# mpkuse/rgbd_odometry

Measured on AMD Instinct MI355X. Metric: frame-pair aligns/sec (640x480, 4-lvl pyr), higher is better.
Workload: dtype f32

## Files before the change

include/dvo_amd.h:

```cpp
#ifndef DVO_AMD_H_
#define DVO_AMD_H_

#include <stddef.h>
#include <stdint.h>

#ifdef __cplusplus
extern "C" {
#endif

#define DVO_MAX_LEVELS 8
#define DVO_NUM_ACC 29

enum {
    DVO_OK = 0,
    DVO_ERR_INVALID = 1,
    DVO_ERR_NO_DEVICE = 2,
    DVO_ERR_HIP = 3,
    DVO_ERR_STATE = 4,
    DVO_ERR_NOMEM = 5
};

enum {
    DVO_FLAG_FINAL_OUTPUTS = 1,
    DVO_FLAG_IDENTITY_START = 2,
// ... 62 lines not shown
                                   float *xyz_out, float *uv_out, int capacity, int *N_out);

int  dvo_run_iterations(dvo_ctx *ctx, int level, int max_iters, double *R, double *t,
                        float *energy, float *final_eps, float *final_reproj,
                        int *best_idx, float *visible_ratio);
int  dvo_run_iterations_pair(dvo_ctx *ctx, int pair, int level, int max_iters, double *R, double *t,
                             float *energy, float *final_eps, float *final_reproj,
                             int *best_idx, float *visible_ratio);

int  dvo_align_pyramid(dvo_ctx *ctx, int n_levels, const int *iters, int flags, double *R, double *t);
int  dvo_align_batch(dvo_ctx *ctx, int first_pair, int n_pairs, int n_levels, const int *iters,
                     int flags, double *R, double *t);

int  dvo_set_poses(dvo_ctx *ctx, int first_pair, int n_pairs, const double *R, const double *t);
int  dvo_align_batch_enqueue(dvo_ctx *ctx, int first_pair, int n_pairs, int n_levels,
                             const int *iters, int flags);
int  dvo_get_poses(dvo_ctx *ctx, int first_pair, int n_pairs, double *R, double *t);

int  dvo_get_level_report(dvo_ctx *ctx, int pair, int level, float *energy, int n_energy,
                          int *best_idx, float *visible_ratio);
int  dvo_get_level_normal_matrix(dvo_ctx *ctx, int pair, int level, int itr, double *H36);
int  dvo_get_final_outputs(dvo_ctx *ctx, int pair, float *final_eps, float *final_reproj, int capacity,
                           int *N_out);

int  dvo_iter_begin(dvo_ctx *ctx, int pair, int level, int max_iters, const double *R, const double *t);
int  dvo_iter_accumulate(dvo_ctx *ctx, int pair, int level, int first_point, int n_points, double *d_acc32);
int  dvo_iter_update(dvo_ctx *ctx, int pair, int level, int itr, int n_total, const double *d_acc32);
int  dvo_iter_end(dvo_ctx *ctx, int pair, int level, double *R, double *t, float *energy ,
                  int *best_idx, float *visible_ratio);

int  dvo_align_pyramid_wide(dvo_ctx *ctx, int pair, int n_levels, const int *iters, int flags, double *R, double *t);

int  dvo_tiled_attach(dvo_ctx *ctx, void *nccl_comm, int rank, int world, const char *rccl_library);
int  dvo_tiled_detach(dvo_ctx *ctx);
int  dvo_align_pyramid_tiled(dvo_ctx *ctx, int pair, int n_levels, const int *iters, int flags, double *R, double *t);
int  dvo_tiled_shard(dvo_ctx *ctx, int pair, int level, int *first, int *count);
int  dvo_tiled_graph_replayed(dvo_ctx *ctx, int *graph_replayed);
int  dvo_wide_packed_levels(dvo_ctx *ctx, int *levels_mask, int *solo_mask);
int  dvo_wide_team_levels(dvo_ctx *ctx, int *levels_mask);

int  dvo_eval_points(dvo_ctx *ctx, int pair, int level, const double *R, const double *t,
                     float *reproj, float *J, float *eps, float *w, int *visible);
int  dvo_accumulate(dvo_ctx *ctx, int pair, int level, const double *R, const double *t,
                    double *acc29);
int  dvo_device_se3_exp(dvo_ctx *ctx, const double *psi6, double *R, double *t);
int  dvo_device_se3_log(dvo_ctx *ctx, const double *R, const double *t, double *psi6);
int  dvo_device_rotationize(dvo_ctx *ctx, double *R);

int  dvo_get_level_texel_mode(dvo_ctx *ctx, int pair, int level, int *mode);
int  dvo_get_level_exact_fallback(dvo_ctx *ctx, int pair, int level, int *ran);
int  dvo_get_level_energy_sweeps(dvo_ctx *ctx, int pair, int level, int *n);
int  dvo_get_level_points4(dvo_ctx *ctx, int pair, int level, int *used);
int  dvo_get_level_ranks_in_lds(dvo_ctx *ctx, int pair, int level, int *used);

int  dvo_get_last_launch_shape(dvo_ctx *ctx, int *block_threads, int *team_size, int *packed);

#define DVO_COMPACT_NOW_AFTER 16
int  dvo_now_prepare(dvo_ctx *ctx, int first_pair, int count);
int  dvo_set_direct_compact(dvo_ctx *ctx, int on);
int  dvo_get_now_compact_info(dvo_ctx *ctx, int pair, int level, int *palette_size);
int  dvo_get_now_compact_partial(dvo_ctx *ctx, int pair, int level, int *partial);

int  dvo_debug_stamps(dvo_ctx *ctx, int pair, unsigned long long *out64);

int  dvo_algorithmic_bytes(dvo_ctx *ctx, int pair, int n_levels, const int *iters, int flags,
                           uint64_t *bytes);
int  dvo_point_iterations(dvo_ctx *ctx, int pair, int n_levels, const int *iters, uint64_t *count);

enum { DVO_PIX_U8 = 0, DVO_PIX_U16 = 1, DVO_PIX_F32 = 2 };
enum { DVO_LAYOUT_COL_MAJOR = 0,
       DVO_LAYOUT_ROW_MAJOR = 1 };
enum { DVO_UPLOAD_ASYNC = 1,
       DVO_UPLOAD_DEPTH_RAW = 2,
       DVO_UPLOAD_DIRECT = 4 };
enum { DVO_UPLOAD_MAPPED = 16 };
void *dvo_host_alloc_mapped(size_t bytes);
void  dvo_host_free_mapped(void *p);
enum { DVO_UPLOAD_DEVICE = 8 };

typedef struct dvo_image {
    const void *data;
    int rows, cols;
    int dtype;
    int layout;
} dvo_image;

int  dvo_frames_reserve(dvo_ctx *ctx, int n_slots);
int  dvo_frames_upload_pyramids(dvo_ctx *ctx, int first_slot, int count, int n_levels,
                                const dvo_image *grey, const dvo_image *depth, int now_first_pair, int flags);
int  dvo_frames_set_undistort(dvo_ctx *ctx, int rows, int cols, const double *K4, const double *D5);
int  dvo_frames_upload_cameras(dvo_ctx *ctx, int first_slot, int count, const unsigned char *const *bgr8,
                               const float *const *depth_m, int rows, int cols, int n_levels, int first_shift,
                               int now_first_pair, int flags);
int  dvo_frames_as_now(dvo_ctx *ctx, int first_slot, int first_pair, int count);
int  dvo_frames_as_ref(dvo_ctx *ctx, int first_slot, int first_pair, int count, int *N_out);
int  dvo_frame_get_level(dvo_ctx *ctx, int slot, int level, int *rows, int *cols, unsigned char *grey,
                         float *depth_mm, unsigned char *edge, int *n_edges);
int  dvo_frames_num_levels(const dvo_ctx *ctx);

typedef struct dvo_photo_params {
    double fx, fy, cx, cy;
    int    gradient_threshold;
    int    max_jacobian_size;
    int    min_required_pts;
    int    iterations;
    double eps_norm_stop;
// ... 14 lines not shown
```

rgbd_odometry_amd/capi.py:

```python
from __future__ import annotations

import ctypes as C
import os
from typing import Optional, Sequence

import numpy as np

DVO_MAX_LEVELS = 8
DVO_NUM_ACC = 29
DVO_OK, DVO_ERR_INVALID, DVO_ERR_NO_DEVICE, DVO_ERR_HIP, DVO_ERR_STATE, DVO_ERR_NOMEM = range(6)
DVO_FLAG_FINAL_OUTPUTS = 1
DVO_FLAG_IDENTITY_START = 2
DVO_FLAG_NORMAL_MATRIX = 4

_HERE = os.path.dirname(os.path.abspath(__file__))

C_ABI_SYMBOLS = [
    "dvo_params_default", "dvo_create", "dvo_create_batch", "dvo_destroy", "dvo_last_error",
    "dvo_num_pairs", "dvo_set_stream", "dvo_use_own_stream", "dvo_synchronize", "dvo_set_keep_warm", "dvo_set_keep_warm2", "dvo_set_intrinsics",
    "dvo_set_ref_level", "dvo_set_ref_level_pair", "dvo_set_now_level", "dvo_set_now_level_pair",
    "dvo_set_ref_level_device", "dvo_set_now_level_device", "dvo_set_ref_level_from_images",
    "dvo_run_iterations", "dvo_run_iterations_pair", "dvo_align_pyramid", "dvo_align_batch",
    "dvo_set_poses", "dvo_align_batch_enqueue", "dvo_get_poses", "dvo_get_level_report",
    "dvo_get_final_outputs", "dvo_get_level_normal_matrix", "dvo_eval_points", "dvo_accumulate", "dvo_device_se3_exp",
    "dvo_device_se3_log", "dvo_device_rotationize", "dvo_algorithmic_bytes", "dvo_point_iterations",
    "dvo_debug_stamps", "dvo_get_level_texel_mode", "dvo_get_level_exact_fallback", "dvo_get_level_energy_sweeps", "dvo_get_level_points4", "dvo_get_level_ranks_in_lds", "dvo_now_prepare", "dvo_set_direct_compact", "dvo_host_alloc_mapped", "dvo_host_free_mapped", "dvo_get_now_compact_info", "dvo_get_now_compact_partial", "dvo_get_last_launch_shape", "dvo_replicate_pairs", "dvo_set_now_level_from_edges", "dvo_get_now_level", "dvo_iter_begin", "dvo_iter_accumulate", "dvo_iter_update", "dvo_iter_end",
    "dvo_align_pyramid_wide", "dvo_tiled_attach", "dvo_tiled_detach", "dvo_align_pyramid_tiled", "dvo_tiled_shard", "dvo_tiled_graph_replayed", "dvo_wide_packed_levels", "dvo_wide_team_levels",
    "dvo_get_ref_level", "dvo_frames_reserve", "dvo_frames_upload_pyramids", "dvo_frames_upload_cameras", "dvo_frames_set_undistort",
    "dvo_photo_params_default", "dvo_photo_configure", "dvo_photo_set_ref", "dvo_photo_align", "dvo_photo_get_jacobian", "dvo_frames_as_now",
    "dvo_frames_as_ref", "dvo_frame_get_level", "dvo_frames_num_levels",
]

DVO_PIX_U8, DVO_PIX_U16, DVO_PIX_F32 = 0, 1, 2
DVO_LAYOUT_COL_MAJOR, DVO_LAYOUT_ROW_MAJOR = 0, 1
DVO_UPLOAD_ASYNC = 1
DVO_UPLOAD_DEPTH_RAW = 2
DVO_UPLOAD_DIRECT = 4
DVO_UPLOAD_DEVICE = 8
DVO_UPLOAD_MAPPED = 16


class DvoImage(C.Structure):
    _fields_ = [("data", C.c_void_p), ("rows", C.c_int), ("cols", C.c_int), ("dtype", C.c_int), ("layout", C.c_int)]


class DvoParams(C.Structure):
    _fields_ = [
        ("beta", C.c_double), ("precond_rot", C.c_double), ("reg_lambda", C.c_double),
        ("step_a", C.c_double), ("step_b", C.c_double),
        ("step_decay_after", C.c_int), ("step_decay_offset", C.c_int),
        ("trust_radius", C.c_float), ("psi_norm_stop", C.c_float),
        ("enable_rotationize", C.c_int), ("enable_l2_reg", C.c_int), ("interpolate_dt", C.c_int),
        ("block_threads", C.c_int), ("points_in_flight", C.c_int), ("engine_variant", C.c_int),
        ("lds_point_bytes", C.c_int), ("debug_alias_mod", C.c_int),
        ("canny_threshold1", C.c_int), ("canny_threshold2", C.c_int), ("team_size", C.c_int),
    ]


class DvoPhotoParams(C.Structure):
    _fields_ = [("fx", C.c_double), ("fy", C.c_double), ("cx", C.c_double), ("cy", C.c_double),
                ("gradient_threshold", C.c_int), ("max_jacobian_size", C.c_int), ("min_required_pts", C.c_int),
                ("iterations", C.c_int), ("eps_norm_stop", C.c_double), ("fixed", C.c_int), ("reserved", C.c_int)]


class RcclComm:
    RCCL = "/opt/rocm/lib/librccl.so.1"

    class _Id(C.Structure):
        _fields_ = [("internal", C.c_char * 128)]

    @classmethod
    def _lib(cls):
        import torch
        lib = C.CDLL(cls.RCCL, mode=C.RTLD_GLOBAL)
        lib.ncclGetUniqueId.argtypes = [C.POINTER(cls._Id)]
        lib.ncclCommInitRank.argtypes = [C.POINTER(C.c_void_p), C.c_int, cls._Id, C.c_int]
        lib.ncclCommDestroy.argtypes = [C.c_void_p]
        return lib

# ... 95 lines not shown
        return _lib
    if os.environ.get("DVO_NO_TORCH", "0") != "1":
        import torch
    path = library_path()
    if not os.path.exists(path) and not os.environ.get("DVO_LIB_VARIANT"):
        _build_native()
    if not os.path.exists(path):
        raise FileNotFoundError(
            f"{path} not found: build the HIP extension first "
            "(python -c 'import __graft_entry__ as g; g.build()' or make -C rgbd_odometry_amd/csrc)")
    lib = C.CDLL(path)
    vp, ip, fp, dp = C.c_void_p, C.POINTER(C.c_int), C.POINTER(C.c_float), C.POINTER(C.c_double)
    i, f = C.c_int, C.c_float
    sig = {
        "dvo_params_default": [C.POINTER(DvoParams)],
        "dvo_create": [C.POINTER(DvoParams), C.POINTER(vp)],
        "dvo_create_batch": [C.POINTER(DvoParams), i, C.POINTER(vp)],
        "dvo_destroy": [vp],
        "dvo_num_pairs": [vp],
        "dvo_set_stream": [vp, vp],
        "dvo_use_own_stream": [vp],
        "dvo_synchronize": [vp],
        "dvo_set_keep_warm": [vp, i],
        "dvo_set_keep_warm2": [vp, i, i],
        "dvo_set_intrinsics": [vp, f, f, f, f],
        "dvo_set_ref_level": [vp, i, vp, i],
        "dvo_set_ref_level_pair": [vp, i, i, vp, i],
        "dvo_set_now_level": [vp, i, vp, vp, vp, i, i],
        "dvo_set_now_level_pair": [vp, i, i, vp, vp, vp, i, i],
        "dvo_set_ref_level_device": [vp, i, i, vp, i],
        "dvo_set_now_level_device": [vp, i, i, vp, vp, vp, i, i],
        "dvo_set_ref_level_from_images": [vp, i, i, vp, vp, i, i, vp, vp, i, ip],
        "dvo_run_iterations": [vp, i, i, vp, vp, vp, vp, vp, ip, fp],
        "dvo_run_iterations_pair": [vp, i, i, i, vp, vp, vp, vp, vp, ip, fp],
        "dvo_align_pyramid": [vp, i, ip, i, vp, vp],
        "dvo_align_batch": [vp, i, i, i, ip, i, vp, vp],
        "dvo_set_poses": [vp, i, i, vp, vp],
        "dvo_align_batch_enqueue": [vp, i, i, i, ip, i],
        "dvo_get_poses": [vp, i, i, vp, vp],
        "dvo_get_level_report": [vp, i, i, vp, i, ip, fp],
        "dvo_get_final_outputs": [vp, i, vp, vp, i, ip],
        "dvo_get_level_normal_matrix": [vp, i, i, i, vp],
        "dvo_eval_points": [vp, i, i, vp, vp, vp, vp, vp, vp, vp],
        "dvo_accumulate": [vp, i, i, vp, vp, vp],
        "dvo_device_se3_exp": [vp, vp, vp, vp],
        "dvo_device_se3_log": [vp, vp, vp, vp],
        "dvo_device_rotationize": [vp, vp],
        "dvo_debug_stamps": [vp, i, vp],
        "dvo_get_level_texel_mode": [vp, i, i, ip],
        "dvo_get_level_exact_fallback": [vp, i, i, ip],
        "dvo_get_level_energy_sweeps": [vp, i, i, ip],
        "dvo_get_level_points4": [vp, i, i, ip],
        "dvo_get_level_ranks_in_lds": [vp, i, i, ip],
        "dvo_now_prepare": [vp, i, i],
        "dvo_get_last_launch_shape": [vp, ip, ip, ip],
        "dvo_get_now_compact_info": [vp, i, i, ip],
        "dvo_get_now_compact_partial": [vp, i, i, ip],
        "dvo_set_direct_compact": [vp, i],
        "dvo_host_alloc_mapped": [C.c_size_t],
        "dvo_host_free_mapped": [vp],
        "dvo_replicate_pairs": [vp, i, i, i],
        "dvo_set_now_level_from_edges": [vp, i, i, vp, i, i],
        "dvo_get_now_level": [vp, i, i, vp, vp, vp],
        "dvo_iter_begin": [vp, i, i, i, vp, vp],
        "dvo_iter_accumulate": [vp, i, i, i, i, vp],
        "dvo_iter_update": [vp, i, i, i, i, vp],
        "dvo_iter_end": [vp, i, i, vp, vp, vp, ip, fp],
        "dvo_align_pyramid_wide": [vp, i, i, ip, i, vp, vp],
        "dvo_frames_set_undistort": [vp, i, i, vp, vp],
        "dvo_photo_params_default": [C.POINTER(DvoPhotoParams)],
        "dvo_photo_configure": [vp, C.POINTER(DvoPhotoParams)],
        "dvo_photo_set_ref": [vp, i, i, ip],
        "dvo_photo_align": [vp, i, ip, i, vp, vp, ip],
        "dvo_photo_get_jacobian": [vp, i, vp, vp, vp, i, vp, ip],
        "dvo_tiled_attach": [vp, vp, i, i, C.c_char_p],
        "dvo_tiled_detach": [vp],
        "dvo_align_pyramid_tiled": [vp, i, i, ip, i, vp, vp],
        "dvo_tiled_shard": [vp, i, i, ip, ip],
        "dvo_tiled_graph_replayed": [vp, ip],
        "dvo_wide_packed_levels": [vp, ip, ip],
        "dvo_wide_team_levels": [vp, ip],
        "dvo_get_ref_level": [vp, i, i, vp, i, ip],
        "dvo_frames_reserve": [vp, i],
        "dvo_frames_upload_pyramids": [vp, i, i, i, C.POINTER(DvoImage), C.POINTER(DvoImage), i, i],
        "dvo_frames_upload_cameras": [vp, i, i, C.POINTER(vp), C.POINTER(vp), i, i, i, i, i, i],
        "dvo_frames_as_now": [vp, i, i, i],
        "dvo_frames_as_ref": [vp, i, i, i, ip],
        "dvo_frame_get_level": [vp, i, i, ip, ip, vp, vp, vp, ip],
        "dvo_frames_num_levels": [vp],
        "dvo_algorithmic_bytes": [vp, i, i, ip, i, C.POINTER(C.c_uint64)],
        "dvo_point_iterations": [vp, i, i, ip, C.POINTER(C.c_uint64)],
    }
    for name, args in sig.items():
        fn = getattr(lib, name)
        fn.argtypes = args
        fn.restype = C.c_int
    lib.dvo_last_error.argtypes = [vp]
    lib.dvo_last_error.restype = C.c_char_p
    lib.dvo_host_alloc_mapped.restype = C.c_void_p
    lib.dvo_host_free_mapped.restype = None
    _lib = lib
    return lib


def _f32(a) -> np.ndarray:
    return np.ascontiguousarray(a, dtype=np.float32)
# ... 417 lines not shown
        psi = np.array(psi, dtype=np.float64)
        R = np.zeros((3, 3), order="F")
        t = np.zeros(3)
        self._chk(self.lib.dvo_device_se3_exp(self._h, _ptr(psi), _ptr(R), _ptr(t)))
        return R, t

    def se3_log(self, R, t):
        R = np.array(R, dtype=np.float64, order="F")
        t = np.array(t, dtype=np.float64)
        psi = np.zeros(6)
        self._chk(self.lib.dvo_device_se3_log(self._h, _ptr(R), _ptr(t), _ptr(psi)))
        return psi

    def rotationize(self, R):
        R = np.array(R, dtype=np.float64, order="F").copy(order="F")
        self._chk(self.lib.dvo_device_rotationize(self._h, _ptr(R)))
        return R

    def debug_stamps(self, pair: int = 0) -> np.ndarray:
        out = np.zeros(64, np.uint64)
        self._chk(self.lib.dvo_debug_stamps(self._h, pair, _ptr(out)))
        return out.reshape(8, 8)

    def level_normal_matrix(self, pair: int, level: int, itr: int = -1) -> np.ndarray:
        H = np.zeros(36, np.float64)
        self._chk(self.lib.dvo_get_level_normal_matrix(self._h, pair, level, itr, _ptr(H)))
        return H.reshape(6, 6)

    def level_texel_mode(self, pair: int, level: int) -> int:
        m = C.c_int(-2)
        self._chk(self.lib.dvo_get_level_texel_mode(self._h, pair, level, C.byref(m)))
        return m.value

    def level_energy_sweeps(self, pair: int, level: int) -> int:
        m = C.c_int(0)
        self._chk(self.lib.dvo_get_level_energy_sweeps(self._h, pair, level, C.byref(m)))
        return m.value

    def level_exact_fallback(self, pair: int, level: int) -> bool:
        m = C.c_int(0)
        self._chk(self.lib.dvo_get_level_exact_fallback(self._h, pair, level, C.byref(m)))
        return bool(m.value)

    def level_points4(self, pair: int, level: int) -> bool:
        m = C.c_int(0)
        self._chk(self.lib.dvo_get_level_points4(self._h, pair, level, C.byref(m)))
        return bool(m.value)

    def level_ranks_in_lds(self, pair: int, level: int) -> bool:
        m = C.c_int(0)
        self._chk(self.lib.dvo_get_level_ranks_in_lds(self._h, pair, level, C.byref(m)))
        return bool(m.value)

    def last_launch_shape(self):
        b, t, k = C.c_int(0), C.c_int(0), C.c_int(0)
        self._chk(self.lib.dvo_get_last_launch_shape(self._h, C.byref(b), C.byref(t), C.byref(k)))
        return b.value, t.value, bool(k.value)

    def now_prepare(self, first_pair: int = 0, count: Optional[int] = None):
        count = self.n_pairs - first_pair if count is None else count
        self._chk(self.lib.dvo_now_prepare(self._h, first_pair, count))

    def set_direct_compact(self, on: bool = True):
        self._chk(self.lib.dvo_set_direct_compact(self._h, 1 if on else 0))

    def now_compact_info(self, pair: int, level: int) -> int:
        m = C.c_int(0)
        self._chk(self.lib.dvo_get_now_compact_info(self._h, pair, level, C.byref(m)))
        return m.value

    def now_compact_partial(self, pair: int, level: int) -> bool:
        m = C.c_int(0)
        self._chk(self.lib.dvo_get_now_compact_partial(self._h, pair, level, C.byref(m)))
        return bool(m.value)

    def algorithmic_bytes(self, iters: Sequence[int], pair: int = 0, flags: int = 0) -> int:
        b = C.c_uint64(0)
        self._chk(self.lib.dvo_algorithmic_bytes(self._h, pair, len(iters), _iters(iters), flags, C.byref(b)))
        return b.value

    def point_iterations(self, iters: Sequence[int], pair: int = 0) -> int:
        b = C.c_uint64(0)
        self._chk(self.lib.dvo_point_iterations(self._h, pair, len(iters), _iters(iters), C.byref(b)))
        return b.value
```

rgbd_odometry_amd/csrc/dvo_capi.cpp:

```cpp
#include "dvo_ctx.h"
#include "dvo_palette.h"

#include <atomic>
#include <chrono>
#include <thread>

using namespace dvo;


namespace { thread_local std::string g_create_error; }

namespace dvo_host {

int fail(dvo_ctx *c, int code, const std::string &msg) {
    if (c) c->err = msg; else g_create_error = msg;
    return code;
}

hipError_t stream_wait(hipStream_t s) {
    static const bool block = [] { const char *e = std::getenv("DVO_WAIT"); return e && std::strcmp(e, "block") == 0; }();
    if (!block) {
        const auto t0 = std::chrono::steady_clock::now();
        for (int n = 0;; n++) {
            const hipError_t e = hipStreamQuery(s);
// ... 139 lines not shown
    HIPCHK(c, hipMemcpyAsync(pn.data(), L.d_pal_n + first, sizeof(int) * (size_t)count, hipMemcpyDeviceToHost, stream));
    HIPCHK(c, stream_wait(stream));
    if (L.p4_known.empty()) { L.p4_known.assign(c->n_pairs, Level::P4_UNKNOWN); L.p4_fresh.assign(c->n_pairs, 0); }
    auto needs_tex = [&](int v) { return v <= 0 || pal_partial(v); };
    for (int i = 0; i < count; i++) {
        L.p4_known[first + i] = pn[i] <= 0 ? Level::P4_REFUSED : (pal_partial(pn[i]) ? Level::P4_PARTIAL : Level::P4_OK);
        L.p4_fresh[first + i] = 1;
    }
    int n = 0;
    for (int i = 0; i < count; ) {
        if (!needs_tex(pn[i])) { i++; continue; }
        int j = i;
        while (j < count && needs_tex(pn[j])) j++;
        const int rc = map_texels(c, level, first + i, j - i, stream);
        if (rc) return rc;
        n += j - i;
        i = j;
    }
    *n_failed = n;
    return DVO_OK;
}
int refresh_p4_known(dvo_ctx *c, int level, int first, int count, bool skip_native) {
    Level &L = c->lv[level];
    if (!L.d_pal_n || L.pal_built.empty()) return DVO_OK;
    if (L.p4_known.empty()) { L.p4_known.assign(c->n_pairs, Level::P4_UNKNOWN); L.p4_fresh.assign(c->n_pairs, 0); }
    if (L.p4_native.empty()) L.p4_native.assign(c->n_pairs, 0);
    auto unknown = [&](int p) { return L.pal_built[p] && L.p4_known[p] == Level::P4_UNKNOWN && !(skip_native && L.p4_native[p]); };
    for (int p = first; p < first + count; ) {
        if (!unknown(p)) { p++; continue; }
        int q = p;
        while (q < first + count && unknown(q)) q++;
        std::vector<int> pn((size_t)(q - p));
        HIPCHK(c, hipMemcpyAsync(pn.data(), L.d_pal_n + p, sizeof(int) * (size_t)(q - p), hipMemcpyDeviceToHost, c->stream));
        HIPCHK(c, stream_wait(c->stream));
        for (int i = p; i < q; i++) {
            const int v = pn[i - p];
            L.p4_known[i] = v <= 0 ? Level::P4_REFUSED : (pal_partial(v) ? Level::P4_PARTIAL : Level::P4_OK);
            if ((v <= 0 || pal_partial(v)) && !L.tex16_stale.empty()) L.tex16_stale[i] = 0;
        }
        p = q;
    }
    return DVO_OK;
}

int ensure_texels(dvo_ctx *c, int level, int rows, int cols) {
    Level &L = c->lv[level];
    if (L.have_now.empty()) L.have_now.assign(c->n_pairs, 0);
    if (L.tex && L.rows == rows && L.cols == cols) return DVO_OK;
    if (L.tex) {
        HIPCHK(c, stream_wait(c->stream));
        free_texels(c, L);
        std::fill(L.have_now.begin(), L.have_now.end(), 0);
        if (L.p4) { (void)hipFree(L.p4); (void)hipFree(L.pal); (void)hipFree(L.d_pal_n); L.p4 = nullptr; L.pal = nullptr; L.d_pal_n = nullptr; }
        L.pal_built.clear(); L.now_uses.clear(); L.tex16_stale.clear(); L.p4_known.clear(); L.p4_fresh.clear(); L.p4_native.clear();
    }

    L.rows = rows; L.cols = cols;
    L.tex_stride = texel_count(rows, cols);
    const size_t bytes = sizeof(float4) * L.tex_stride * c->n_pairs;
    if (tex_sparse_wanted(bytes)) {
        hipMemAllocationProp prop = {};
        prop.type = hipMemAllocationTypePinned;
        prop.location.type = hipMemLocationTypeDevice;
        prop.location.id = c->device;
        size_t gran = 0;
        void *va = nullptr;
        if (hipMemGetAllocationGranularity(&gran, &prop, hipMemAllocationGranularityMinimum) == hipSuccess && gran > 0) {
            const size_t chunk = ((((size_t)16 << 20) + gran - 1) / gran) * gran;
            const size_t va_bytes = (bytes + chunk - 1) / chunk * chunk;
            if (hipMemAddressReserve(&va, va_bytes, chunk, nullptr, 0) == hipSuccess && va) {
                L.tex = reinterpret_cast<float4 *>(va);
                L.tex_sparse = true; L.tex_chunk = chunk; L.tex_va_bytes = va_bytes;
                L.tex_handles.assign(va_bytes / chunk, hipMemGenericAllocationHandle_t{});
                L.tex_mapped.assign(va_bytes / chunk, 0);
                return DVO_OK;
            }
        }
        (void)hipGetLastError();
    }
    HIPCHK(c, hipMalloc((void **)&L.tex, bytes));
    if (L.tex_stride != (size_t)rows * cols)
        HIPCHK(c, hipMemsetAsync(L.tex, 0, bytes, c->stream));
    return DVO_OK;
}

static void level_flags(dvo_ctx *c, Level &L) {
    if (L.pal_built.empty()) { L.pal_built.assign(c->n_pairs, 0); L.now_uses.assign(c->n_pairs, 0); }
    if (L.tex16_stale.empty()) L.tex16_stale.assign(c->n_pairs, 0);
    if (L.have_now.empty()) L.have_now.assign(c->n_pairs, 0);
    if (L.p4_known.empty()) { L.p4_known.assign(c->n_pairs, Level::P4_UNKNOWN); L.p4_fresh.assign(c->n_pairs, 0); }
    if (L.p4_native.empty()) L.p4_native.assign(c->n_pairs, 0);
}

bool native_compact_wanted(const dvo_ctx *c) { return c->prm.engine_variant != 4 && compact_now_policy() != 2; }
static bool direct_compact_wanted(const dvo_ctx *c) {
    const char *e = getenv("DVO_DIRECT_COMPACT");
    const bool on = e ? !strcmp(e, "on") : (c->direct_compact < 0 ? c->n_pairs >= 64 : c->direct_compact != 0);
    return native_compact_wanted(c) && on;
}
static bool p4_addressable(int rows, int cols) {
    return !(p4_count(rows, cols) * sizeof(unsigned) >= ((size_t)1 << 32) || rows >= (1 << 16) || ((cols + 3) >> 2) >= (1 << 24) ||
             (size_t)p4_tiles_per_col(rows) * 128 >= ((size_t)1 << 24));
}

int ensure_compact_slabs(dvo_ctx *c, int level) {
    Level &L = c->lv[level];
    if (L.p4) return DVO_OK;
    L.p4_stride = p4_count(L.rows, L.cols);
    HIPCHK(c, hipMalloc((void **)&L.p4, sizeof(unsigned) * L.p4_stride * c->n_pairs));
    HIPCHK(c, hipMalloc((void **)&L.pal, sizeof(float2) * DVO_PAL_MAX * (size_t)c->n_pairs));
    HIPCHK(c, hipMalloc((void **)&L.d_pal_n, sizeof(int) * (size_t)c->n_pairs));
    HIPCHK(c, hipMemsetAsync(L.d_pal_n, 0, sizeof(int) * (size_t)c->n_pairs, c->stream));
    HIPCHK(c, stream_wait(c->stream));
    return DVO_OK;
}

int now_written_compact(dvo_ctx *c, int level, int first_pair, int count) {
    Level &L = c->lv[level];
    level_flags(c, L);
    for (int p = first_pair; p < first_pair + count; p++) {
        L.have_now[p] = 1; L.now_uses[p] = 0; L.pal_built[p] = 1;
        L.p4_native[p] = 1;
        if (L.p4_fresh[p]) L.p4_fresh[p] = 0;
        else L.p4_known[p] = Level::P4_UNKNOWN;
        L.tex16_stale[p] = (L.p4_known[p] == Level::P4_REFUSED || L.p4_known[p] == Level::P4_PARTIAL) ? 0 : 1;
    }
    return DVO_OK;
}

int ensure_tex16(dvo_ctx *c, int level, int first_pair, int count) {
    Level &L = c->lv[level];
    if (L.tex16_stale.empty() || !L.p4) return DVO_OK;
    for (int p = first_pair; p < first_pair + count; ) {
        if (!L.tex16_stale[p]) { p++; continue; }
        int q = p;
        while (q < first_pair + count && L.tex16_stale[q]) q++;
        { const int mrc = map_texels(c, level, p, q - p); if (mrc) return mrc; }
        HIPCHK(c, launch_p4_decode_texels(L.p4, L.p4_stride, L.pal, L.d_pal_n, L.tex, L.tex_stride, L.rows, L.cols, p, q - p, c->stream));
        for (int i = p; i < q; i++) L.tex16_stale[i] = 0;
        p = q;
    }
    return DVO_OK;
}

int now_written(dvo_ctx *c, int level, int first_pair, int count) {
    Level &L = c->lv[level];
    level_flags(c, L);
    for (int p = first_pair; p < first_pair + count; p++) { L.tex16_stale[p] = 0; L.p4_known[p] = Level::P4_UNKNOWN; L.p4_fresh[p] = 0; L.p4_native[p] = 0; }
    for (int p = first_pair; p < first_pair + count; ) {
        L.have_now[p] = 1; L.now_uses[p] = 0;
        if (!L.pal_built[p]) { p++; continue; }
        int q = p;
        while (q < first_pair + count && L.pal_built[q]) { L.pal_built[q] = 0; L.have_now[q] = 1; L.now_uses[q] = 0; q++; }
        HIPCHK(c, hipMemsetAsync(L.d_pal_n + p, 0, sizeof(int) * (size_t)(q - p), c->stream));
        p = q;
    }
    return DVO_OK;
}

int build_compact_now(dvo_ctx *c, int level, int first_pair, int count, bool only_reused) {
    Level &L = c->lv[level];
    if (!L.tex || L.have_now.empty()) return DVO_OK;
    if (p4_count(L.rows, L.cols) * sizeof(unsigned) >= ((size_t)1 << 32) || L.rows >= (1 << 16) || ((L.cols + 3) >> 2) >= (1 << 24) ||
        (size_t)p4_tiles_per_col(L.rows) * 128 >= ((size_t)1 << 24))
        return DVO_OK;
    level_flags(c, L);
    for (int p = first_pair; p < first_pair + count; ) {
        auto wanted = [&](int i) { return L.have_now[i] && !L.pal_built[i] && (!only_reused || L.now_uses[i] >= DVO_COMPACT_NOW_AFTER); };
        if (!wanted(p)) { p++; continue; }
        int q = p;
        while (q < first_pair + count && wanted(q)) q++;
        { const int rc = ensure_compact_slabs(c, level); if (rc) return rc; }
        for (int b = p; b < q; b += 1024) {
            const int nb = std::min(1024, q - b);
            if (palette_work_ints(nb) > c->pal_work_ints) {
                if (c->pal_work) { HIPCHK(c, stream_wait(c->stream)); HIPCHK(c, hipFree(c->pal_work)); c->pal_work = nullptr; c->pal_work_ints = 0; }
                HIPCHK(c, hipMalloc((void **)&c->pal_work, sizeof(unsigned) * palette_work_ints(nb)));
                c->pal_work_ints = palette_work_ints(nb);
            }
            HIPCHK(c, launch_palette_build(L.tex, L.tex_stride, L.rows, L.cols, L.p4, L.p4_stride, L.pal, L.d_pal_n, b, nb, c->pal_work, c->stream));
        }
        for (int i = p; i < q; i++) { L.pal_built[i] = 1; L.p4_known[i] = Level::P4_UNKNOWN; if (!L.p4_native.empty()) L.p4_native[i] = 0; }
        p = q;
    }
    return DVO_OK;
}

}

using namespace dvo_host;

namespace dvo_host {

LevelSlab slab_of(const dvo_ctx *c, int level) {
    const Level &L = c->lv[level];
    LevelSlab s;
    s.tex = L.tex; s.pts = L.pts; s.cpts = L.cpts; s.cidx = L.cidx; s.N = L.dN;
    s.cpt4 = L.cpt4; s.chdr = L.chdr; s.pt4_ok = L.d_pt4_ok;
    s.tex_stride = L.tex_stride; s.pt_cap = L.pt_cap; s.rows = L.rows; s.cols = L.cols;
    s.p4 = L.p4; s.pal = L.pal; s.pal_n = L.d_pal_n; s.p4_stride = L.p4_stride;
    return s;
}

int check_ready(dvo_ctx *c, int pair, int level) {
    if (!c->have_K) return fail(c, DVO_ERR_STATE, "intrinsics not set (dvo_set_intrinsics)");
    const Level &L = c->lv[level];
    if (L.hN.empty() || L.hN[pair] <= 0)
        return fail(c, DVO_ERR_STATE, "reference points of pair " + std::to_string(pair) + " level " +
                                          std::to_string(level) + " not set");
    if (L.have_now.empty() || !L.have_now[pair])
        return fail(c, DVO_ERR_STATE, "now level " + std::to_string(level) + " of pair " +
                                          std::to_string(pair) + " not set");
    return DVO_OK;
}

int build_schedule(dvo_ctx *c, int n_levels, const int *iters, int flags, Schedule &sc) {
    if (n_levels < 1 || n_levels > DVO_LEVELS || !iters) return fail(c, DVO_ERR_INVALID, "bad level schedule");
    std::memset(&sc, 0, sizeof(sc));
    sc.n_levels = n_levels;
    sc.flags = flags;
    sc.last_level = -1;
    int off = 0;
    for (int l = 0; l < n_levels; l++) {
        sc.iters[l] = iters[l] > 0 ? iters[l] : 0;
        sc.e_off[l] = off;
        off += sc.iters[l];
    }
    for (int l = n_levels - 1; l >= 0; l--) if (sc.iters[l] > 0) sc.last_level = l;
    if (sc.last_level < 0) return fail(c, DVO_ERR_INVALID, "schedule has no iterations");
    sc.e_stride = off;
    return DVO_OK;
}

int ensure_outputs(dvo_ctx *c, const Schedule &sc) {
    const size_t need = (size_t)sc.e_stride * c->n_pairs;
    if (need > c->energy_floats) {
        if (c->d_energy) { HIPCHK(c, stream_wait(c->stream)); HIPCHK(c, hipFree(c->d_energy)); }
        HIPCHK(c, hipMalloc((void **)&c->d_energy, sizeof(float) * need));
        c->energy_floats = need;
        c->sched_gen++;
    }
    if (sc.flags & DVO_FLAG_NORMAL_MATRIX) {
        const size_t needH = need * 21;
        if (needH > c->H_doubles) {
            if (c->d_H) { HIPCHK(c, stream_wait(c->stream)); HIPCHK(c, hipFree(c->d_H)); }
            HIPCHK(c, hipMalloc((void **)&c->d_H, sizeof(double) * needH));
            c->H_doubles = needH;
            c->sched_gen++;
        }
    }
    if (sc.flags & DVO_FLAG_FINAL_OUTPUTS) {
        const int cap = c->lv[sc.last_level].pt_cap;
        if (cap > c->final_cap) {
// ... 136 lines not shown
            for (int p = first_pair; p < first_pair + n_pairs; p++) max_n = std::max(max_n, c->lv[l].hN[p]);
        }
        if ((size_t)max_n * 12 <= 77000 && !c->prm.interpolate_dt && 2 * n_pairs > c->n_cu) { block = 256; auto_lds = 80 * 1024; }
        else if (all_p4 && 2 * n_pairs >= 3 * c->n_cu && (size_t)max_n * 8 <= 2 * (size_t)77000) { block = 256; auto_lds = 80 * 1024; }
        else if (all_p4 && n_pairs > c->n_cu) { block = 256; auto_lds = 80 * 1024; }
        else if ((size_t)max_n * 12 > 4 * (size_t)155000 && !c->prm.interpolate_dt) { block = 1024; auto_lds = 155000; }
        else { block = 512; auto_lds = 155000; }
    }
    {
        int bytes = c->prm.lds_point_bytes;
        if (bytes == 0) bytes = auto_lds ? auto_lds : ((block >= 512) ? 155000 : 80 * 1024);
        if (packed && block_auto && block == 1024) block = 512;
        const int static_lds = packed ? (int)fused2_static_lds(block, with_h) : (int)(sizeof(double) * (block / 64) * DVO_NACC_PAD + 256 + pose_state_bytes());
        const int max_dyn = ((block == 256) ? 80 * 1024 : 160 * 1024) - static_lds - 64;
        if (bytes > max_dyn) bytes = max_dyn;
        if (bytes < 0) bytes = 0;
        bytes &= ~63;
        sc.lds_bytes = bytes;
        sc.no_lds_tex = (c->prm.engine_variant == 2) ? 1 : 0;
        sc.force_exact = (c->prm.engine_variant == 3) ? 1 : 0;
        sc.force_e2 = (c->prm.engine_variant == 5) ? 1 : 0;
        static const bool no_pt4_env = [] { const char *e = std::getenv("DVO_POINTS4"); return e && std::strcmp(e, "off") == 0; }();
        sc.no_pt4 = no_pt4_env ? 1 : 0;
        static const int pt4_factor_env = [] { const char *e = std::getenv("DVO_POINTS4_FACTOR"); return e ? std::atoi(e) : 1; }();
        sc.pt4_factor = pt4_factor_env;
        for (int l = 0; l < n_levels && !sc.no_pt4; l++) {
            if (sc.iters[l] <= 0 || c->lv[l].pt4_rows.empty()) continue;
            const Level &L = c->lv[l];
            for (int p = first_pair; p < first_pair + n_pairs; p++) {
                const int dp = sc.alias_mod > 0 ? p % sc.alias_mod : p;
                if (L.pt4_rows[dp] != 0 && L.pt4_rows[dp] != L.rows) { sc.no_pt4 = 1; break; }
            }
        }
        sc.lds_points = bytes / (sc.compact ? 8 : 12);
        if (c->prm.lds_point_bytes < 0) { sc.lds_points = 0; sc.lds_bytes = 0; }
    }
    if (!packed || sc.no_p4 || (size_t)sc.lds_bytes < sizeof(float2) * DVO_PAL_MAX + 64) {
        if (!packed) sc.no_p4 = 1;
        for (int l = 0; l < n_levels; l++) {
            if (sc.iters[l] <= 0) continue;
            if ((rc = ensure_tex16(c, l, first_pair, n_pairs))) return rc;
            if (sc.alias_mod > 0 && (rc = ensure_tex16(c, l, 0, std::min(sc.alias_mod, c->n_pairs)))) return rc;
        }
    }
    int u = c->prm.points_in_flight;
    if (u != 1 && u != 2 && u != 4) u = 1;
    sc.team = 1;
    sc.n_pairs_launch = n_pairs;
    {
        static const bool no_plain = [] { const char *e = std::getenv("DVO_TEAM_PLAIN_STORES"); return e && std::strcmp(e, "off") == 0; }();
        sc.team_no_plain = no_plain ? 1 : 0;
        static const bool no_r16 = [] { const char *e = std::getenv("DVO_RANKS_LDS"); return e && std::strcmp(e, "off") == 0; }();
        sc.no_r16 = no_r16 ? 1 : 0;
        static const int solo_max = [] { const char *e = std::getenv("DVO_TEAM_SOLO_MAX"); return e ? std::atoi(e) : DVO_TEAM_SOLO_MAX_DEFAULT; }();
        sc.team_solo_max = solo_max;
    }
    c->team_used = false;
    if (sc.compact && c->prm.engine_variant != 1 && !(sc.flags & DVO_FLAG_NORMAL_MATRIX) && block == 512 && c->prm.team_size != 1) {
        const int slots8 = 8 * ((n_pairs + 7) / 8);
        int n_fine = 0;
        for (int p = first_pair; p < first_pair + n_pairs; p++) n_fine = std::max(n_fine, c->lv[sc.last_level].hN[p]);
        const int g_cap = (n_fine >= 262144) ? 32 : ((n_fine >= 65536) ? 16 : 8);
        int g = 1;
        if (n_fine >= 5000)
            while (g * 2 <= g_cap && slots8 * g * 2 <= c->n_cu && n_fine >= 1800 * g * 2) g *= 2;
        bool super_team = (n_pairs == 1 && n_fine >= 100000 && c->n_cu >= 256);
        if (super_team) g = (n_fine >= 400000) ? 256 : 64;
        if (c->prm.team_size > 1) {
            g = c->prm.team_size;
            super_team = (g == 64 || g == 128 || g == 256) && n_pairs == 1;
            if (super_team ? (g > c->n_cu) : (g > 32 || slots8 * g > c->n_cu))
                return fail(c, DVO_ERR_INVALID, "team_size: the launch would need more workgroups than compute units (members must be co-resident; 64 / 128 / 256 only for a single pair)");
        }
        if (g > 1) {
            const size_t buf_bytes = 16 * 2 * 32 * 8 * (size_t)std::max(c->n_pairs, 9);
            bool zero = false;
            if (!c->d_team_buf) {
                HIPCHK(c, hipMalloc((void **)&c->d_team_buf, buf_bytes));
                HIPCHK(c, hipMalloc((void **)&c->d_team_cnt, sizeof(unsigned) * ((size_t)c->n_pairs + 1)));
                zero = c->team_err_dirty = true;
                if (const char *e = std::getenv("DVO_TEAM_EPOCH0")) c->team_epoch = (unsigned)std::strtoul(e, nullptr, 0);
            }
            unsigned need = 2;
            for (int l = 0; l < n_levels; l++) if (sc.iters[l] > 0) need += 2u * (unsigned)sc.iters[l] + 2u;
            hipStreamCaptureStatus cap = hipStreamCaptureStatusNone;
            if (c->stream && hipStreamIsCapturing(c->stream, &cap) == hipSuccess && cap != hipStreamCaptureStatusNone) c->team_legacy = true;
            if (c->team_legacy || c->team_epoch > 0xfffffff0u - need) zero = true;
            if (zero) {
                HIPCHK(c, hipMemsetAsync(c->d_team_buf, 0, buf_bytes, c->stream));
                if (c->team_legacy || c->team_epoch > 0xfffffff0u - need) c->team_epoch = 0;
            }
            if (c->team_err_dirty || c->team_legacy) {
                HIPCHK(c, hipMemsetAsync(c->d_team_cnt, 0, sizeof(unsigned) * ((size_t)c->n_pairs + 1), c->stream));
                c->team_err_dirty = false;
            }
            sc.team_epoch0 = c->team_epoch;
            if (!c->team_legacy) c->team_epoch += need;
            sc.team = g;
            c->team_used = true;
        }
    }
    if (packed) {
        Outputs o = outputs_of(c);
        static const bool no_lpt = std::getenv("DVO_NO_LPT") != nullptr;
        if (sc.team == 1 && n_pairs > c->n_cu && !no_lpt) {
            unsigned long long sched_hash = 1469598103934665603ull;
// ... 136 lines not shown
struct dvo_keep_warm_state {
    std::thread th;
    std::atomic<bool> stop{false};
    hipStream_t stream = nullptr;
    int busy_us = 0, pause_us = 0;
};
static void keep_warm_stop(dvo_ctx *c) {
    dvo_keep_warm_state *w = c->warm;
    if (!w) return;
    w->stop.store(true);
    if (w->th.joinable()) w->th.join();
    if (w->stream) { (void)hipStreamSynchronize(w->stream); (void)hipStreamDestroy(w->stream); }
    delete w;
    c->warm = nullptr;
}
int dvo_set_keep_warm2(dvo_ctx *c, int busy_us, int pause_us) {
    DVO_ENTER(c);
    keep_warm_stop(c);
    if (busy_us <= 0) return DVO_OK;
    dvo_keep_warm_state *w = new dvo_keep_warm_state();
    w->busy_us = busy_us; w->pause_us = pause_us < 0 ? 0 : pause_us;
    if (hipStreamCreateWithFlags(&w->stream, hipStreamNonBlocking) != hipSuccess) { delete w; return fail(c, DVO_ERR_HIP, "keep-warm: cannot create a stream"); }
    const int device = c->device;
    w->th = std::thread([w, device]() {
        (void)hipSetDevice(device);
        while (!w->stop.load()) {
            (void)launch_keep_warm(w->busy_us, w->stream);
            if (w->pause_us == 0) (void)launch_keep_warm(w->busy_us, w->stream);
            (void)hipStreamSynchronize(w->stream);
            if (w->pause_us > 0) std::this_thread::sleep_for(std::chrono::microseconds(w->pause_us));
        }
    });
    c->warm = w;
    return DVO_OK;
}
int dvo_set_keep_warm(dvo_ctx *c, int period_us) {
    return dvo_set_keep_warm2(c, period_us > 0 ? 5 : 0, period_us);
}

int dvo_destroy(dvo_ctx *c) {
    if (!c) return DVO_OK;
    DeviceGuard guard(c);
    keep_warm_stop(c);
    if (c->stream) (void)stream_wait(c->stream);
    for (int l = 0; l < DVO_LEVELS; l++) {
        free_texels(c, c->lv[l]);
        if (c->lv[l].pts) (void)hipFree(c->lv[l].pts);
        if (c->lv[l].cpts) (void)hipFree(c->lv[l].cpts);
        if (c->lv[l].cidx) (void)hipFree(c->lv[l].cidx);
        if (c->lv[l].cpt4) { (void)hipFree(c->lv[l].cpt4); (void)hipFree(c->lv[l].chdr); }
        if (c->lv[l].d_pt4_ok) (void)hipFree(c->lv[l].d_pt4_ok);
        if (c->lv[l].dN) (void)hipFree(c->lv[l].dN);
        if (c->lv[l].p4) { (void)hipFree(c->lv[l].p4); (void)hipFree(c->lv[l].pal); (void)hipFree(c->lv[l].d_pal_n); }
    }
    if (c->pal_work) (void)hipFree(c->pal_work);
    if (c->d_order) (void)hipFree(c->d_order);
    tiled_forget(c);
    photo_forget(c);
    for (int l = 0; l < DVO_LEVELS; l++) {
        FrameLevel &F = c->fs.lv[l];
        void *fp[] = {F.grey, F.edge, F.depth};
        for (void *p : fp) if (p) (void)hipFree(p);
    }
    if (c->work) (void)hipFree(c->work);
    if (c->d_umap_xy) (void)hipFree(c->d_umap_xy);
    if (c->d_umap_frac) (void)hipFree(c->d_umap_frac);
    if (c->wide_exec) (void)hipGraphExecDestroy(c->wide_exec);
    if (c->tiled_exec) (void)hipGraphExecDestroy(c->tiled_exec);
    if (c->d_step_state) { (void)hipFree(c->d_step_state); (void)hipFree(c->d_step_acc); (void)hipFree(c->d_step_ticket); }
    if (c->h_pose) (void)hipHostFree(c->h_pose);
    if (c->h_poses) (void)hipHostFree(c->h_poses);
    for (int l = 0; l < DVO_LEVELS; l++) {
        if (c->lvl_stream[l]) { (void)hipStreamSynchronize(c->lvl_stream[l]); (void)hipStreamDestroy(c->lvl_stream[l]); }
        if (c->ev_join[l]) (void)hipEventDestroy(c->ev_join[l]);
    }
    if (c->ev_fork) (void)hipEventDestroy(c->ev_fork);
    if (c->copy_stream) { (void)hipStreamSynchronize(c->copy_stream); (void)hipStreamDestroy(c->copy_stream); }
    if (c->copy_stream2) { (void)hipStreamSynchronize(c->copy_stream2); (void)hipStreamDestroy(c->copy_stream2); }
    for (int b = 0; b < 2; b++) {
        if (c->up_buf[b]) (void)hipFree(c->up_buf[b]);
        if (b == 0) { if (c->src_tab_dev) (void)hipFree(c->src_tab_dev); if (c->src_tab_host) (void)hipHostFree(c->src_tab_host); if (c->ev_src_tab) (void)hipEventDestroy(c->ev_src_tab); }
        if (c->up_host[b]) (void)hipHostFree(c->up_host[b]);
        if (c->ev_copied[b]) (void)hipEventDestroy(c->ev_copied[b]);
        if (c->ev_copied2[b]) (void)hipEventDestroy(c->ev_copied2[b]);
        if (c->ev_done[b]) (void)hipEventDestroy(c->ev_done[b]);
    }
    void *ptrs[] = {c->staging, c->d_poses, c->d_energy, c->d_best, c->d_ratio, c->d_final_eps,
                    c->d_final_reproj, c->d_final_N, c->d_scratch, c->d_colcounts, c->d_dbg,
                    c->d_states, c->d_iter_energy, c->d_tex_mode, c->d_H, c->d_team_buf, c->d_team_cnt};
    for (void *p : ptrs) if (p) (void)hipFree(p);
    if (c->own_stream) (void)hipStreamDestroy(c->own_stream);
    delete c;
    return DVO_OK;
}

const char *dvo_last_error(const dvo_ctx *c) { return c ? c->err.c_str() : g_create_error.c_str(); }
int dvo_num_pairs(const dvo_ctx *c) { return c ? c->n_pairs : 0; }

int dvo_set_stream(dvo_ctx *c, void *hip_stream) {
    DVO_ENTER(c);
    HIPCHK(c, stream_wait(c->stream));
    c->stream = (hipStream_t)hip_stream;
    return DVO_OK;
}
int dvo_use_own_stream(dvo_ctx *c) {
    DVO_ENTER(c);
// ... 150 lines not shown
            HIPCHK(c, hipMemcpyAsync(c->h_poses, L.d_pal_n + pair, sizeof(int), hipMemcpyDeviceToHost, c->stream));
        }
    }
    if (!device_src) {
        HIPCHK(c, stream_wait(c->stream));
        if (direct && *reinterpret_cast<const int *>(c->h_poses) <= 0) L.pal_built[pair] = 0;
    }
    return DVO_OK;
}
void *dvo_host_alloc_mapped(size_t bytes) {
    void *p = nullptr;
    if (bytes == 0 || hipHostMalloc(&p, bytes, hipHostMallocMapped | hipHostMallocPortable) != hipSuccess) { (void)hipGetLastError(); return nullptr; }
    return p;
}
void dvo_host_free_mapped(void *p) { if (p) (void)hipHostFree(p); }

int dvo_set_direct_compact(dvo_ctx *c, int on) {
    DVO_ENTER(c);
    c->direct_compact = on ? 1 : 0;
    return DVO_OK;
}
int dvo_set_now_level_pair(dvo_ctx *c, int pair, int level, const float *dt, const float *gx,
                           const float *gy, int rows, int cols) {
    return set_now_common(c, pair, level, dt, gx, gy, rows, cols, false);
}
int dvo_set_now_level(dvo_ctx *c, int level, const float *dt, const float *gx, const float *gy,
                      int rows, int cols) {
    return set_now_common(c, 0, level, dt, gx, gy, rows, cols, false);
}
int dvo_set_now_level_device(dvo_ctx *c, int pair, int level, const float *d_dt, const float *d_gx,
                             const float *d_gy, int rows, int cols) {
    return set_now_common(c, pair, level, d_dt, d_gx, d_gy, rows, cols, true);
}

int dvo_set_now_level_from_edges(dvo_ctx *c, int pair, int level, const unsigned char *edge, int rows, int cols) {
    DVO_ENTER(c);
    if (!pair_ok(c, pair) || !level_ok(level)) return fail(c, DVO_ERR_INVALID, "pair/level out of range");
    if (!edge || rows < 1 || cols < 1) return fail(c, DVO_ERR_INVALID, "bad image arguments");
    if ((long long)rows + cols + 1 > 46340) return fail(c, DVO_ERR_INVALID, "image too large for the exact distance transform (rows + cols must stay below 46339)");
    int rc = ensure_texels(c, level, rows, cols);
    if (rc) return rc;
    const size_t npx = (size_t)rows * cols;
    bool any = false;
    for (size_t i = 0; i < npx && !any; i++) any = edge[i] != 0;
    if (!any) return fail(c, DVO_ERR_INVALID, "edge mask has no edge pixel: the distance transform is undefined");
    const size_t edge_ints = (npx + 3) / 4;
    if ((rc = ensure_staging(c, sizeof(int) * (edge_ints + edt_work_ints(rows, cols, 1) + 1)))) return rc;
    unsigned char *d_edge = (unsigned char *)c->staging;
    int *work = (int *)c->staging + edge_ints;
    HIPCHK(c, hipMemcpyAsync(d_edge, edge, npx, hipMemcpyHostToDevice, c->stream));
    Level &L = c->lv[level];
    const bool compact = native_compact_wanted(c);
    if (compact && (rc = ensure_compact_slabs(c, level))) return rc;
    const bool defer = compact && L.tex_sparse;
    if (L.tex_sparse && !compact && (rc = map_texels(c, level, pair, 1))) return rc;
    HIPCHK(c, launch_edges_to_now(d_edge, 0, ImgBatch{rows, cols, 1}, work, defer ? nullptr : L.tex + (size_t)pair * L.tex_stride, L.tex_stride,
                                  compact ? L.p4 : nullptr, L.p4_stride, L.pal, L.d_pal_n, pair, c->stream));
    if (defer) {
        int n_failed = 0;
        if ((rc = sparse_map_compact_failures(c, level, pair, 1, c->stream, &n_failed))) return rc;
        if (n_failed)
            HIPCHK(c, launch_edges_to_now(d_edge, 0, ImgBatch{rows, cols, 1}, work, L.tex + (size_t)pair * L.tex_stride, L.tex_stride,
                                          L.p4, L.p4_stride, L.pal, L.d_pal_n, pair, c->stream, true));
    }
    if ((rc = compact ? now_written_compact(c, level, pair, 1) : now_written(c, level, pair, 1))) return rc;
    HIPCHK(c, stream_wait(c->stream));
    return DVO_OK;
}

int dvo_get_now_level(dvo_ctx *c, int pair, int level, float *dt, float *gx, float *gy) {
    DVO_ENTER(c);
    if (!pair_ok(c, pair) || !level_ok(level)) return fail(c, DVO_ERR_INVALID, "pair/level out of range");
    Level &L = c->lv[level];
    if (L.have_now.empty() || !L.have_now[pair]) return fail(c, DVO_ERR_STATE, "now level not set");
    const size_t npx = (size_t)L.rows * L.cols;
    int rc = ensure_staging(c, sizeof(float) * 3 * npx);
    if (rc) return rc;
    if ((rc = ensure_tex16(c, level, pair, 1))) return rc;
    float *d = c->staging;
    HIPCHK(c, launch_unpack_texels(L.tex + (size_t)pair * L.tex_stride, L.rows, L.cols, d, d + npx, d + 2 * npx, c->stream));
    if (dt) HIPCHK(c, hipMemcpyAsync(dt, d, sizeof(float) * npx, hipMemcpyDeviceToHost, c->stream));
    if (gx) HIPCHK(c, hipMemcpyAsync(gx, d + npx, sizeof(float) * npx, hipMemcpyDeviceToHost, c->stream));
    if (gy) HIPCHK(c, hipMemcpyAsync(gy, d + 2 * npx, sizeof(float) * npx, hipMemcpyDeviceToHost, c->stream));
    HIPCHK(c, stream_wait(c->stream));
    return DVO_OK;
}

int dvo_get_ref_level(dvo_ctx *c, int pair, int level, float *xyz_out, int capacity, int *N_out) {
    DVO_ENTER(c);
    if (!pair_ok(c, pair) || !level_ok(level)) return fail(c, DVO_ERR_INVALID, "pair/level out of range");
    Level &L = c->lv[level];
    if (L.hN.empty() || L.hN[pair] <= 0) return fail(c, DVO_ERR_STATE, "reference level not set");
    const int N = L.hN[pair];
    if (N_out) *N_out = N;
    const int ncopy = std::min(N, capacity);
    if (xyz_out && ncopy > 0) {
        HIPCHK(c, hipMemcpyAsync(xyz_out, L.pts + (size_t)pair * L.pt_cap * 3, sizeof(float) * 3 * (size_t)ncopy,
                                 hipMemcpyDeviceToHost, c->stream));
        HIPCHK(c, stream_wait(c->stream));
    }
    return DVO_OK;
}

int dvo_replicate_pairs(dvo_ctx *c, int n_src, int dst_first, int dst_count) {
    DVO_ENTER(c);
    if (n_src < 1 || dst_first < 0 || dst_count < 0 || dst_first + dst_count > c->n_pairs || n_src > c->n_pairs)
        return fail(c, DVO_ERR_INVALID, "bad replicate arguments");
    if (dst_first != 0 && dst_first < n_src) return fail(c, DVO_ERR_INVALID, "destination range overlaps the sources");
    for (int l = 0; l < DVO_LEVELS; l++) {
        Level &L = c->lv[l];
        if (!L.tex && !L.pts) continue;
        for (int p = 0; p < n_src; p++) {
            int rc = check_ready(c, p, l);
            if (rc) return rc;
        }
        { const int prc = refresh_p4_known(c, l, 0, n_src); if (prc) return prc; }
        bool any_tex16 = false, any_compact = false;
        for (int p = 0; p < n_src; p++) {
            const bool stale = !L.tex16_stale.empty() && L.tex16_stale[p];
            any_tex16 = any_tex16 || !stale;
            any_compact = any_compact || (!L.pal_built.empty() && L.pal_built[p]);
        }
        unsigned char *d_has_tex = nullptr;
        if (any_tex16 && L.tex) {
            std::vector<unsigned char> has((size_t)n_src);
            bool all = true;
            for (int p = 0; p < n_src; p++) { has[p] = !(!L.tex16_stale.empty() && L.tex16_stale[p]); all = all && has[p]; }
            for (int p = 0; p < n_src; p++)
                if (has[p]) { const int mrc = map_texels(c, l, p, 1); if (mrc) return mrc; }
            for (int p = dst_first; p < dst_first + dst_count; ) {
                if (!has[(p - dst_first) % n_src]) { p++; continue; }
                int q = p;
                while (q < dst_first + dst_count && has[(q - dst_first) % n_src]) q++;
                const int mrc = map_texels(c, l, p, q - p);
                if (mrc) return mrc;
                p = q;
            }
            if (!all) {
                HIPCHK(c, hipMalloc((void **)&d_has_tex, (size_t)n_src));
                HIPCHK(c, hipMemcpyAsync(d_has_tex, has.data(), (size_t)n_src, hipMemcpyHostToDevice, c->stream));
                HIPCHK(c, stream_wait(c->stream));
            }
        }
        {
            const hipError_t le = launch_replicate_level(any_tex16 ? L.tex : nullptr, d_has_tex, L.tex_stride, L.pts, L.cpts, L.cidx, L.cpt4, L.chdr, L.d_pt4_ok,
                                                         L.pt_cap, L.dN, n_src, dst_first, dst_count, c->stream);
            if (d_has_tex) { (void)hipStreamSynchronize(c->stream); (void)hipFree(d_has_tex); }
            HIPCHK(c, le);
        }
        for (int p = dst_first; p < dst_first + dst_count; p++) {
            const int src = (p - dst_first) % n_src;
            if (src == p) continue;
            L.hN[p] = L.hN[src];
            ref_list_written(c, l, p, 1, L.pt4_rows.empty() ? 0 : L.pt4_rows[src]);
            L.compact_ok[p] = L.compact_ok[src];
        }
        const int w_first = (dst_first == 0) ? std::min(n_src, dst_count) : dst_first;
        const int w_count = dst_first + dst_count - w_first;
        if (L.tex && w_count > 0) {
            int rc = now_written(c, l, w_first, w_count);
            if (rc) return rc;
            if (any_compact) {
                HIPCHK(c, launch_replicate_compact(L.p4, L.p4_stride, L.pal, L.d_pal_n, n_src, dst_first, dst_count, c->stream));
                for (int p = dst_first; p < dst_first + dst_count; p++) {
                    const int src = (p - dst_first) % n_src;
                    if (p == src) continue;
                    L.pal_built[p] = L.pal_built[src];
                    L.tex16_stale[p] = L.tex16_stale[src];
                    L.p4_known[p] = L.p4_known[src];
                    if (!L.p4_native.empty()) L.p4_native[p] = L.p4_native[src];
                }
            }
        }
    }
    HIPCHK(c, stream_wait(c->stream));
    return DVO_OK;
}

int dvo_get_last_launch_shape(dvo_ctx *c, int *block_threads, int *team_size, int *packed) {
    DVO_ENTER(c);
    if (block_threads) *block_threads = c->last_block;
    if (team_size) *team_size = c->last_team;
    if (packed) *packed = c->last_packed;
    return DVO_OK;
}

int dvo_now_prepare(dvo_ctx *c, int first_pair, int count) {
    DVO_ENTER(c);
    if (!pair_ok(c, first_pair) || count < 1 || first_pair + count > c->n_pairs) return fail(c, DVO_ERR_INVALID, "pair range out of bounds");
    if (c->prm.engine_variant == 4 || compact_now_policy() == 2) return DVO_OK;
    for (int l = 0; l < DVO_LEVELS; l++) {
        int rc = build_compact_now(c, l, first_pair, count, false);
        if (rc) return rc;
    }
    HIPCHK(c, stream_wait(c->stream));
    return DVO_OK;
}

int dvo_get_now_compact_info(dvo_ctx *c, int pair, int level, int *palette_size) {
    DVO_ENTER(c);
    if (!pair_ok(c, pair) || !level_ok(level) || !palette_size) return fail(c, DVO_ERR_INVALID, "bad arguments");
    Level &L = c->lv[level];
    *palette_size = 0;
    if (!L.d_pal_n) return DVO_OK;
    HIPCHK(c, hipMemcpyAsync(palette_size, L.d_pal_n + pair, sizeof(int), hipMemcpyDeviceToHost, c->stream));
    HIPCHK(c, stream_wait(c->stream));
    if (*palette_size > 0) *palette_size = pal_count(*palette_size);
    return DVO_OK;
}
int dvo_get_now_compact_partial(dvo_ctx *c, int pair, int level, int *partial) {
    DVO_ENTER(c);
    if (!pair_ok(c, pair) || !level_ok(level) || !partial) return fail(c, DVO_ERR_INVALID, "bad arguments");
    Level &L = c->lv[level];
    *partial = 0;
    if (!L.d_pal_n) return DVO_OK;
    int v = 0;
// ... 596 lines not shown
    HIPCHK(c, hipMemcpyAsync(psi6, d + 16, sizeof(double) * 6, hipMemcpyDeviceToHost, c->stream));
    HIPCHK(c, stream_wait(c->stream));
    return DVO_OK;
}
int dvo_device_rotationize(dvo_ctx *c, double *R) {
    DVO_ENTER(c);
    if (!R) return DVO_ERR_INVALID;
    double *d = c->d_scratch;
    HIPCHK(c, hipMemcpyAsync(d, R, sizeof(double) * 9, hipMemcpyHostToDevice, c->stream));
    HIPCHK(c, launch_rotationize(d, c->stream));
    HIPCHK(c, hipMemcpyAsync(R, d, sizeof(double) * 9, hipMemcpyDeviceToHost, c->stream));
    HIPCHK(c, stream_wait(c->stream));
    return DVO_OK;
}

int dvo_debug_stamps(dvo_ctx *c, int pair, unsigned long long *out64) {
    DVO_ENTER(c);
    if (!out64 || !pair_ok(c, pair)) return DVO_ERR_INVALID;
    std::memset(out64, 0, sizeof(unsigned long long) * 64);
    if (!c->d_dbg) return DVO_OK;
    HIPCHK(c, stream_wait(c->stream));
    HIPCHK(c, hipMemcpy(out64, c->d_dbg + (size_t)pair * 64, sizeof(unsigned long long) * 64, hipMemcpyDeviceToHost));
    HIPCHK(c, hipMemset(c->d_dbg + (size_t)pair * 64, 0, sizeof(unsigned long long) * 64));
    return DVO_OK;
}

int dvo_get_level_texel_mode(dvo_ctx *c, int pair, int level, int *mode) {
    DVO_ENTER(c);
    if (!pair_ok(c, pair) || !level_ok(level) || !mode) return fail(c, DVO_ERR_INVALID, "bad arguments");
    HIPCHK(c, stream_wait(c->stream));
    int v = -1;
    HIPCHK(c, hipMemcpy(&v, c->d_tex_mode + (size_t)pair * DVO_LEVELS + level, sizeof(int), hipMemcpyDeviceToHost));
    *mode = (v < 0) ? -1 : (v & 0xff);
    return DVO_OK;
}
int dvo_get_level_points4(dvo_ctx *c, int pair, int level, int *used) {
    DVO_ENTER(c);
    if (!pair_ok(c, pair) || !level_ok(level) || !used) return fail(c, DVO_ERR_INVALID, "bad arguments");
    HIPCHK(c, stream_wait(c->stream));
    int v = -1;
    HIPCHK(c, hipMemcpy(&v, c->d_tex_mode + (size_t)pair * DVO_LEVELS + level, sizeof(int), hipMemcpyDeviceToHost));
    *used = (v >= 0 && (v & DVO_TEXMODE_PT4)) ? 1 : 0;
    return DVO_OK;
}
int dvo_get_level_ranks_in_lds(dvo_ctx *c, int pair, int level, int *used) {
    DVO_ENTER(c);
    if (!pair_ok(c, pair) || !level_ok(level) || !used) return fail(c, DVO_ERR_INVALID, "bad arguments");
    HIPCHK(c, stream_wait(c->stream));
    int v = -1;
    HIPCHK(c, hipMemcpy(&v, c->d_tex_mode + (size_t)pair * DVO_LEVELS + level, sizeof(int), hipMemcpyDeviceToHost));
    *used = (v >= 0 && (v & DVO_TEXMODE_RANKS_LDS)) ? 1 : 0;
    return DVO_OK;
}
int dvo_get_level_exact_fallback(dvo_ctx *c, int pair, int level, int *ran) {
    DVO_ENTER(c);
    if (!pair_ok(c, pair) || !level_ok(level) || !ran) return fail(c, DVO_ERR_INVALID, "bad arguments");
    HIPCHK(c, stream_wait(c->stream));
    int v = -1;
    HIPCHK(c, hipMemcpy(&v, c->d_tex_mode + (size_t)pair * DVO_LEVELS + level, sizeof(int), hipMemcpyDeviceToHost));
    *ran = (v >= 0 && (v & DVO_TEXMODE_EXACT_RAN)) ? 1 : 0;
    return DVO_OK;
}

int dvo_get_level_energy_sweeps(dvo_ctx *c, int pair, int level, int *n) {
    DVO_ENTER(c);
    if (!pair_ok(c, pair) || !level_ok(level) || !n) return fail(c, DVO_ERR_INVALID, "bad arguments");
    HIPCHK(c, stream_wait(c->stream));
    int v = -1;
    HIPCHK(c, hipMemcpy(&v, c->d_tex_mode + (size_t)pair * DVO_LEVELS + level, sizeof(int), hipMemcpyDeviceToHost));
    *n = (v < 0) ? 0 : ((v >> DVO_TEXMODE_E2_SHIFT) & DVO_TEXMODE_E2_MAX);
    return DVO_OK;
}

int dvo_algorithmic_bytes(dvo_ctx *c, int pair, int n_levels, const int *iters, int flags, uint64_t *bytes) {
    DVO_ENTER(c);
    if (!bytes) return DVO_ERR_INVALID;
    if (!pair_ok(c, pair)) return fail(c, DVO_ERR_INVALID, "pair out of range");
    Schedule sc;
    int rc = build_schedule(c, n_levels, iters, flags, sc);
    if (rc) return rc;
    uint64_t b = 0;
    for (int l = 0; l < n_levels; l++) {
        if (sc.iters[l] <= 0) continue;
        if ((rc = check_ready(c, pair, l))) return rc;
        b += 12ull * (uint64_t)c->lv[l].rows * (uint64_t)c->lv[l].cols;
        b += 12ull * (uint64_t)c->lv[l].hN[pair];
    }
    if (flags & DVO_FLAG_FINAL_OUTPUTS) b += 16ull * (uint64_t)c->lv[sc.last_level].hN[pair];
    *bytes = b;
    return DVO_OK;
}

int dvo_point_iterations(dvo_ctx *c, int pair, int n_levels, const int *iters, uint64_t *count) {
    DVO_ENTER(c);
    if (!count) return DVO_ERR_INVALID;
    if (!pair_ok(c, pair)) return fail(c, DVO_ERR_INVALID, "pair out of range");
    Schedule sc;
    int rc = build_schedule(c, n_levels, iters, 0, sc);
    if (rc) return rc;
    uint64_t n = 0;
    for (int l = 0; l < n_levels; l++) {
        if (sc.iters[l] <= 0) continue;
        if ((rc = check_ready(c, pair, l))) return rc;
        n += (uint64_t)sc.iters[l] * (uint64_t)c->lv[l].hN[pair];
    }
    *count = n;
// ... 5 lines not shown
```

rgbd_odometry_amd/csrc/dvo_ctx.h:

```cpp
#ifndef DVO_CTX_H_
#define DVO_CTX_H_

#include "../../include/dvo_amd.h"
#include "dvo_launch.h"

#include <algorithm>
#include <cmath>
#include <cstdio>
#include <cstdlib>
#include <cstring>
#include <functional>
#include <string>
#include <vector>

namespace dvo_host {

struct Level {
    int rows = 0, cols = 0;
    float4 *tex = nullptr;
    size_t tex_stride = 0;
    bool tex_sparse = false;
    size_t tex_chunk = 0, tex_va_bytes = 0;
    std::vector<hipMemGenericAllocationHandle_t> tex_handles;
    std::vector<char> tex_mapped;
    float *pts = nullptr;
    uint2 *cpts = nullptr;
    unsigned *cidx = nullptr;
    unsigned *cpt4 = nullptr;
    unsigned *chdr = nullptr;
    int *d_pt4_ok = nullptr;
    std::vector<char> compact_ok;
    std::vector<unsigned long long> list_gen;
    std::vector<int> pt4_rows;
    int pt_cap = 0;
    int *dN = nullptr;
    std::vector<int> hN;
    std::vector<char> have_now;
    unsigned *p4 = nullptr;
    float2 *pal = nullptr;
    int *d_pal_n = nullptr;
    size_t p4_stride = 0;
    std::vector<char> pal_built;
    std::vector<int> now_uses;
    std::vector<char> tex16_stale;
    enum : char { P4_UNKNOWN = 0, P4_OK = 1, P4_REFUSED = 2, P4_PARTIAL = 3  };
    std::vector<char> p4_known;
    std::vector<char> p4_native;
    std::vector<char> p4_fresh;
};

struct FrameLevel {
    int rows = 0, cols = 0;
    size_t npx = 0;
    unsigned char *grey = nullptr, *edge = nullptr;
    float *depth = nullptr;
};
struct FrameStore {
    int n_slots = 0, n_levels = 0;
    FrameLevel lv[DVO_LEVELS];
    std::vector<char> valid, has_depth;
};
inline bool compact_block_order() {
    static const bool on = [] { const char *e = std::getenv("DVO_COMPACT_ORDER"); return !(e && std::strcmp(e, "colmajor") == 0); }();
    return on;
}
inline int compact_now_policy() {
    static const int pol = [] {
        const char *e = std::getenv("DVO_COMPACT_NOW");
        return (e && std::strcmp(e, "eager") == 0) ? 1 : ((e && std::strcmp(e, "off") == 0) ? 2 : 0);
    }();
    return pol;
}
}

struct dvo_ctx {
    dvo_params prm;
    dvo::DevParams dprm;
    int n_pairs = 0;
    int device = 0;
    int n_cu = 256;
    hipStream_t stream = nullptr;
    hipStream_t own_stream = nullptr;
    dvo::Intrinsics K{0, 0, 0, 0, 0};
    bool have_K = false;
    dvo_host::Level lv[DVO_LEVELS];
    float *staging = nullptr;
    size_t staging_bytes = 0;
    double *d_poses = nullptr;
    float *d_energy = nullptr;
    size_t energy_floats = 0;
    int *d_best = nullptr;
    float *d_ratio = nullptr;
    float *d_final_eps = nullptr, *d_final_reproj = nullptr;
    int *d_final_N = nullptr;
// ... 134 lines not shown
```

rgbd_odometry_amd/csrc/dvo_edt_band.h:

```cpp
#ifndef DVO_EDT_BAND_H_
#define DVO_EDT_BAND_H_

constexpr int EB_PAD = 8;
constexpr unsigned EB_D2_END = 32000;
constexpr int EB_LUT_WORDS = (int)(EB_D2_END / 32);
constexpr int EB_TRIPS = 23;
constexpr int EB_NANR = 1;
constexpr int EB_MAX_ROWS = 512, EB_MAX_COLS = 1024;
static_assert(EB_D2_END % 32 == 0 && (8 * EB_TRIPS + 1) * (8 * EB_TRIPS + 1) >= (int)EB_D2_END && (8 * EB_TRIPS + 1) * (8 * EB_TRIPS + 1) < 65536, "scan radius");

struct EdtSosLut { unsigned bm[EB_LUT_WORDS]; unsigned short pre[EB_LUT_WORDS]; int total; };
constexpr EdtSosLut edt_sos_lut_make() {
    EdtSosLut t{};
    for (unsigned a = 0; a * a < EB_D2_END; a++)
        for (unsigned b = a; a * a + b * b < EB_D2_END; b++) { const unsigned v = a * a + b * b; t.bm[v >> 5] |= 1u << (v & 31u); }
    int run = 0;
    for (int w = 0; w < EB_LUT_WORDS; w++) {
        t.pre[w] = (unsigned short)run;
        unsigned v = t.bm[w];
        while (v) { v &= v - 1u; run++; }
    }
    t.total = run;
    return t;
}
__device__ const EdtSosLut EDT_SOS_LUT = edt_sos_lut_make();
static_assert(edt_sos_lut_make().total + 4 <= DVO_PAL_MAX, "every rank + the two fixed entries + the two entries a consumer copies beyond pal_n fit the 13-bit field");

struct EdtBandLevels {
    int n, first_pair;
    int rows[DVO_LEVELS], cols[DVO_LEVELS], nwords[DVO_LEVELS], nbands[DVO_LEVELS], tpc[DVO_LEVELS], n_partial[DVO_LEVELS];
    unsigned firstA[DVO_LEVELS + 1], firstB[DVO_LEVELS + 1];
    const unsigned char *edge[DVO_LEVELS]; size_t edge_stride[DVO_LEVELS];
    unsigned *maskT[DVO_LEVELS], *carryT[DVO_LEVELS];
    unsigned *imax[DVO_LEVELS]; int *done[DVO_LEVELS]; int *flags[DVO_LEVELS];
    const int *partial[DVO_LEVELS];
    unsigned *p4[DVO_LEVELS]; size_t p4_stride[DVO_LEVELS]; float2 *pal[DVO_LEVELS]; int *pal_n[DVO_LEVELS];
    int *list;
};

DVO_DEV unsigned eb_load_mask8(const unsigned char *col, bool vec, int y0, int rows) {
    if (y0 >= rows) return 0u;
    if (vec) {
        const uint2 v = *reinterpret_cast<const uint2 *>(col + y0);
        return edt_nonzero_bytes(v.x) | (edt_nonzero_bytes(v.y) << 4);
    }
    unsigned m = 0;
    for (int j = 0; j < 8; j++) if (y0 + j < rows && col[y0 + j] != 0) m |= 1u << j;
    return m;
}

__global__ void __launch_bounds__(512) edt_colmask_levels_kernel(const EdtBandLevels t) {
    __shared__ unsigned sm[16][33], sc[16][33];
    const int l = level_of_block(t.firstA, t.n, blockIdx.x);
    const int bx = (int)(blockIdx.x - t.firstA[l]), by = blockIdx.y;
    const int rows = t.rows[l], cols = t.cols[l], nwords = t.nwords[l];
    const int tid = threadIdx.x, lane = tid & 63, wave = tid >> 6;
    if (bx == 0 && tid == 0) { t.imax[l][by] = 0u; t.done[l][by] = 0; t.flags[l][by] = 0; }
    if (blockIdx.x == 0 && by == 0 && tid == 0) t.list[0] = 0;
    const unsigned char *img = t.edge[l] + (size_t)by * t.edge_stride[l];
    const int INF = DVO_EDT_INF(rows, cols);
    const int x0 = bx * 32;
    unsigned m8[4];
#pragma unroll
    for (int k = 0; k < 4; k++) {
        const int xx = x0 + wave + 8 * k;
        const unsigned char *col = img + (size_t)(xx < cols ? xx : 0) * rows;
        const unsigned m = eb_load_mask8(col, ((rows & 7) == 0) && ((reinterpret_cast<size_t>(col) & 7) == 0), lane * 8, rows);
        m8[k] = xx < cols ? m : 0u;
    }
    const int w = lane >> 2;
#pragma unroll
    for (int k = 0; k < 4; k++) {
        const unsigned long long bal = __ballot(m8[k] != 0u);
        unsigned v = m8[k] | ((unsigned)__shfl_down((int)m8[k], 1) << 8);
        v |= (unsigned)__shfl_down((int)v, 2) << 16;
        const unsigned long long lower = bal & ((1ull << (4 * w)) - 1ull);
        const unsigned long long upper = (w == 15) ? 0ull : (bal & (~0ull << (4 * w + 4)));
        const int lpu = lower ? 63 - __clzll((long long)lower) : 0;
        const int lpd = upper ? __ffsll((long long)upper) - 1 : 0;
        const unsigned mlu = (unsigned)__shfl((int)m8[k], lpu), mld = (unsigned)__shfl((int)m8[k], lpd);
        const int U = lower ? (32 * w - 1) - (lpu * 8 + (31 - __clz((int)mlu))) : INF;
        const int D = upper ? (lpd * 8 + (__ffs((int)mld) - 1)) - 32 * (w + 1) : INF;
        if ((lane & 3) == 0) { sm[w][wave + 8 * k] = v; sc[w][wave + 8 * k] = (unsigned)U | ((unsigned)D << 16); }
    }
    __syncthreads();
    unsigned *mk = t.maskT[l] + (size_t)by * nwords * cols, *cr = t.carryT[l] + (size_t)by * nwords * cols;
    for (int idx = tid; idx < nwords * 32; idx += 512) {
        const int ww = idx >> 5, c = idx & 31, xx = x0 + c;
        if (xx < cols) { mk[(size_t)ww * cols + xx] = sm[ww][c]; cr[(size_t)ww * cols + xx] = sc[ww][c]; }
// ... 188 lines not shown
    EDT_T(t_scanned);
#pragma unroll
    for (int it = 0; it < NI; it++) {
        const int p = it * THREADS + tid;
        if (p < total) {
            const int h = p & (LPC - 1), col = p / LPC;
            eb_lds4[(size_t)(EB_PAD + col) * C4 + h] = res[it];
            if (col == 1) eb_lds4[(size_t)(EB_PAD - 1) * C4 + h] = res[it];
            if (col == cols - 2) eb_lds4[(size_t)(EB_PAD + cols) * C4 + h] = res[it];
        }
    }
    __syncthreads();

    const int tpc = t.tpc[l], ntc = (cols + 3) >> 2;
    const int ty0 = band * T, nty = (tpc - ty0 < T) ? tpc - ty0 : T;
    unsigned *p4 = t.p4[l] + (size_t)(t.first_pair + by) * t.p4_stride[l];
    if (band == 0 && tid < 32) p4[tid] = 0u;
    bool part = false;
    {
        typedef __attribute__((address_space(3))) const unsigned lds_cu;
        constexpr int PL = 16 * T, G = THREADS / PL;
        const int grp = tid / PL, rem = tid - grp * PL;
        const int tyl = rem >> 4, xl = (rem >> 2) & 3, sp = rem & 3;
        const int ty = ty0 + tyl;
        const int ys0 = ty * DVO_P4_ROWS + 2 * sp - 1;
        const bool in0 = sp >= 1 && ys0 < rows;
        const bool in1 = sp <= 2 && ys0 + 1 < rows;
        const unsigned keep = (in0 ? 0x0000ffffu : 0u) | (in1 ? 0xffff0000u : 0u);
        const unsigned cmask = (ys0 + 1 <= rows) ? 0xffffffffu : 0x0000ffffu;
        if (grp < G && tyl < nty) {
            unsigned lds_a = tq_lds + (unsigned)((EB_PAD + xl) * CB + (tyl * 3 + sp) * 4) + (unsigned)(grp * 4 * CB);
            unsigned *dst = p4 + 32u + ((size_t)grp * tpc + ty) * 32u + (xl * 8 + 2 * sp);
            for (int tc = grp; tc < ntc; tc += G, lds_a += (unsigned)(G * 4 * CB), dst += (size_t)G * tpc * 32u) {
                unsigned word0 = 0u, word1 = 0u;
                if (ys0 <= rows && tc * 4 + xl < cols) {
                    lds_cu *pc = (lds_cu *)(size_t)lds_a;
                    const unsigned C = pc[0] & cmask, R = pc[CD], L = pc[-CD];
                    const edt_us2 dR = edt_as_us2(R) - edt_as_us2(C), dL = edt_as_us2(L) - edt_as_us2(C);
                    const unsigned bad = (edt_as_u32(dR + edt_as_us2(0x00800080u)) | edt_as_u32(dL + edt_as_us2(0x00800080u))) & 0xff00ff00u & keep;
                    unsigned steps = __builtin_amdgcn_perm(edt_as_u32(dL), edt_as_u32(dR), 0x06020400u) & keep;
                    unsigned c0 = C & 0xffffu, c1 = C >> 16;
                    if (bad) {
                        if (bad & 0x0000ff00u) { c0 = EB_NANR; steps &= 0xffff0000u; }
                        if (bad & 0xff000000u) { c1 = EB_NANR; steps &= 0x0000ffffu; }
                        part = true;
                    }
                    word0 = (c0 << 3) | (steps << 16);
                    word1 = (c1 << 3) | (steps & 0xffff0000u);
                }
                *reinterpret_cast<uint2 *>(dst) = make_uint2(word0, word1);
            }
        }
    }
    EDT_T(t_words);
    EDT_ACC(3, t_scanned, t_words);

    __shared__ int s_red[THREADS / 64];
    for (int o = 32; o > 0; o >>= 1) { const unsigned v = (unsigned)__shfl_down((int)mx, o, 64); mx = v > mx ? v : mx; }
    if ((tid & 63) == 0) s_red[tid >> 6] = (int)mx;
    const int any_far = __syncthreads_or(far ? 1 : 0), any_part = __syncthreads_or(part ? 1 : 0);
    if (tid == 0) {
        int mred = 0;
        for (int k = 0; k < THREADS / 64; k++) mred = s_red[k] > mred ? s_red[k] : mred;
        unsigned seen = atomicMax(t.imax[l] + by, (unsigned)mred);
        if (any_far || any_part) seen += (unsigned)atomicOr(t.flags[l] + by, (int)EDT_FLAG_PARTIAL | (any_far ? (int)EDT_FLAG_FAR : 0));
        asm volatile("s_waitcnt vmcnt(0)" :: "v"(seen) : "memory");
        const bool last = atomicAdd(t.done[l] + by, 1) == t.nbands[l] - 1;
        if (last && (atomicOr(t.flags[l] + by, 0) & (int)EDT_FLAG_PARTIAL)) {
            const int k = atomicAdd(t.list, 1);
            t.list[1 + k] = (l << 24) | by;
        }
    }
#ifdef DVO_EDT_STAMPS
    {
        EDT_T(t_end);
        EDT_ACC(4, t_words, t_end);
        EDT_ACC(7, t_begin, t_end);
        acc_t[5] = 1;
        const unsigned slot = ((blockIdx.y * gridDim.x + blockIdx.x) * (unsigned)(THREADS / 64) + (threadIdx.x >> 6)) & (unsigned)(EDT_STAMP_SLOTS - 1);
        if ((threadIdx.x & 63) == 0)
            for (int k = 0; k < 8; k++) g_edt_stamp[slot][k] = acc_t[k];
    }
#endif
}

__global__ void __launch_bounds__(256) edt_palette_levels_kernel(const EdtBandLevels t) {
    const int l = blockIdx.x, by = blockIdx.y, tid = threadIdx.x;
    const int rows = t.rows[l], cols = t.cols[l], pair = t.first_pair + by;
    if (rows < 2 || cols < 2) { if (tid == 0) t.pal_n[l][pair] = -(int)PAL_SHAPE; return; }
    __shared__ int s_max;
    const int f = t.flags[l][by];
    int m = 0;
    if (f & (int)EDT_FLAG_FAR) {
        const int *partial = t.partial[l] + (size_t)by * t.n_partial[l];
        for (int k = tid; k < t.n_partial[l]; k += 256) { const int v = partial[k]; m = v > m ? v : m; }
    } else if (tid == 0) m = (int)t.imax[l][by];
    m = block_reduce_256<true>(m);
    if (tid == 0) s_max = m;
    __syncthreads();
    const unsigned m2 = (unsigned)s_max;
    const EdtScale sc = edt_scale(m2, rows, cols);
    const unsigned m2c = m2 < EB_D2_END ? m2 : EB_D2_END - 1u;
    float2 *pal = t.pal[l] + (size_t)pair * DVO_PAL_MAX;
    const int nw = (int)(m2c >> 5) + 1;
    const float qnan = __uint_as_float(0x7fc00000u);
    if (tid == 0) { pal[0] = make_float2(0.0f, 0.0f); pal[1] = make_float2(qnan, qnan); }
    for (int w = tid; w < nw; w += 256) {
        unsigned v = EDT_SOS_LUT.bm[w];
        int r = 2 + (int)EDT_SOS_LUT.pre[w];
        while (v) {
            const int b = __ffs((int)v) - 1;
            v &= v - 1u;
            const unsigned val = (unsigned)(w * 32 + b);
            if (val > m2c) break;
            const float P = edt_value(val, sc);
            pal[r] = make_float2(P, weight_of(P));
            r++;
        }
        if (w == nw - 1) {
            pal[r] = make_float2(0.0f, 0.0f); pal[r + 1] = make_float2(0.0f, 0.0f);
            t.pal_n[l][pair] = r | ((f & (int)EDT_FLAG_PARTIAL) ? DVO_PAL_PARTIAL : 0);
        }
    }
}

struct EdtListShape { int gx_cols[DVO_LEVELS], gxmax_cols, gxmax_rows; };
template <int WAVES>
__global__ void __launch_bounds__(WAVES * 64) edt_columns8_list_kernel(const EdtLevels t, const EdtListShape sh, const int *__restrict__ list) {
    const int n = list[0];
    for (int k = blockIdx.x; k < n * sh.gxmax_cols; k += gridDim.x) {
        const int e = list[1 + k / sh.gxmax_cols], bx = k % sh.gxmax_cols, l = e >> 24, by = e & 0xffffff;
        if (bx < sh.gx_cols[l])
            edt_columns8_body<WAVES>(bx, sh.gx_cols[l], by, t.edge[l], t.edge_stride[l], t.rows[l], t.cols[l], t.R, t.g[l], t.bitmap[l], t.bm_words[l], t.flags[l], true);
        __syncthreads();
    }
}
template <int R>
__global__ void __launch_bounds__(256) edt_rows_pk_list_kernel(const EdtLevels t, const EdtListShape sh, const int *__restrict__ list) {
    const int n = list[0];
    for (int k = blockIdx.x; k < n * sh.gxmax_rows; k += gridDim.x) {
        const int e = list[1 + k / sh.gxmax_rows], bx = k % sh.gxmax_rows, l = e >> 24, by = e & 0xffffff;
        if (bx < t.n_partial[l])
            edt_rows_pk_body<R>(bx, t.n_partial[l], by, t.g[l], t.rows[l], t.cols[l], t.d2[l], t.partial[l], t.bitmap[l], t.bm_words[l], t.flags[l]);
        __syncthreads();
    }
}

#endif
```

rgbd_odometry_amd/csrc/dvo_frames.hip:

```cpp
#include "dvo_launch.h"
#include "dvo_palette.h"
#include <stdlib.h>
#include <stdio.h>
#include <string.h>

namespace dvo {

namespace {

DVO_DEV float pow2_neg_f(int level) { return __int_as_float((127 - level) << 23); }
template <bool MAX>
DVO_DEV int block_reduce_256(int v) {
    __shared__ int part[4];
    for (int off = 32; off > 0; off >>= 1) { const int o = __shfl_down(v, off, 64); v = MAX ? (o > v ? o : v) : v + o; }
    if ((threadIdx.x & 63) == 0) part[threadIdx.x >> 6] = v;
    __syncthreads();
    if (threadIdx.x == 0) {
        for (int k = 1; k < 4; k++) v = MAX ? (part[k] > v ? part[k] : v) : v + part[k];
    }
    return v;
}
inline unsigned grid_x(size_t n, unsigned cap = 2048) {
    size_t b = (n + 255) / 256;
    if (b < 1) b = 1;
// ... 1689 lines not shown
    const int lane = threadIdx.x & 63, wave = threadIdx.x >> 6;
#pragma unroll
    for (int it = 0; it < 4; it++) {
        const int t = it * 32 + wave * 8 + (lane >> 3);
        const int cp = t >> 4, rg = t & 15;
        const int ly = rg * 4 + (lane & 3), lx = cp * 2 + ((lane >> 2) & 1);
        const int yy = y0 + ly, xx = x0 + lx;
        if (yy < rows && xx < cols) {
            const float *c = sn + (lx + 1) * SH + (ly + 1);
            const float v = c[0];
            out[texel_index(yy, xx, tpc)] = make_float4(v, 0.5f * c[SH] - 0.5f * c[-SH], 0.5f * c[1] - 0.5f * c[-1], weight_of(v));
        }
    }
    __syncthreads();
    }
}

template <int WAVES>
__global__ void __launch_bounds__(WAVES * 64)
edt_columns8_kernel(const unsigned char *__restrict__ edge, size_t edge_stride, int rows, int cols, int R, unsigned short *__restrict__ g,
                    unsigned *__restrict__ bitmap, int bm_words, int *__restrict__ flags) {
    edt_columns8_body<WAVES>(blockIdx.x, gridDim.x, blockIdx.y, edge, edge_stride, rows, cols, R, g, bitmap, bm_words, flags);
}
template <int R>
__global__ void __launch_bounds__(256)
edt_rows_pk_kernel(const unsigned short *__restrict__ g, int rows, int cols, unsigned *__restrict__ d2, int *__restrict__ partial,
                   unsigned *__restrict__ bitmap, int bm_words, int *__restrict__ flags) {
    edt_rows_pk_body<R>(blockIdx.x, gridDim.x, blockIdx.y, g, rows, cols, d2, partial, bitmap, bm_words, flags);
}
template <int BM_WORDS>
__global__ void __launch_bounds__(256)
edt_rank_pack_kernel(const unsigned *__restrict__ d2, int rows, int cols, int R, int tiles_y, int strip, const int *__restrict__ partial, int n_partial,
                     const unsigned *__restrict__ bitmap, int bm_words, int *__restrict__ flags,
                     unsigned *__restrict__ p4, size_t p4_stride, float2 *__restrict__ pal, int *__restrict__ pal_n, int first_pair,
                     const unsigned *__restrict__ unit_bits) {
    edt_rank_pack_body<BM_WORDS>(blockIdx.x, gridDim.x, blockIdx.y, d2, rows, cols, R, tiles_y, strip, partial, n_partial, bitmap, bm_words, flags,
                                 p4, p4_stride, pal, pal_n, first_pair, unit_bits);
}
__global__ void __launch_bounds__(256)
dt_normalize_gradient_pack_kernel(const unsigned *__restrict__ d2, int rows, int cols, int R, int tiles_y,
                                  const int *__restrict__ partial, int n_partial, float4 *__restrict__ out, size_t tex_stride,
                                  int *__restrict__ pal_n, const int *__restrict__ flags, int first_pair, int n_tiles) {
    dt_normalize_gradient_pack_body(blockIdx.x, gridDim.x, blockIdx.y, d2, rows, cols, R, tiles_y, partial, n_partial, out, tex_stride, pal_n, flags, first_pair, n_tiles);
}

struct EdtLevels {
    int n, R, first_pair;
    int rows[DVO_LEVELS], cols[DVO_LEVELS], bm_words[DVO_LEVELS], n_partial[DVO_LEVELS], ptiles_y[DVO_LEVELS], strip[DVO_LEVELS], ntiles_y[DVO_LEVELS];
    unsigned first[DVO_LEVELS + 1];
    const unsigned char *edge[DVO_LEVELS]; size_t edge_stride[DVO_LEVELS];
    unsigned short *g[DVO_LEVELS]; unsigned *d2[DVO_LEVELS]; int *partial[DVO_LEVELS]; unsigned *bitmap[DVO_LEVELS]; int *flags[DVO_LEVELS];
    float4 *tex[DVO_LEVELS]; size_t tex_stride[DVO_LEVELS];
    unsigned *p4[DVO_LEVELS]; size_t p4_stride[DVO_LEVELS]; float2 *pal[DVO_LEVELS]; int *pal_n[DVO_LEVELS];
};
template <int WAVES>
__global__ void __launch_bounds__(WAVES * 64) edt_columns8_levels_kernel(const EdtLevels t) {
    const int l = level_of_block(t.first, t.n, blockIdx.x);
    edt_columns8_body<WAVES>((int)(blockIdx.x - t.first[l]), (int)(t.first[l + 1] - t.first[l]), blockIdx.y, t.edge[l], t.edge_stride[l], t.rows[l], t.cols[l],
                             t.R, t.g[l], t.bitmap[l], t.bm_words[l], t.flags[l]);
}
template <int R>
__global__ void __launch_bounds__(256) edt_rows_pk_levels_kernel(const EdtLevels t) {
    const int l = level_of_block(t.first, t.n, blockIdx.x);
    edt_rows_pk_body<R>((int)(blockIdx.x - t.first[l]), (int)(t.first[l + 1] - t.first[l]), blockIdx.y, t.g[l], t.rows[l], t.cols[l], t.d2[l], t.partial[l],
                        t.bitmap[l], t.bm_words[l], t.flags[l]);
}
template <int BM_WORDS>
__global__ void __launch_bounds__(256) edt_rank_pack_levels_kernel(const EdtLevels t) {
    const int l = level_of_block(t.first, t.n, blockIdx.x);
    edt_rank_pack_body<BM_WORDS>((int)(blockIdx.x - t.first[l]), (int)(t.first[l + 1] - t.first[l]), blockIdx.y, t.d2[l], t.rows[l], t.cols[l], t.R,
                                 t.ptiles_y[l], t.strip[l], t.partial[l], t.n_partial[l], t.bitmap[l], t.bm_words[l], t.flags[l],
                                 t.p4[l], t.p4_stride[l], t.pal[l], t.pal_n[l], t.first_pair, nullptr);
}
__global__ void __launch_bounds__(256) dt_normalize_gradient_pack_levels_kernel(const EdtLevels t, int with_p4) {
    const int l = level_of_block(t.first, t.n, blockIdx.x);
    dt_normalize_gradient_pack_body((int)(blockIdx.x - t.first[l]), (int)(t.first[l + 1] - t.first[l]), blockIdx.y, t.d2[l], t.rows[l], t.cols[l], t.R,
                                    t.ntiles_y[l], t.partial[l], t.n_partial[l], t.tex[l], t.tex_stride[l], with_p4 ? t.pal_n[l] : nullptr, t.flags[l],
                                    t.first_pair, t.ntiles_y[l] * ((t.cols[l] + NP_TX - 1) / NP_TX));
}

#include "dvo_edt_band.h"

__global__ void __launch_bounds__(256)
p4_decode_texels_kernel(const unsigned *__restrict__ p4, size_t p4_stride, const float2 *__restrict__ pal, const int *__restrict__ pal_n,
                        float4 *__restrict__ tex, size_t tex_stride, int rows, int cols, int first_pair) {
    const int pair = first_pair + blockIdx.y;
    if (pal_n[pair] <= 0 || pal_partial(pal_n[pair])) return;
    p4 += (size_t)pair * p4_stride;
    pal += (size_t)pair * DVO_PAL_MAX;
    tex += (size_t)pair * tex_stride;
    const int tpc = p4_tiles_per_col(rows), tpc16 = texel_tiles_per_col(rows);
    const size_t n = (size_t)rows * cols;
    for (size_t p = (size_t)blockIdx.x * blockDim.x + threadIdx.x; p < n; p += (size_t)gridDim.x * blockDim.x) {
        const int xx = (int)(p / rows), yy = (int)(p - (size_t)xx * rows);
        const int ty = yy / DVO_P4_ROWS;
        const size_t slot = p4_slot(ty, yy - ty * DVO_P4_ROWS + 1, xx, tpc);
        const unsigned wu = p4[slot - 1], wc = p4[slot], wd = p4[slot + 1];
        const int c = (int)((wc >> 3) & 0x1fffu);
        const int r = c + (int)(signed char)((wc >> 16) & 0xffu), l = c + (int)(signed char)(wc >> 24);
        const float2 pc = pal[c];
        const float pr = pal[r].x, pl = pal[l].x, pu = pal[(wu >> 3) & 0x1fffu].x, pd = pal[(wd >> 3) & 0x1fffu].x;
        tex[texel_index(yy, xx, tpc16)] = make_float4(pc.x, (pr - pl) * 0.5f, (pd - pu) * 0.5f, pc.y);
    }
}
hipError_t launch_p4_decode_texels(const unsigned *p4, size_t p4_stride, const float2 *pal, const int *pal_n, float4 *tex,
                                   size_t tex_stride, int rows, int cols, int first_pair, int count, hipStream_t s) {
// ... 66 lines not shown
    if (lds > 48 * 1024) {
        const hipError_t e = hipFuncSetAttribute((const void *)kern, hipFuncAttributeMaxDynamicSharedMemorySize, (int)lds);
        if (e != hipSuccess) return e;
    }
    hipLaunchKernelGGL(kern, dim3(nblk, gb.count), dim3(256), lds, s, g, gb.rows, gb.cols, d2, partial, bitmap, bm_words, flags);
    return hipGetLastError();
}

template <int WAVES>
static void edt_columns8_list_launch(const EdtLevels &t, const EdtListShape &ls, const int *list, size_t lds, hipStream_t s) {
    hipLaunchKernelGGL(edt_columns8_list_kernel<WAVES>, dim3(64), dim3(WAVES * 64), lds, s, t, ls, list);
}
template <int R>
static hipError_t edt_rows_pk_list_launch(const EdtLevels &t, const EdtListShape &ls, const int *list, size_t lds, hipStream_t s) {
    auto kern = edt_rows_pk_list_kernel<R>;
    if (lds > 48 * 1024) {
        const hipError_t e = hipFuncSetAttribute((const void *)kern, hipFuncAttributeMaxDynamicSharedMemorySize, (int)lds);
        if (e != hipSuccess) return e;
    }
    hipLaunchKernelGGL(kern, dim3(64), dim3(256), lds, s, t, ls, list);
    return hipGetLastError();
}
template <int T, int THREADS, int NI>
static hipError_t edt_band_kernel_launch(const EdtBandLevels &tb, unsigned g, int count, size_t lds, hipStream_t s) {
    auto kern = edt_band_levels_kernel<T, THREADS, NI>;
    if (lds > 48 * 1024) {
        const hipError_t e = hipFuncSetAttribute((const void *)kern, hipFuncAttributeMaxDynamicSharedMemorySize, (int)lds);
        if (e != hipSuccess) return e;
    }
    hipLaunchKernelGGL(kern, dim3(g, count), dim3(THREADS), lds, s, tb);
    return hipGetLastError();
}
static hipError_t edt_band_run(const EdtLevels &t, const EdtLevelShape &sh, EdtBandLevels &tb, int count, hipStream_t s) {
    const int n = t.n;
    int cmax = 0;
    for (int l = 0; l < n; l++) cmax = t.cols[l] > cmax ? t.cols[l] : cmax;
    int tiles = 0;
    for (int l = 0; l < n; l++) tiles += p4_tiles_per_col(t.rows[l]);
    const int T = edt_band_T_for(count, tiles);
    if (cmax > EB_MAX_COLS || (sh.waves != 8 && sh.waves != 4)) return hipErrorInvalidValue;
    tb.n = n; tb.first_pair = t.first_pair;
    tb.firstA[0] = 0; tb.firstB[0] = 0;
    EdtListShape ls;
    ls.gxmax_cols = 1; ls.gxmax_rows = 1;
    for (int l = 0; l < n; l++) {
        tb.rows[l] = t.rows[l]; tb.cols[l] = t.cols[l];
        tb.nwords[l] = (t.rows[l] + 31) / 32;
        tb.tpc[l] = p4_tiles_per_col(t.rows[l]);
        tb.nbands[l] = (tb.tpc[l] + T - 1) / T;
        tb.n_partial[l] = t.n_partial[l];
        tb.edge[l] = t.edge[l]; tb.edge_stride[l] = t.edge_stride[l];
        tb.flags[l] = t.flags[l]; tb.partial[l] = t.partial[l];
        tb.p4[l] = t.p4[l]; tb.p4_stride[l] = t.p4_stride[l]; tb.pal[l] = t.pal[l]; tb.pal_n[l] = t.pal_n[l];
        tb.firstA[l + 1] = tb.firstA[l] + (unsigned)((t.cols[l] + 31) / 32);
        tb.firstB[l + 1] = tb.firstB[l] + (unsigned)tb.nbands[l];
        const int ngroups = (t.cols[l] + sh.waves - 1) / sh.waves;
        ls.gx_cols[l] = ngroups < 16 ? ngroups : 16;
        ls.gxmax_cols = ls.gx_cols[l] > ls.gxmax_cols ? ls.gx_cols[l] : ls.gxmax_cols;
        ls.gxmax_rows = t.n_partial[l] > ls.gxmax_rows ? t.n_partial[l] : ls.gxmax_rows;
    }
    for (int l = n; l < DVO_LEVELS; l++) ls.gx_cols[l] = 0;
    hipLaunchKernelGGL(edt_colmask_levels_kernel, dim3(tb.firstA[n], count), dim3(512), 0, s, tb);
    hipError_t e;
    const size_t lds = edt_band_lds(cmax, T);
    if (T == 5) e = (cmax <= 640) ? edt_band_kernel_launch<5, 512, 5>(tb, tb.firstB[n], count, lds, s) : edt_band_kernel_launch<5, 512, 8>(tb, tb.firstB[n], count, lds, s);
    else e = (cmax <= 640) ? edt_band_kernel_launch<2, 256, 5>(tb, tb.firstB[n], count, lds, s) : edt_band_kernel_launch<2, 256, 8>(tb, tb.firstB[n], count, lds, s);
    if (e != hipSuccess) return e;
    if (sh.waves == 8) edt_columns8_list_launch<8>(t, ls, tb.list, sh.lds_cols, s);
    else edt_columns8_list_launch<4>(t, ls, tb.list, sh.lds_cols, s);
    switch (sh.R) {
    case 16: e = edt_rows_pk_list_launch<16>(t, ls, tb.list, sh.lds_rows, s); break;
    case 8: e = edt_rows_pk_list_launch<8>(t, ls, tb.list, sh.lds_rows, s); break;
    case 4: e = edt_rows_pk_list_launch<4>(t, ls, tb.list, sh.lds_rows, s); break;
    case 2: e = edt_rows_pk_list_launch<2>(t, ls, tb.list, sh.lds_rows, s); break;
    default: return hipErrorInvalidValue;
    }
    if (e != hipSuccess) return e;
    hipLaunchKernelGGL(edt_palette_levels_kernel, dim3(n, count), dim3(256), 0, s, tb);
    return hipGetLastError();
}

hipError_t launch_edges_to_now(const unsigned char *edge, size_t edge_stride, ImgBatch gb, int *work,
                               float4 *tex_out, size_t tex_stride, unsigned *p4, size_t p4_stride, float2 *pal, int *pal_n,
                               int first_pair, hipStream_t s, bool only_texels) {
    const int R = edt_rows_per_block(gb.cols);
    const unsigned nblk = edt_row_blocks(gb.rows, gb.cols);
    const int bm_words = edt_bitmap_words(gb.rows, gb.cols);
    const size_t ng = edt_g_count(gb.rows, gb.cols, R);
    unsigned short *g = reinterpret_cast<unsigned short *>(work);
    unsigned *d2 = reinterpret_cast<unsigned *>(work) + (((ng * gb.count + 1) / 2 + 3) & ~(size_t)3);
    int *partial = reinterpret_cast<int *>(d2 + ng * gb.count);
    unsigned *bitmap = reinterpret_cast<unsigned *>(partial + (size_t)nblk * gb.count);
    int *flags = reinterpret_cast<int *>(bitmap + (size_t)bm_words * gb.count);
    hipError_t e;
    const bool band = p4 && !only_texels && R >= 2 && edt_band_ok(gb.rows, gb.cols);
    if (band) {
        EdtLevels t{};
        t.n = 1; t.R = R; t.first_pair = first_pair;
        t.rows[0] = gb.rows; t.cols[0] = gb.cols; t.bm_words[0] = bm_words; t.n_partial[0] = (int)nblk;
        t.edge[0] = edge; t.edge_stride[0] = edge_stride;
        t.g[0] = g; t.d2[0] = d2; t.partial[0] = partial; t.bitmap[0] = bitmap; t.flags[0] = flags;
        t.p4[0] = p4; t.p4_stride[0] = p4_stride; t.pal[0] = pal; t.pal_n[0] = pal_n;
        EdtLevelShape sh;
        const size_t lds_wave = 16;
        sh.R = R; sh.waves = (R <= 8) ? 8 : 4; sh.lds_cols = lds_wave * sh.waves; sh.lds_rows = edt_pk_lds_bytes(gb.cols, R);
        EdtBandLevels tb{};
        int *wb = edt_band_carve(flags + gb.count, gb.rows, gb.cols, gb.count, tb, 0);
        tb.list = wb;
        if ((e = edt_band_run(t, sh, tb, gb.count, s)) != hipSuccess) return e;
        if (getenv("DVO_EDT_DEBUG")) {
            (void)hipStreamSynchronize(s);
            unsigned im = 0; int fl = 0, pn = 0, dn = 0, li = 0;
            (void)hipMemcpy(&im, tb.imax[0], 4, hipMemcpyDeviceToHost); (void)hipMemcpy(&fl, tb.flags[0], 4, hipMemcpyDeviceToHost);
            (void)hipMemcpy(&dn, tb.done[0], 4, hipMemcpyDeviceToHost); (void)hipMemcpy(&li, tb.list, 4, hipMemcpyDeviceToHost);
            (void)hipMemcpy(&pn, pal_n + first_pair, 4, hipMemcpyDeviceToHost);
            fprintf(stderr, "[edt band] %dx%d imax %u flags %d done %d list %d pal_n %d nbands %d\n", gb.rows, gb.cols, im, fl, dn, li, pn, tb.nbands[0]);
        }
    }
    if (!only_texels && !band) {
        const size_t lds_wave = (((size_t)((gb.rows + 511) / 512) * 2 * sizeof(int)) + 15) & ~(size_t)15;
        if (R <= 8 && lds_wave * 8 <= 48 * 1024) {
            const int cg = gb.count >= 64 ? 4 : (gb.count >= 16 ? 2 : 1);
            hipLaunchKernelGGL(edt_columns8_kernel<8>, dim3(((gb.cols + 7) / 8 + cg - 1) / cg, gb.count), dim3(512), lds_wave * 8, s, edge, edge_stride,
                               gb.rows, gb.cols, R, g, bitmap, bm_words, flags);
        } else if (lds_wave * 4 <= 48 * 1024) {
            hipLaunchKernelGGL(edt_columns8_kernel<4>, dim3((gb.cols + 3) / 4, gb.count), dim3(256), lds_wave * 4, s, edge, edge_stride,
                               gb.rows, gb.cols, R, g, bitmap, bm_words, flags);
        } else {
            auto kern = edt_columns8_kernel<1>;
            if ((e = hipFuncSetAttribute((const void *)kern, hipFuncAttributeMaxDynamicSharedMemorySize, (int)lds_wave)) != hipSuccess) return e;
            hipLaunchKernelGGL(kern, dim3(gb.cols, gb.count), dim3(64), lds_wave, s, edge, edge_stride, gb.rows, gb.cols, R, g, bitmap,
                               bm_words, flags);
        }
    }
    if (only_texels || band) e = hipSuccess;
    else switch (R) {
    case 16: e = edt_rows_pk_launch<16>(g, gb, nblk, d2, partial, bitmap, bm_words, flags, s); break;
    case 8: e = edt_rows_pk_launch<8>(g, gb, nblk, d2, partial, bitmap, bm_words, flags, s); break;
    case 4: e = edt_rows_pk_launch<4>(g, gb, nblk, d2, partial, bitmap, bm_words, flags, s); break;
    case 2: e = edt_rows_pk_launch<2>(g, gb, nblk, d2, partial, bitmap, bm_words, flags, s); break;
    default:
        e = ((size_t)gb.cols * 4 <= 64 * 1024) ? edt_rows_launch<1, unsigned>(g, gb, nblk, d2, partial, bitmap, bm_words, flags, s)
                                               : edt_rows_launch<1, unsigned short>(g, gb, nblk, d2, partial, bitmap, bm_words, flags, s);
        break;
    }
    if (e != hipSuccess) return e;
    if (p4 && !only_texels && !band) {
        const int ptiles_y = (p4_tiles_per_col(gb.rows) + PK_LR - 1) / PK_LR, ptiles_x = (((gb.cols + 3) >> 2) + PK_LC - 1) / PK_LC;
        long long strip = (long long)gb.count * ptiles_y * ptiles_x / 2048;
        strip = strip < 1 ? 1 : (strip > ptiles_y ? ptiles_y : strip);
        const int n_strips = (ptiles_y + (int)strip - 1) / (int)strip;
        hipLaunchKernelGGL(edt_rank_pack_kernel<PK_SMALL_WORDS>, dim3(n_strips * ptiles_x, gb.count), dim3(256), 0, s, d2, gb.rows, gb.cols, R, ptiles_y,
                           (int)strip, partial, (int)nblk, bitmap, bm_words, flags, p4, p4_stride, pal, pal_n, first_pair, nullptr);
        if (bm_words > PK_SMALL_WORDS)
            hipLaunchKernelGGL(edt_rank_pack_kernel<DVO_EDT_BITMAP_BITS / 32>, dim3(std::min(n_strips * ptiles_x, 8), gb.count), dim3(256), 0, s, d2, gb.rows,
// ... 15 lines not shown
    const size_t lds_wave = (((size_t)((r0 + 511) / 512) * 2 * sizeof(int)) + 15) & ~(size_t)15;
    sh.waves = (sh.R <= 8 && lds_wave * 8 <= 48 * 1024) ? 8 : ((lds_wave * 4 <= 48 * 1024) ? 4 : 0);
    if (!sh.waves) return false;
    sh.lds_cols = lds_wave * sh.waves;
    sh.lds_rows = edt_pk_lds_bytes(c0, sh.R);
    return true;
}
bool edt_levels_ok(int n, const int *rows, const int *cols) { EdtLevelShape sh; return edt_levels_shape(n, rows, cols, sh); }
static size_t edt_level_ints(int rows, int cols, int R, int count) {
    const size_t ng = edt_g_count(rows, cols, R);
    return (((ng * count + 1) / 2 + 3) & ~(size_t)3) + ng * count + ((size_t)((rows + R - 1) / R) + (size_t)edt_bitmap_words(rows, cols) + 1) * count + 8;
}
size_t edt_levels_work_ints(int n, const int *rows, const int *cols, int count) {
    EdtLevelShape sh;
    if (!edt_levels_shape(n, rows, cols, sh)) return 0;
    size_t t = 0;
    for (int l = 0; l < n; l++) t += ((edt_level_ints(rows[l], cols[l], sh.R, count) + 3) & ~(size_t)3) + edt_band_ints(rows[l], cols[l], count);
    return t + 64 + edt_band_list_ints(count);
}
template <int R>
static hipError_t edt_rows_pk_levels_launch(const EdtLevels &t, unsigned g, int count, size_t lds, hipStream_t s) {
    auto kern = edt_rows_pk_levels_kernel<R>;
    if (lds > 48 * 1024) {
        const hipError_t e = hipFuncSetAttribute((const void *)kern, hipFuncAttributeMaxDynamicSharedMemorySize, (int)lds);
        if (e != hipSuccess) return e;
    }
    hipLaunchKernelGGL(kern, dim3(g, count), dim3(256), lds, s, t);
    return hipGetLastError();
}
hipError_t launch_edges_to_now_levels(int n, const int *rows, const int *cols, const unsigned char *const *edge, const size_t *edge_stride, int count,
                                      int *work, float4 *const *tex_out, const size_t *tex_stride, unsigned *const *p4, const size_t *p4_stride,
                                      float2 *const *pal, int *const *pal_n, int first_pair, hipStream_t s, bool only_texels) {
    EdtLevelShape sh;
    if (!edt_levels_shape(n, rows, cols, sh)) return hipErrorInvalidValue;
    EdtLevels t;
    t.n = n; t.R = sh.R; t.first_pair = first_pair;
    const bool with_p4 = p4 && p4[0];
    int *w = work;
    int max_bm = 0;
    for (int l = 0; l < n; l++) {
        const size_t ng = edt_g_count(rows[l], cols[l], sh.R);
        const int nblk = (rows[l] + sh.R - 1) / sh.R;
        t.rows[l] = rows[l]; t.cols[l] = cols[l]; t.bm_words[l] = edt_bitmap_words(rows[l], cols[l]); t.n_partial[l] = nblk;
        max_bm = t.bm_words[l] > max_bm ? t.bm_words[l] : max_bm;
        t.edge[l] = edge[l]; t.edge_stride[l] = edge_stride[l];
        t.g[l] = reinterpret_cast<unsigned short *>(w);
        t.d2[l] = reinterpret_cast<unsigned *>(w) + (((ng * count + 1) / 2 + 3) & ~(size_t)3);
        t.partial[l] = reinterpret_cast<int *>(t.d2[l] + ng * count);
        t.bitmap[l] = reinterpret_cast<unsigned *>(t.partial[l] + (size_t)nblk * count);
        t.flags[l] = reinterpret_cast<int *>(t.bitmap[l] + (size_t)t.bm_words[l] * count);
        w += (edt_level_ints(rows[l], cols[l], sh.R, count) + 3) & ~(size_t)3;
        t.tex[l] = tex_out[l]; t.tex_stride[l] = tex_stride[l];
        t.p4[l] = with_p4 ? p4[l] : nullptr; t.p4_stride[l] = p4_stride[l]; t.pal[l] = pal[l]; t.pal_n[l] = pal_n[l];
        const int pty = (p4_tiles_per_col(rows[l]) + PK_LR - 1) / PK_LR, ptx = (((cols[l] + 3) >> 2) + PK_LC - 1) / PK_LC;
        long long strip = (long long)count * pty * ptx / 2048;
        strip = strip < 1 ? 1 : (strip > pty ? pty : strip);
        t.ptiles_y[l] = pty; t.strip[l] = (int)strip;
        t.ntiles_y[l] = (rows[l] + NP_TY - 1) / NP_TY;
    }
    auto prefix = [&](auto blocks_of) { t.first[0] = 0; for (int l = 0; l < n; l++) t.first[l + 1] = t.first[l] + blocks_of(l); return t.first[n]; };
    hipError_t e = hipSuccess;
    unsigned g = 0;
    bool band = with_p4 && !only_texels;
    for (int l = 0; l < n && band; l++) band = edt_band_ok(rows[l], cols[l]);
    if (band) {
        EdtBandLevels tb{};
        int *wb = w;
        for (int l = 0; l < n; l++) wb = edt_band_carve(wb, rows[l], cols[l], count, tb, l);
        tb.list = wb;
        if ((e = edt_band_run(t, sh, tb, count, s)) != hipSuccess) return e;
    }
    if (!only_texels && !band) {
        const int cg = count >= 64 ? 4 : (count >= 16 ? 2 : 1);
        g = prefix([&](int l) { const int ng = (cols[l] + sh.waves - 1) / sh.waves; return (unsigned)((ng + cg - 1) / cg); });
        if (sh.waves == 8) hipLaunchKernelGGL(edt_columns8_levels_kernel<8>, dim3(g, count), dim3(512), sh.lds_cols, s, t);
        else hipLaunchKernelGGL(edt_columns8_levels_kernel<4>, dim3(g, count), dim3(256), sh.lds_cols, s, t);
        g = prefix([&](int l) { return (unsigned)t.n_partial[l]; });
        switch (sh.R) {
        case 16: e = edt_rows_pk_levels_launch<16>(t, g, count, sh.lds_rows, s); break;
        case 8: e = edt_rows_pk_levels_launch<8>(t, g, count, sh.lds_rows, s); break;
        case 4: e = edt_rows_pk_levels_launch<4>(t, g, count, sh.lds_rows, s); break;
        default: e = edt_rows_pk_levels_launch<2>(t, g, count, sh.lds_rows, s); break;
        }
    }
    if (e != hipSuccess) return e;
    if (with_p4 && !only_texels && !band) {
        g = prefix([&](int l) {
            const int ptx = (((cols[l] + 3) >> 2) + PK_LC - 1) / PK_LC, n_strips = (t.ptiles_y[l] + t.strip[l] - 1) / t.strip[l];
            return (unsigned)(n_strips * ptx);
        });
        hipLaunchKernelGGL(edt_rank_pack_levels_kernel<PK_SMALL_WORDS>, dim3(g, count), dim3(256), 0, s, t);
        if (max_bm > PK_SMALL_WORDS) {
            g = prefix([&](int l) {
                const int ptx = (((cols[l] + 3) >> 2) + PK_LC - 1) / PK_LC, n_strips = (t.ptiles_y[l] + t.strip[l] - 1) / t.strip[l];
                return std::min((unsigned)(n_strips * ptx), 8u);
            });
            hipLaunchKernelGGL(edt_rank_pack_levels_kernel<DVO_EDT_BITMAP_BITS / 32>, dim3(g, count), dim3(256), 0, s, t);
        }
    }
    g = prefix([&](int l) { const unsigned nt = (unsigned)(t.ntiles_y[l] * ((cols[l] + NP_TX - 1) / NP_TX)); return with_p4 ? std::min(nt, 8u) : nt; });
    hipLaunchKernelGGL(dt_normalize_gradient_pack_levels_kernel, dim3(g, count), dim3(256), 0, s, t, with_p4 ? 1 : 0);
    return hipGetLastError();
}

__global__ void __launch_bounds__(256)
float_level_unit_kernel(const float *__restrict__ dt, size_t n, unsigned *__restrict__ unit_bits, int *__restrict__ flags) {
// ... 291 lines not shown
```

rgbd_odometry_amd/csrc/dvo_fused.hip:

```cpp
#include "dvo_kernel_common.h"
#include "dvo_point_pk.h"
#include "dvo_palette.h"
#include "dvo_tiled_step.h"

#include <cstdlib>
#include <type_traits>

#ifndef DVO_WPE256
#define DVO_WPE256 2
#endif
#ifndef DVO_P4_DEPTH
#define DVO_P4_DEPTH(BLOCK) ((BLOCK) == 256 ? 3 : 2)
#endif

namespace dvo {

DVO_DEV unsigned long long stamp_real() {
    unsigned long long t;
    asm volatile("s_memrealtime %0\n\ts_waitcnt lgkmcnt(0)" : "=s"(t) :: "memory");
    return t;
}

template <bool WITH_H, bool WITH_E2 = false>
struct Acc7T {
    static constexpr bool with_h = WITH_H, with_e2 = WITH_E2;
    double g[6];
    double e2;
    int nvis;
    double H[WITH_H ? 21 : 1];
    E2Limbs l;
};
typedef Acc7T<false> Acc7;

template <typename ACC>
DVO_DEV void acc7_zero(ACC &a) {
#pragma unroll
    for (int k = 0; k < 6; k++) a.g[k] = 0.0;
    a.e2 = 0.0;
    a.nvis = 0;
    if constexpr (ACC::with_h) {
#pragma unroll
        for (int k = 0; k < 21; k++) a.H[k] = 0.0;
    }
    if constexpr (ACC::with_e2) e2_limbs_zero(a.l);
}
template <typename ACC>
DVO_DEV void acc_h_add(ACC &a, const double *jwd, const double *Jd) {
#pragma unroll
    for (int i = 0; i < 6; i++)
#pragma unroll
        for (int j = i; j < 6; j++) a.H[i * 6 - (i * (i - 1)) / 2 + (j - i)] = fma(jwd[i], Jd[j], a.H[i * 6 - (i * (i - 1)) / 2 + (j - i)]);
}

enum { TEX_G16 = DVO_TEXMODE_GLOBAL16, TEX_L16 = DVO_TEXMODE_LDS16, TEX_P4 = DVO_TEXMODE_PAL4, TEX_R16 = 3 };

struct TexSrc {
    const char *g16;
    unsigned tile_col_bytes;
    const char *l16;
    const char *p4;
    unsigned p4_col_bytes;
    unsigned r16_org, r16_col_bytes, r16_sent;
};

struct __attribute__((packed, aligned(4))) U3 { unsigned a, b, c; };

template <int TEX> struct Round2 {
    v2f xn, yn, zn;
    v4f t0, t1;
    bool vis0, vis1;
};
template <> struct Round2<TEX_P4> {
    v2f xn, yn, zn;
    U3 t0, t1;
};
template <> struct Round2<TEX_R16> {
    v2f xn, yn, zn;
    unsigned c0, u0, d0, l0, r0, c1, u1, d1, l1, r1;
};
typedef const __attribute__((address_space(3))) unsigned short lds_cushort;

typedef const __attribute__((address_space(3))) float lds_cfloat;
typedef const __attribute__((address_space(3))) v2f lds_cv2f;

DVO_DEV unsigned texel_byte_offset(int yy, int xx, unsigned tile_col_bytes ) {
    static_assert(DVO_TILE_Y_LOG2 == 2 && DVO_TILE_X_LOG2 == 1, "written for 4x2 tiles");
    return __umul24((unsigned)(xx >> 1), tile_col_bytes) + ((unsigned)yy << 5) - (((unsigned)yy & 3u) << 4) + (((unsigned)xx & 1u) << 6);
}

DVO_DEV unsigned p4_byte_offset(int yy, int xx, unsigned p4_col_bytes ) {
    static_assert(DVO_P4_ROWS == 6, "written for 6 interior rows per line");
    const unsigned ty = __umul24((unsigned)yy, 43691u) >> 18;
    return __umul24((unsigned)(xx >> 2), p4_col_bytes) + 128u  + (((unsigned)xx & 3u) << 5) + ((unsigned)yy << 2) + __umul24(ty, 104u);
}

struct LdsPoints {
    const uint2 *p;
    const unsigned *w4;
    const unsigned *g4;
    const unsigned *hdr;
};

template <bool LDS_SRC>
DVO_DEV void load_compact(const LdsPoints &lp, const uint2 *__restrict__ gpts, int j, unsigned &k, float &z) {
    const uint2 a = LDS_SRC ? lp.p[j] : gpts[j];
    k = a.x; z = __uint_as_float(a.y);
}

struct PointPf { uint2 p0, p1; unsigned h0, h1;  };

DVO_DEV unsigned pt4_header(const LdsPoints &lp, int i, int end) {
    const int chunk = __builtin_amdgcn_readfirstlane(min(i, end - 1)) >> 6;
    return lp.hdr[chunk];
}
struct PointPf4 { unsigned w0, w1; };

DVO_DEV uint2 stream_point(const uint2 *__restrict__ p) {
#if defined(DVO_NT_POINTS)
    typedef unsigned nt_u2 __attribute__((ext_vector_type(2)));
    const nt_u2 v = __builtin_nontemporal_load(reinterpret_cast<const nt_u2 *>(p));
    return make_uint2(v.x, v.y);
#else
    return *p;
#endif
}
DVO_DEV unsigned stream_word(const unsigned *__restrict__ p) {
#if defined(DVO_NT_POINTS)
    return __builtin_nontemporal_load(p);
#else
    return *p;
#endif
}
template <bool LDS_SRC, int TEX, bool PT4 = false, bool FULL = false>
DVO_DEV void round2_issue(const IterConst &c, const TexSrc &ts, const LdsPoints &lp, const uint2 *__restrict__ gpts,
                          int i0, int i1, int end, int step, PointPf &pf, Round2<TEX> &b, bool &any_odd, int &nvis) {
    const bool valid0 = FULL || i0 < end, valid1 = FULL || i1 < end;
    v2f xx, yy, Z;
    if constexpr (PT4) {
        unsigned w0, w1;
        if constexpr (LDS_SRC) {
            w0 = lp.w4[valid0 ? i0 : (end - 1)];
            w1 = lp.w4[valid1 ? i1 : (end - 1)];
        } else {
            w0 = pf.p0.x; w1 = pf.p1.x;
            pf.p0.x = stream_word(lp.g4 + min(i0 + step, end - 1));
            pf.p1.x = stream_word(lp.g4 + min(i1 + step, end - 1));
        }
        float x0, y0, z0, x1, y1, z1;
        const unsigned L00 = pf.h0, L01 = pf.h1;
        pf.h0 = pt4_header(lp, i0 + step, end);
        pf.h1 = pt4_header(lp, i1 + step, end);
        pt4_decode(c.nby, c.inv_nby, c.half_inv_nby, w0, L00, x0, y0, z0);
        pt4_decode(c.nby, c.inv_nby, c.half_inv_nby, w1, L01, x1, y1, z1);
        xx.x = x0; xx.y = x1; yy.x = y0; yy.y = y1; Z.x = z0; Z.y = z1;
    } else {
    unsigned k0, k1;
    float z0, z1;
    if constexpr (LDS_SRC) {
        const int j0 = valid0 ? i0 : (end - 1), j1 = valid1 ? i1 : (end - 1);
        load_compact<true>(lp, gpts, j0, k0, z0);
        load_compact<true>(lp, gpts, j1, k1, z1);
    } else {
        k0 = pf.p0.x; z0 = __uint_as_float(pf.p0.y);
        k1 = pf.p1.x; z1 = __uint_as_float(pf.p1.y);
        pf.p0 = stream_point(gpts + min(i0 + step, end - 1));
        pf.p1 = stream_point(gpts + min(i1 + step, end - 1));
    }
    xx.x = (float)(k0 & 0xffffu); xx.y = (float)(k1 & 0xffffu);
    yy.x = (float)(k0 >> 16);     yy.y = (float)(k1 >> 16);
    Z.x = z0; Z.y = z1;
    }
    const v2f X = (Z * (xx - c.pcx)) * c.pfx;
    const v2f Y = (Z * (yy - c.pcy)) * c.pfy;
    v2f xn, yn, zn, u, v;
#ifndef DVO_NO_VALU_DIET
    if constexpr (TEX == TEX_P4 || TEX == TEX_R16) {
        lanemask odd;
        project_point2m(c, X, Y, Z, xn, yn, zn, u, v, odd);
        any_odd |= (odd != 0ull);
        int px0, py0, px1, py1;
        const lanemask in0 = pixel_in_range_mask(u.x, c.cols, px0) & pixel_in_range_mask(v.x, c.rows, py0);
        const lanemask in1 = pixel_in_range_mask(u.y, c.cols, px1) & pixel_in_range_mask(v.y, c.rows, py1);
        const lanemask vis0 = FULL ? in0 : (in0 & mask_lt_i32(i0, end)), vis1 = FULL ? in1 : (in1 & mask_lt_i32(i1, end));
        b.xn = xn; b.yn = yn; b.zn = zn;
        nvis += __popcll(vis0) + __popcll(vis1);
        if constexpr (TEX == TEX_R16) {
            const unsigned a0 = select_or(vis0, ts.r16_org + __umul24((unsigned)px0 + 1u, ts.r16_col_bytes) + ((unsigned)py0 << 1), ts.r16_sent);
            const unsigned a1 = select_or(vis1, ts.r16_org + __umul24((unsigned)px1 + 1u, ts.r16_col_bytes) + ((unsigned)py1 << 1), ts.r16_sent);
            b.u0 = *(lds_cushort *)(size_t)(a0);     b.c0 = *(lds_cushort *)(size_t)(a0 + 2u); b.d0 = *(lds_cushort *)(size_t)(a0 + 4u);
            b.l0 = *(lds_cushort *)(size_t)(a0 + 2u - ts.r16_col_bytes); b.r0 = *(lds_cushort *)(size_t)(a0 + 2u + ts.r16_col_bytes);
            b.u1 = *(lds_cushort *)(size_t)(a1);     b.c1 = *(lds_cushort *)(size_t)(a1 + 2u); b.d1 = *(lds_cushort *)(size_t)(a1 + 4u);
            b.l1 = *(lds_cushort *)(size_t)(a1 + 2u - ts.r16_col_bytes); b.r1 = *(lds_cushort *)(size_t)(a1 + 2u + ts.r16_col_bytes);
        } else {
            const unsigned o0 = select_or_zero(vis0, p4_byte_offset(py0, px0, ts.p4_col_bytes));
            const unsigned o1 = select_or_zero(vis1, p4_byte_offset(py1, px1, ts.p4_col_bytes));
            b.t0 = *reinterpret_cast<const U3 *>(ts.p4 + o0);
            b.t1 = *reinterpret_cast<const U3 *>(ts.p4 + o1);
        }
        return;
    }
#endif
    bool odd0, odd1;
    project_point2(c, X, Y, Z, xn, yn, zn, u, v, odd0, odd1);
    any_odd |= (__builtin_amdgcn_ballot_w64(odd0 || odd1) != 0ull);
    int px0, py0, px1, py1;
    const bool inx0 = pixel_in_range(u.x, c.cols, px0), iny0 = pixel_in_range(v.x, c.rows, py0);
    const bool inx1 = pixel_in_range(u.y, c.cols, px1), iny1 = pixel_in_range(v.y, c.rows, py1);
    const bool vis0 = inx0 && iny0 && valid0;
    const bool vis1 = inx1 && iny1 && valid1;
    b.xn = xn; b.yn = yn; b.zn = zn;
    if constexpr (TEX == TEX_R16) {
        nvis += __popcll(__builtin_amdgcn_ballot_w64(vis0)) + __popcll(__builtin_amdgcn_ballot_w64(vis1));
        unsigned a0 = ts.r16_org + __umul24((unsigned)px0 + 1u, ts.r16_col_bytes) + ((unsigned)py0 << 1);
        unsigned a1 = ts.r16_org + __umul24((unsigned)px1 + 1u, ts.r16_col_bytes) + ((unsigned)py1 << 1);
        a0 = vis0 ? a0 : ts.r16_sent;
        a1 = vis1 ? a1 : ts.r16_sent;
        b.u0 = *(lds_cushort *)(size_t)(a0);     b.c0 = *(lds_cushort *)(size_t)(a0 + 2u); b.d0 = *(lds_cushort *)(size_t)(a0 + 4u);
        b.l0 = *(lds_cushort *)(size_t)(a0 + 2u - ts.r16_col_bytes); b.r0 = *(lds_cushort *)(size_t)(a0 + 2u + ts.r16_col_bytes);
        b.u1 = *(lds_cushort *)(size_t)(a1);     b.c1 = *(lds_cushort *)(size_t)(a1 + 2u); b.d1 = *(lds_cushort *)(size_t)(a1 + 4u);
        b.l1 = *(lds_cushort *)(size_t)(a1 + 2u - ts.r16_col_bytes); b.r1 = *(lds_cushort *)(size_t)(a1 + 2u + ts.r16_col_bytes);
    } else if constexpr (TEX == TEX_P4) {
        nvis += __popcll(__builtin_amdgcn_ballot_w64(vis0)) + __popcll(__builtin_amdgcn_ballot_w64(vis1));
        unsigned o0 = p4_byte_offset(py0, px0, ts.p4_col_bytes);
        unsigned o1 = p4_byte_offset(py1, px1, ts.p4_col_bytes);
        o0 = vis0 ? o0 : 0u;
        o1 = vis1 ? o1 : 0u;
        b.t0 = *reinterpret_cast<const U3 *>(ts.p4 + o0);
        b.t1 = *reinterpret_cast<const U3 *>(ts.p4 + o1);
    } else {
        b.vis0 = vis0; b.vis1 = vis1;
        unsigned o0 = texel_byte_offset(py0, px0, ts.tile_col_bytes);
        unsigned o1 = texel_byte_offset(py1, px1, ts.tile_col_bytes);
        o0 = vis0 ? o0 : 0u;
        o1 = vis1 ? o1 : 0u;
        const char *base = (TEX == TEX_L16) ? ts.l16 : ts.g16;
        b.t0 = *reinterpret_cast<const v4f *>(base + o0);
        b.t1 = *reinterpret_cast<const v4f *>(base + o1);
    }
}

DVO_DEV unsigned lshl3_add(int d, unsigned c) {
    unsigned r;
    asm("v_lshl_add_u32 %0, %1, 3, %2" : "=v"(r) : "v"(d), "v"(c));
    return r;
}
template <unsigned PAL>
DVO_DEV void p4_decode2(const U3 &t0, const U3 &t1, v2f &dt, v2f &gx, v2f &gy, v2f &w) {
    const unsigned c0 = t0.b & 0xfff8u, c1 = t1.b & 0xfff8u;
    const v2f pw0 = *(lds_cv2f *)(size_t)(PAL + c0);
    const v2f pw1 = *(lds_cv2f *)(size_t)(PAL + c1);
    v2f pu, pd, pr, pl;
    pu.x = *(lds_cfloat *)(size_t)(PAL + (t0.a & 0xfff8u));
    pu.y = *(lds_cfloat *)(size_t)(PAL + (t1.a & 0xfff8u));
    pd.x = *(lds_cfloat *)(size_t)(PAL + (t0.c & 0xfff8u));
    pd.y = *(lds_cfloat *)(size_t)(PAL + (t1.c & 0xfff8u));
    pr.x = *(lds_cfloat *)(size_t)(PAL + lshl3_add(__builtin_amdgcn_sbfe((int)t0.b, 16, 8), c0));
    pr.y = *(lds_cfloat *)(size_t)(PAL + lshl3_add(__builtin_amdgcn_sbfe((int)t1.b, 16, 8), c1));
    pl.x = *(lds_cfloat *)(size_t)(PAL + lshl3_add(((int)t0.b) >> 24, c0));
    pl.y = *(lds_cfloat *)(size_t)(PAL + lshl3_add(((int)t1.b) >> 24, c1));
    dt.x = pw0.x; dt.y = pw1.x; w.x = pw0.y; w.y = pw1.y;
    gx = (pr - pl) * 0.5f;
    gy = (pd - pu) * 0.5f;
}

template <typename ACC>
DVO_DEV void acc7_add(ACC &a, const float *jw, const float *J, float eps) {
    const double e = (double)eps;
    double jwd[6];
#pragma unroll
    for (int k = 0; k < 6; k++) { jwd[k] = (double)jw[k]; a.g[k] = fma(jwd[k], e, a.g[k]); }
    a.e2 = fma(e, e, a.e2);
    if constexpr (ACC::with_e2) e2_limbs_add(a.l, eps);
    if constexpr (ACC::with_h) {
        double Jd[6];
#pragma unroll
        for (int k = 0; k < 6; k++) Jd[k] = (double)J[k];
        acc_h_add(a, jwd, Jd);
    }
}

DVO_DEV void iter_const_pose(IterConst &c, const float *Rf, const float *tf) {
    c.r[0] = uniform_f(Rf[0]); c.r[1] = uniform_f(Rf[1]); c.r[2] = uniform_f(Rf[2]);
    c.r[3] = uniform_f(Rf[3]); c.r[4] = uniform_f(Rf[4]); c.r[5] = uniform_f(Rf[5]);
    c.r[6] = uniform_f(Rf[6]); c.r[7] = uniform_f(Rf[7]); c.r[8] = uniform_f(Rf[8]);
    c.t[0] = uniform_f(tf[0]); c.t[1] = uniform_f(tf[1]); c.t[2] = uniform_f(tf[2]);
}

struct AccE2 {
    static constexpr bool with_h = false;
    E2Limbs l;
    int nvis;
};
DVO_DEV void acc7_add(AccE2 &a, const float *, const float *, float eps) { e2_limbs_add(a.l, eps); }

template <int TEX, unsigned PAL, typename ACC>
DVO_DEV void round2_compute(const IterConst &c, const Round2<TEX> &b, ACC &a) {
    v2f jw[6], J[6];
    float eps0, eps1;
    if constexpr (TEX == TEX_R16) {
        const v2f pw0 = *(lds_cv2f *)(size_t)(PAL + b.c0), pw1 = *(lds_cv2f *)(size_t)(PAL + b.c1);
        v2f pu, pd, pr, pl, dt, wt;
        pu.x = *(lds_cfloat *)(size_t)(PAL + b.u0); pu.y = *(lds_cfloat *)(size_t)(PAL + b.u1);
        pd.x = *(lds_cfloat *)(size_t)(PAL + b.d0); pd.y = *(lds_cfloat *)(size_t)(PAL + b.d1);
        pr.x = *(lds_cfloat *)(size_t)(PAL + b.r0); pr.y = *(lds_cfloat *)(size_t)(PAL + b.r1);
        pl.x = *(lds_cfloat *)(size_t)(PAL + b.l0); pl.y = *(lds_cfloat *)(size_t)(PAL + b.l1);
        dt.x = pw0.x; dt.y = pw1.x; wt.x = pw0.y; wt.y = pw1.y;
        const v2f gx = (pr - pl) * 0.5f, gy = (pd - pu) * 0.5f;
        eps0 = dt.x; eps1 = dt.y;
        jacobian_weighted2p(c, b.xn, b.yn, b.zn, gx, gy, wt, jw, ACC::with_h ? J : nullptr);
    } else if constexpr (TEX == TEX_P4) {
        v2f dt, gx, gy, wt;
        p4_decode2<PAL>(b.t0, b.t1, dt, gx, gy, wt);
        eps0 = dt.x; eps1 = dt.y;
        jacobian_weighted2p(c, b.xn, b.yn, b.zn, gx, gy, wt, jw, ACC::with_h ? J : nullptr);
    } else {
        a.nvis += __popcll(__builtin_amdgcn_ballot_w64(b.vis0)) + __popcll(__builtin_amdgcn_ballot_w64(b.vis1));
        eps0 = b.vis0 ? b.t0.x : 0.0f; eps1 = b.vis1 ? b.t1.x : 0.0f;
        const float w0 = b.vis0 ? b.t0.w : 0.0f, w1 = b.vis1 ? b.t1.w : 0.0f;
        const float gx0 = b.vis0 ? b.t0.y : 0.0f, gx1 = b.vis1 ? b.t1.y : 0.0f;
        const float gy0 = b.vis0 ? b.t0.z : 0.0f, gy1 = b.vis1 ? b.t1.z : 0.0f;
        jacobian_weighted2(c, b.xn, b.yn, b.zn, gx0, gx1, gy0, gy1, w0, w1, jw, ACC::with_h ? J : nullptr);
    }
    const double e0 = (double)eps0, e1 = (double)eps1;
    if constexpr (ACC::with_e2) { e2_limbs_add(a.l, eps0); e2_limbs_add(a.l, eps1); }
    if constexpr (!ACC::with_h) {
#pragma unroll
        for (int k = 0; k < 6; k++) {
            a.g[k] = fma((double)jw[k].x, e0, a.g[k]);
            a.g[k] = fma((double)jw[k].y, e1, a.g[k]);
        }
        a.e2 = fma(e0, e0, a.e2);
        a.e2 = fma(e1, e1, a.e2);
    } else {
        {
            double jd[6], Jd[6];
#pragma unroll
            for (int k = 0; k < 6; k++) { jd[k] = (double)jw[k].x; Jd[k] = (double)J[k].x; a.g[k] = fma(jd[k], e0, a.g[k]); }
            a.e2 = fma(e0, e0, a.e2);
            acc_h_add(a, jd, Jd);
        }
        __builtin_amdgcn_sched_barrier(0);
        {
            double jd[6], Jd[6];
#pragma unroll
            for (int k = 0; k < 6; k++) { jd[k] = (double)jw[k].y; Jd[k] = (double)J[k].y; a.g[k] = fma(jd[k], e1, a.g[k]); }
            a.e2 = fma(e1, e1, a.e2);
            acc_h_add(a, jd, Jd);
        }
        __builtin_amdgcn_sched_barrier(0);
    }
}

template <int BLOCK, bool LDS_SRC, int TEX, int DEPTH = 2, unsigned PAL = 0, bool PT4 = false, typename ACC = Acc7>
DVO_DEV void accumulate_points2(const IterConst &c, const TexSrc &ts, const LdsPoints &lp, const uint2 *__restrict__ gpts,
                                int first, int end, int lane_off, ACC &a, bool &any_odd) {
    if (first >= end) return;
    constexpr int STEP = 2 * BLOCK;
    const int wave_off = __builtin_amdgcn_readfirstlane(lane_off - (int)(threadIdx.x & 63));
// ... 455 lines not shown
    __syncthreads();

    for (int l = sc.n_levels - 1; l >= 0; --l) {
        const int iters = sc.iters[l];
        if (iters <= 0) continue;
        const LevelSlab &L = lv.l[l];
        const int dpair = (sc.alias_mod > 0) ? (pair % sc.alias_mod) : pair;
        const int Nall = __builtin_amdgcn_readfirstlane(L.N[dpair]);
        int pfirst = 0, N = Nall;
        const bool solo = TEAM && Nall <= sc.team_solo_max;
        const bool works = !solo || member == 0;
        if (TEAM && !solo) {
            const int chunk = (((Nall + G - 1) / G) + 1) & ~1;
            pfirst = min(Nall, member * chunk);
            N = min(Nall, pfirst + chunk) - pfirst;
        }
        if (!works) N = 0;
        const int iters_run = works ? iters : 0;
        const char *__restrict__ tex = reinterpret_cast<const char *>(L.tex + (size_t)dpair * L.tex_stride);
        const uint2 *__restrict__ gpts = L.cpts + (size_t)dpair * L.pt_cap + pfirst;
        float *energy = out.energy + (size_t)pair * sc.e_stride + sc.e_off[l];

        IterConst c;
        level_consts(c, K, l, L.rows, L.cols);
        DVO_STAMP(ts0);

        if (member == 0)
            for (int i = tid; i < iters; i += BLOCK) energy[i] = 0.0f;
        if (tid == 0) { pose_state_begin(st); pose_regulariser_precompute(st, st.p[0], uc); }

        const int lds_words = sc.lds_bytes >> 2;
        const int n_pad = (N + 3) & ~3;
        const int tex16_words = (int)(L.tex_stride * 4);
        const int pal_n_raw = (!sc.no_p4 && L.pal_n) ? __builtin_amdgcn_readfirstlane(L.pal_n[dpair]) : 0;
        const int n_pal = pal_count(pal_n_raw);
        const bool p4_partial = pal_partial(pal_n_raw);
        const int mode = (n_pal > 0 && pal_base_ok && 2 * n_pal + 8 <= lds_words) ? TEX_P4
                         : ((!TEAM && !sc.no_lds_tex && 2 * n_pad + tex16_words <= lds_words) ? TEX_L16 : TEX_G16);
        const int n_pal_lds = n_pal + (p4_partial ? 2 : 1);
        const int pal_words = (mode == TEX_P4) ? ((2 * n_pal_lds + 3) & ~3) : 0;
        const int r16_col = L.rows + 2;
        const int r16_elems = r16_col * (L.cols + 2) + 2 * r16_col + 4;
        const int r16_words = ((r16_elems + 1) / 2 + 3) & ~3;
#ifdef DVO_ENABLE_R16
        constexpr bool kR16 = !WITH_H;
#else
        constexpr bool kR16 = false;
#endif
        const bool r16 = kR16 && !TEAM && mode == TEX_P4 && !sc.no_r16 && !((sc.flags & 1) && l == sc.last_level) &&
                         pal_words + r16_words + 8 * BLOCK <= lds_words;
        const int img_words = r16 ? r16_words : 0;
        const bool pt4 = !TEAM && mode == TEX_P4 && !r16 && !sc.no_pt4 && N >= sc.pt4_factor * (((lds_words - pal_words - img_words) >> 1) & ~1) && L.pt4_ok &&
                         __builtin_amdgcn_readfirstlane(L.pt4_ok[dpair]) != 0;
        float *const lds_pts = lds_dyn + pal_words + img_words;
        const int cap = (mode == TEX_L16) ? n_pad
                        : (pt4 ? ((lds_words - pal_words - img_words) & ~1) : (((lds_words - pal_words - img_words) >> 1) & ~1));
        const int n_lds = (N <= cap) ? N : (cap / (2 * BLOCK)) * (2 * BLOCK);
        float *const lds_tex = lds_pts + 2 * cap;
        if (tid == 0) { st.exact_ran = 0; st.e2_open = 0; st.e2_ran = 0; }
        if (mode == TEX_P4 && works) {
            const float2 *__restrict__ pg = L.pal + (size_t)dpair * DVO_PAL_MAX;
            float2 *pl = reinterpret_cast<float2 *>(lds_dyn);
            for (int i = tid; i < n_pal_lds; i += BLOCK) pl[i] = pg[i];
        }
        const unsigned *__restrict__ g4pts = L.cpt4 + (size_t)dpair * L.pt_cap + pfirst;
        if (pt4) {
            const uint4 *g4 = reinterpret_cast<const uint4 *>(g4pts);
            uint4 *d4 = reinterpret_cast<uint4 *>(lds_pts);
            const int n4 = n_lds >> 2;
            int i = tid;
            for (; i + 3 * BLOCK < n4; i += 4 * BLOCK) {
                uint4 v[4];
#pragma unroll
                for (int q = 0; q < 4; q++) v[q] = g4[i + q * BLOCK];
#pragma unroll
                for (int q = 0; q < 4; q++) d4[i + q * BLOCK] = v[q];
            }
            for (; i < n4; i += BLOCK) d4[i] = g4[i];
            for (int j = (n4 << 2) + tid; j < n_lds; j += BLOCK) reinterpret_cast<unsigned *>(lds_pts)[j] = g4pts[j];
        } else {
            const uint4 *g4 = reinterpret_cast<const uint4 *>(gpts);
            uint4 *d4 = reinterpret_cast<uint4 *>(lds_pts);
            const int n2 = n_lds >> 1;
            int i = tid;
            for (; i + 3 * BLOCK < n2; i += 4 * BLOCK) {
                uint4 v[4];
#pragma unroll
                for (int q = 0; q < 4; q++) v[q] = g4[i + q * BLOCK];
#pragma unroll
                for (int q = 0; q < 4; q++) d4[i + q * BLOCK] = v[q];
            }
            for (; i < n2; i += BLOCK) d4[i] = g4[i];
            if ((n_lds & 1) && tid == 0) reinterpret_cast<uint2 *>(lds_pts)[n_lds - 1] = gpts[n_lds - 1];
        }
        if (mode == TEX_L16) {
            const v4f *g = reinterpret_cast<const v4f *>(tex);
            v4f *d = reinterpret_cast<v4f *>(lds_tex);
            const int n16 = (int)L.tex_stride;
            int i = tid;
            for (; i + 3 * BLOCK < n16; i += 4 * BLOCK) {
                v4f v[4];
#pragma unroll
                for (int q = 0; q < 4; q++) v[q] = g[i + q * BLOCK];
#pragma unroll
                for (int q = 0; q < 4; q++) d[i + q * BLOCK] = v[q];
            }
            for (; i < n16; i += BLOCK) d[i] = g[i];
        }
        LdsPoints lp;
        lp.p = reinterpret_cast<const uint2 *>(lds_pts);
        lp.w4 = reinterpret_cast<const unsigned *>(lds_pts);
        lp.g4 = g4pts;
        lp.hdr = L.chdr + (size_t)dpair * (L.pt_cap >> 6);
        TexSrc ts;
        ts.g16 = tex; ts.tile_col_bytes = (unsigned)c.tiles_per_col * 128u;
        ts.l16 = reinterpret_cast<const char *>(lds_tex);
        ts.p4 = reinterpret_cast<const char *>(L.p4 + (size_t)dpair * L.p4_stride);
        ts.p4_col_bytes = (unsigned)p4_tiles_per_col(L.rows) * 128u;
        ts.r16_org = kStatic + 4u * (unsigned)pal_words;
        ts.r16_col_bytes = 2u * (unsigned)r16_col;
        ts.r16_sent = ts.r16_org + 2u * (unsigned)(r16_col * (L.cols + 2) + r16_col);
        if (r16) {
            unsigned short *img = reinterpret_cast<unsigned short *>(lds_dyn + pal_words);
            const int wv = tid >> 6, ln = tid & 63;
            for (int xc = wv; xc < L.cols + 2; xc += BLOCK / 64) {
                int xx = xc - 1;
                xx = xx < 0 ? -xx : (xx >= L.cols ? 2 * L.cols - 2 - xx : xx);
                for (int yc = ln; yc < r16_col; yc += 64) {
                    int yy = yc - 1;
                    yy = yy < 0 ? -yy : (yy >= L.rows ? 2 * L.rows - 2 - yy : yy);
                    const unsigned w = *reinterpret_cast<const unsigned *>(ts.p4 + p4_byte_offset(yy, xx, ts.p4_col_bytes) + 4u);
                    img[xc * r16_col + yc] = (unsigned short)(w & 0xfff8u);
                }
            }
            for (int i = tid; i < 2 * r16_col + 4; i += BLOCK) img[r16_col * (L.cols + 2) + i] = (unsigned short)(n_pal << 3);
        }
        __syncthreads();
        DVO_STAMP(ts1);
        DVO_STAMP_ADD(5, ts0, ts1);

        const bool exch = TEAM && !solo;
        for (int itr = 0; itr < iters_run; ++itr) {
#ifndef DVO_NO_PROGRESS_PRIO
            if (!TEAM) {
                if (l > 0) __builtin_amdgcn_s_setprio(3);
                else if (2 * itr < iters) __builtin_amdgcn_s_setprio(2);
                else if (4 * itr < 3 * iters) __builtin_amdgcn_s_setprio(1);
                else __builtin_amdgcn_s_setprio(0);
            }
#endif
            const PoseCur &pc = st.p[itr & 1];
            PoseCur &pn = st.p[(itr + 1) & 1];
            iter_const_pose(c, pc.Rf, pc.tf);

            DVO_STAMP(t0);
            Acc7T<WITH_H> a;
            acc7_zero(a);
            bool any_odd = false;
            const int lane_off = BLOCK - 64 - (tid & ~63) + (tid & 63);
            if (mode == TEX_L16) {
                accumulate_points2<BLOCK, true, TEX_L16, 2, 0, false, Acc7T<WITH_H>>(c, ts, lp, gpts, 0, N, lane_off, a, any_odd);
            } else if (r16) {
                accumulate_points2<BLOCK, true, TEX_R16, 2, kStatic, false, Acc7T<WITH_H>>(c, ts, lp, gpts, 0, n_lds, lane_off, a, any_odd);
                accumulate_points2<BLOCK, false, TEX_R16, 2, kStatic, false, Acc7T<WITH_H>>(c, ts, lp, gpts, n_lds, N, lane_off, a, any_odd);
            } else if (mode == TEX_P4 && pt4) {
                accumulate_points2<BLOCK, true, TEX_P4, (WITH_H ? 2 : DVO_P4_DEPTH(BLOCK)), kStatic, true, Acc7T<WITH_H>>(c, ts, lp, gpts, 0, n_lds, lane_off, a, any_odd);
                accumulate_points2<BLOCK, false, TEX_P4, (WITH_H ? 2 : DVO_P4_DEPTH(BLOCK)), kStatic, true, Acc7T<WITH_H>>(c, ts, lp, gpts, n_lds, N, lane_off, a, any_odd);
            } else if (mode == TEX_P4) {
                accumulate_points2<BLOCK, true, TEX_P4, (WITH_H ? 2 : DVO_P4_DEPTH(BLOCK)), kStatic, false, Acc7T<WITH_H>>(c, ts, lp, gpts, 0, n_lds, lane_off, a, any_odd);
                accumulate_points2<BLOCK, false, TEX_P4, (WITH_H ? 2 : DVO_P4_DEPTH(BLOCK)), kStatic, false, Acc7T<WITH_H>>(c, ts, lp, gpts, n_lds, N, lane_off, a, any_odd);
            } else {
                accumulate_points2<BLOCK, true, TEX_G16, 2, 0, false, Acc7T<WITH_H>>(c, ts, lp, gpts, 0, n_lds, lane_off, a, any_odd);
                accumulate_points2<BLOCK, false, TEX_G16, 2, 0, false, Acc7T<WITH_H>>(c, ts, lp, gpts, n_lds, N, lane_off, a, any_odd);
            }
            {
                const double chk = ((a.g[0] + a.g[1]) + (a.g[2] + a.g[3])) + ((a.g[4] + a.g[5]) + a.e2);
                any_odd |= (__builtin_amdgcn_ballot_w64(!__builtin_isfinite(chk)) != 0ull);
            }
            if (any_odd || sc.force_exact) {
                acc7_zero(a);
                sweep_literal<BLOCK>(mode, p4_partial, pt4, c, tex, ts, reinterpret_cast<const float2 *>(lds_dyn), lp, gpts, n_lds, N, lane_off, a);
                if ((tid & 63) == 0) st.exact_ran = 1;
            }
            DVO_STAMP(t1);
            DVO_STAMP_T2_DECL();
            wave_sums7(a, red);
            if constexpr (WITH_H) {
#pragma unroll
                for (int q = 0; q < 3; q++) {
                    double d[8];
#pragma unroll
                    for (int k = 0; k < 8; k++) d[k] = (8 * q + k < 21) ? a.H[8 * q + k] : 0.0;
                    wave_reduce_scatter8_dpp(d);
                    const int idx = reduce_scatter8_dpp_index(tid & 63);
                    if ((tid & 63) < 8) redH[tid >> 6][8 * q + idx] = d[0];
                }
            }
            const int wave = __builtin_amdgcn_readfirstlane(tid >> 6), lane = tid & 63;
            double neg_step = 0.0;
            if (wave == 0) neg_step = pose_neg_step(uc, itr);
            __syncthreads();
            double sl = 0.0;
            if (wave == 0) {
                sl = block_sum8<BLOCK>(red, lane & 7);
                DVO_STAMP_T2();
                if (exch) {
                    sl = team_total(sl);
                    if (lane == 6 || lane == 7) tot[lane] = sl;
                }
            }
            if (exch) __syncthreads();
            if (wave == 0) {
                double psi[6];
                pose_direction_lanes(st, uc, neg_step, sl, lane, psi);
                if (lane == 0) pose_apply(st, pc, pn, uc, psi);
            } else if (WITH_H && wave == 2) {
                if (lane < 21) {
// ... 28 lines not shown
                __syncthreads();
                if (wave == 0) {
                    double sl2 = block_sum8<BLOCK>(red, lane & 7);
                    if (exch) sl2 = team_total(sl2);
                    if (lane < 3) tot[lane] = sl2;
                }
                if (exch) epoch++;
                __syncthreads();
                if (wave == 1 && lane == 0) {
                    const float e = (float)sqrt(e2_from_limbs(tot[0], tot[1], tot[2], st.e2_fast));
                    pose_bookkeep_e(st, pc, itr, Nall, e, st.e2_nvis);
                    if (member == 0) energy[itr] = e;
                    st.e2_open = 0;
                    st.e2_ran++;
                }
                __syncthreads();
            }
            DVO_STAMP_ADD(0, t0, t1); DVO_STAMP_ADD(1, t1, t2); DVO_STAMP_ADD(2, t2, t3); DVO_STAMP_ADD(3, t3, t4);
            DVO_STAMP_ADD(4, t0, t0 + 1);
            if (st.stop) break;
            if (tid == 0 && itr + 1 < iters_run) pose_regulariser_precompute(st, pn, uc);
        }

        if ((sc.flags & 1) && l == sc.last_level) {
            if (st.bestItr >= 0) {
                iter_const_pose(c, st.bRf, st.btf);
                float *fe = out.final_eps + (size_t)pair * out.final_cap;
                float *fr = out.final_reproj + (size_t)pair * out.final_cap * 3;
                float *fes = fe + pfirst, *frs = fr + 3 * (size_t)pfirst;
#ifndef DVO_NO_FINAL
                if (mode == TEX_P4 && pt4) {
                    final_outputs2<BLOCK, true, TEX_P4, kStatic, true>(c, ts, lp, gpts, 0, n_lds, fes, frs, p4_partial);
                    final_outputs2<BLOCK, false, TEX_P4, kStatic, true>(c, ts, lp, gpts, n_lds, N, fes, frs, p4_partial);
                } else if (mode == TEX_P4) {
                    final_outputs2<BLOCK, true, TEX_P4, kStatic>(c, ts, lp, gpts, 0, n_lds, fes, frs, p4_partial);
                    final_outputs2<BLOCK, false, TEX_P4, kStatic>(c, ts, lp, gpts, n_lds, N, fes, frs, p4_partial);
                } else if (mode == TEX_L16) {
                    final_outputs2<BLOCK, true, TEX_L16, kStatic>(c, ts, lp, gpts, 0, N, fes, frs);
                } else {
                    final_outputs2<BLOCK, true, TEX_G16, kStatic>(c, ts, lp, gpts, 0, n_lds, fes, frs);
                    final_outputs2<BLOCK, false, TEX_G16, kStatic>(c, ts, lp, gpts, n_lds, N, fes, frs);
                }
#endif
            }
            if (tid == 0 && member == 0) out.final_N[pair] = (st.bestItr >= 0) ? Nall : 0;
        }
        __syncthreads();
        if (tid == 0) {
            pose_state_finish(st);
            if (member == 0) {
                out.best_idx[pair * DVO_LEVELS + l] = st.bestItr;
                out.ratio[pair * DVO_LEVELS + l] = st.bestRatio;
                out.tex_mode[pair * DVO_LEVELS + l] = mode | (st.exact_ran ? DVO_TEXMODE_EXACT_RAN : 0) | (pt4 ? DVO_TEXMODE_PT4 : 0) | (r16 ? DVO_TEXMODE_RANKS_LDS : 0) |
                                                       (min(st.e2_ran, DVO_TEXMODE_E2_MAX) << DVO_TEXMODE_E2_SHIFT);
            }
        }
        __syncthreads();
        if (TEAM && solo) {
            if (tid < 64) {
                const int k = tid & 7;
                double mine = -0.0;
                if (member == 0 && k < 7) mine = (k < 4) ? st.p[0].q[k] : st.p[0].t[k - 4];
                const double v = team_total(mine);
                if (tid < 4) st.p[0].q[tid] = v;
                else if (tid < 7) st.p[0].t[tid - 4] = v;
            }
            epoch++;
            __syncthreads();
            if (tid == 0) {
                double q[4], R[9];
#pragma unroll
                for (int k = 0; k < 4; k++) q[k] = st.p[0].q[k];
                quat_to_matrix(q, R);
#pragma unroll
                for (int k = 0; k < 9; k++) st.R[k] = R[k];
            }
            __syncthreads();
        }
    }

#ifdef DVO_STAMPS
    if (tid == 0 && out.dbg) out.dbg[(size_t)pair * 64 + 63] = stamp_real();
#endif
    if (tid == 0 && member == 0) {
        double *p = out.poses + (size_t)pair * 12;
#pragma unroll
        for (int k = 0; k < 9; k++) p[k] = st.R[k];
#pragma unroll
        for (int k = 0; k < 3; k++) p[9 + k] = st.p[0].t[k];
    }
}

template <int BLOCK>
static hipError_t launch_fused2_b(const LevelSet &lv, const Schedule &sc, const Intrinsics &K, const DevParams &prm,
                                  const Outputs &out, int first_pair, int n_pairs, hipStream_t s) {
    const size_t dyn = (size_t)sc.lds_bytes;
    hipError_t e;
    if constexpr (BLOCK == 512) {
        if (sc.flags & 4) {
            if (sc.team > 1 || !out.H) return hipErrorInvalidValue;
            auto kern = align_fused2_kernel<512, false, true>;
            if ((e = hipFuncSetAttribute((const void *)kern, hipFuncAttributeMaxDynamicSharedMemorySize, (int)dyn)) != hipSuccess) return e;
            hipLaunchKernelGGL(kern, dim3(n_pairs), dim3(512), dyn, s, lv, sc, K, prm, out, first_pair);
            return hipGetLastError();
        }
    } else if constexpr (BLOCK == 256) {
        if (sc.flags & 4) {
// ... 226 lines not shown
```

rgbd_odometry_amd/csrc/dvo_kernels.hip:

```cpp
#include "dvo_kernel_common.h"
#include "dvo_palette.h"
#include "dvo_tiled_step.h"

namespace dvo {

struct PointSrc {
    const float *__restrict__ g;
    const uint2 *__restrict__ gc;
    const float *l;
    int n_lds, cap;
};
enum { SRC_GLOBAL_XYZ = 0, SRC_LDS_XYZ = 1, SRC_GLOBAL_COMPACT = 2, SRC_LDS_COMPACT = 3 };
template <int SRC>
DVO_DEV void load_point(const IterConst &c, const PointSrc &p, int i, float &X, float &Y, float &Z) {
    if (SRC == SRC_LDS_XYZ) {
        X = p.l[i]; Y = p.l[p.cap + i]; Z = p.l[2 * p.cap + i];
    } else if (SRC == SRC_GLOBAL_XYZ) {
        X = p.g[3 * i]; Y = p.g[3 * i + 1]; Z = p.g[3 * i + 2];
    } else if (SRC == SRC_LDS_COMPACT) {
        expand_compact(c, __float_as_uint(p.l[i]), p.l[p.cap + i], X, Y, Z);
    } else {
        const uint2 v = p.gc[i];
        expand_compact(c, v.x, __uint_as_float(v.y), X, Y, Z);
    }
// ... 138 lines not shown
}

__global__ void __launch_bounds__(256)
points4_build_kernel(const uint2 *__restrict__ cpts, const int *__restrict__ N, int pt_cap, int rows, unsigned *__restrict__ cpt4,
                     unsigned *__restrict__ chdr, int *__restrict__ pt4_ok, int first_pair) {
    const int pair = first_pair + blockIdx.x;
    const int n = N[pair];
    cpts += (size_t)pair * pt_cap; cpt4 += (size_t)pair * pt_cap; chdr += (size_t)pair * (pt_cap / 64);
    const unsigned nby = (unsigned)((rows + 15) >> 4);
    const float inv_nby = 1.0f / (float)nby, half_inv = 0.5f * inv_nby;
    bool bad = false;
    for (int i = threadIdx.x; i < n; i += 256) {
        const uint2 p = cpts[i], p0 = cpts[i & ~63];
        const unsigned xx = p.x & 0xffffu, yy = p.x >> 16;
        const unsigned L = (xx >> 4) * nby + (yy >> 4), L0 = ((p0.x & 0xffffu) >> 4) * nby + ((p0.x >> 16) >> 4);
        const float Z = __uint_as_float(p.y);
        const float dmm = rintf(Z * 1000.0f);
        const bool enc = (L >= L0) && (L - L0 <= 255u) && (L < (1u << 20)) && (dmm >= 0.0f) && (dmm <= 65535.0f);
        const unsigned w = enc ? ((xx & 15u) | ((yy & 15u) << 4) | ((unsigned)dmm << 8) | ((L - L0) << 24)) : 0u;
        float xf, yf, zf;
        pt4_decode(nby, inv_nby, half_inv, w, L0, xf, yf, zf);
        if (!enc || xf != (float)xx || yf != (float)yy || __float_as_uint(zf) != p.y) bad = true;
        cpt4[i] = w;
        if ((i & 63) == 0) chdr[i >> 6] = L0;
    }
    const int any_bad = __syncthreads_or(bad ? 1 : 0);
    if (threadIdx.x == 0) pt4_ok[pair] = (n > 0 && !any_bad) ? 1 : 0;
}
hipError_t launch_points4_build(const uint2 *cpts, const int *N, int pt_cap, int rows, unsigned *cpt4, unsigned *chdr, int *pt4_ok,
                                int first_pair, int count, hipStream_t s) {
    if (count <= 0) return hipSuccess;
    hipLaunchKernelGGL(points4_build_kernel, dim3(count), dim3(256), 0, s, cpts, N, pt_cap, rows, cpt4, chdr, pt4_ok, first_pair);
    return hipGetLastError();
}

__global__ void __launch_bounds__(256)
final_permute_kernel(const unsigned *__restrict__ cidx, const float *__restrict__ fe_blk, const float *__restrict__ fr_blk, int n,
                     float *__restrict__ fe, float *__restrict__ fr) {
    for (int i = blockIdx.x * blockDim.x + threadIdx.x; i < n; i += gridDim.x * blockDim.x) {
        const unsigned j = cidx[i];
        if (j >= (unsigned)n) continue;
        fe[j] = fe_blk[i];
        fr[3 * (size_t)j] = fr_blk[3 * (size_t)i]; fr[3 * (size_t)j + 1] = fr_blk[3 * (size_t)i + 1]; fr[3 * (size_t)j + 2] = fr_blk[3 * (size_t)i + 2];
    }
}
hipError_t launch_final_permute(const unsigned *cidx, const float *fe_blk, const float *fr_blk, int n, float *fe, float *fr, hipStream_t s) {
    if (n <= 0) return hipSuccess;
    int blocks = (n + 255) / 256; if (blocks > 1024) blocks = 1024;
    hipLaunchKernelGGL(final_permute_kernel, dim3(blocks), dim3(256), 0, s, cidx, fe_blk, fr_blk, n, fe, fr);
    return hipGetLastError();
}

__global__ void __launch_bounds__(256)
replicate_compact_kernel(unsigned *p4, size_t p4_stride, float2 *pal, int *pal_n, int n_src, int dst_first) {
    const int p = dst_first + blockIdx.y;
    const int src = blockIdx.y % n_src;
    if (p == src) return;
    const int pn = pal_n[src];
    if (blockIdx.x == 0 && threadIdx.x == 0) pal_n[p] = pn;
    const int n = pal_count(pn);
    if (n <= 0) return;
    const size_t stride = (size_t)gridDim.x * blockDim.x;
    const uint4 *s4 = reinterpret_cast<const uint4 *>(p4 + (size_t)src * p4_stride);
    uint4 *d4 = reinterpret_cast<uint4 *>(p4 + (size_t)p * p4_stride);
    for (size_t i = (size_t)blockIdx.x * blockDim.x + threadIdx.x; i < p4_stride / 4; i += stride) d4[i] = s4[i];
    const float2 *sp = pal + (size_t)src * DVO_PAL_MAX;
    float2 *dp = pal + (size_t)p * DVO_PAL_MAX;
    const size_t n_copy = (size_t)n + (pal_partial(pn) ? 2 : 1);
    for (size_t i = (size_t)blockIdx.x * blockDim.x + threadIdx.x; i < n_copy; i += stride) dp[i] = sp[i];
}
hipError_t launch_replicate_compact(unsigned *p4, size_t p4_stride, float2 *pal, int *pal_n, int n_src, int dst_first,
                                    int dst_count, hipStream_t s) {
    if (dst_count <= 0) return hipSuccess;
    hipLaunchKernelGGL(replicate_compact_kernel, dim3(32, dst_count), dim3(256), 0, s, p4, p4_stride, pal, pal_n, n_src, dst_first);
    return hipGetLastError();
}

#ifdef DVO_STAMPS
DVO_DEV unsigned long long stamp_now() {
    unsigned long long t;
    __builtin_amdgcn_sched_barrier(0);
    asm volatile("s_memtime %0\n\ts_waitcnt lgkmcnt(0)" : "=s"(t) :: "memory");
    __builtin_amdgcn_sched_barrier(0);
    return t;
}
#define DVO_STAMP(var) const unsigned long long var = stamp_now()
#define DVO_STAMP_ADD(slot, a, b) do { if (tid == 0 && out.dbg) out.dbg[(size_t)pair * 64 + l * 8 + (slot)] += (b) - (a); } while (0)
#else
#define DVO_STAMP(var) do {} while (0)
#define DVO_STAMP_ADD(slot, a, b) do {} while (0)
#endif
#ifndef DVO_WAVES_PER_EU
#define DVO_WAVES_PER_EU 1
#endif
template <int BLOCK, int U, int INTERP, bool CP, bool WITH_H = false>
__global__ void __launch_bounds__(BLOCK) __attribute__((amdgpu_waves_per_eu(DVO_WAVES_PER_EU, 8)))
align_fused_kernel(LevelSet lv, Schedule sc, Intrinsics K, DevParams prm, Outputs out, int first_pair) {
    const int pair = first_pair + blockIdx.x;
    const int tid = threadIdx.x;
    __shared__ PoseState st;
    __shared__ double red[BLOCK / 64][DVO_NACC_PAD];
    __shared__ double tot[DVO_NACC_PAD];
    extern __shared__ float lds_points[];

    if (tid == 0) {
        const double *p = out.poses + (size_t)pair * 12;
        const bool ident = (sc.flags & 2) != 0;
        double R0[9], t0[3];
#pragma unroll
        for (int k = 0; k < 9; k++) R0[k] = ident ? ((k % 4 == 0) ? 1.0 : 0.0) : p[k];
#pragma unroll
        for (int k = 0; k < 3; k++) t0[k] = ident ? 0.0 : p[9 + k];
        pose_state_load(st, R0, t0);
        upd_const_build(st.u, prm);
    }
    __syncthreads();

    for (int l = sc.n_levels - 1; l >= 0; --l) {
        const int iters = sc.iters[l];
        if (iters <= 0) continue;
        const LevelSlab &L = lv.l[l];
        const int dpair = (sc.alias_mod > 0) ? (pair % sc.alias_mod) : pair;
        const int N = L.N[dpair];
        const float4 *__restrict__ tex = L.tex + (size_t)dpair * L.tex_stride;
        const float *__restrict__ pts = L.pts + (size_t)dpair * L.pt_cap * 3;
        float *energy = out.energy + (size_t)pair * sc.e_stride + sc.e_off[l];

// ... 578 lines not shown
```

rgbd_odometry_amd/csrc/dvo_launch.h:

```cpp
#ifndef DVO_LAUNCH_H_
#define DVO_LAUNCH_H_

#include <hip/hip_runtime.h>
#include <stddef.h>
#include <stdint.h>

#include "dvo_device_math.h"

#define DVO_LEVELS 8
#define DVO_NACC 29
#define DVO_NACC_PAD 32
enum { DVO_TEXMODE_GLOBAL16 = 0, DVO_TEXMODE_LDS16 = 1, DVO_TEXMODE_PAL4 = 2,
       DVO_TEXMODE_EXACT_RAN = 0x100 ,
       DVO_TEXMODE_PT4 = 0x200       ,
       DVO_TEXMODE_E2_SHIFT = 12, DVO_TEXMODE_E2_MAX = 0xffff ,
       DVO_TEXMODE_RANKS_LDS = 0x400  };

namespace dvo {

struct LevelSlab {
    const float4 *tex;
    const float *pts;
    const uint2 *cpts;
    const unsigned *cidx;
    const unsigned *cpt4;
    const unsigned *chdr;
    const int *pt4_ok;
    const int *N;
    size_t tex_stride;
    int pt_cap;
    int rows, cols;
    const unsigned *p4;
    const float2 *pal;
    const int *pal_n;
    size_t p4_stride;
};
struct LevelSet { LevelSlab l[DVO_LEVELS]; };

struct Schedule {
    int n_levels;
    int iters[DVO_LEVELS];
    int e_off[DVO_LEVELS];
    int e_stride;
    int last_level;
    int flags;
    int alias_mod;
    int lds_points;
    int lds_bytes;
    int no_lds_tex;
    int no_p4;
    int team;
    int n_pairs_launch;
    int force_e2;
    int force_exact;
    int compact;
    int no_pt4;
    int pt4_factor;
    int final_blk;
    int team_no_plain;
    int no_r16;
    unsigned team_epoch0;
    int team_solo_max;
};

#define DVO_TILED_SOLO_MAX_DEFAULT 6144
#define DVO_TEAM_SOLO_MAX_DEFAULT 0

struct Intrinsics { float fx, fy, cx, cy; int interp;  };

struct Outputs {
    double *poses;
    float *energy;
    int *best_idx;
    float *ratio;
    float *final_eps;
    float *final_reproj;
    int *final_N;
    int final_cap;
    unsigned long long *dbg;
    double *H;
    double *team_buf;
    unsigned *team_cnt;
    int *team_err;
    int *tex_mode;
    const int *order;
};

hipError_t launch_pack_texels(const float *dt, const float *gx, const float *gy, float4 *out,
                              int rows, int cols, hipStream_t s);
size_t palette_work_ints(int count);
hipError_t launch_palette_build(const float4 *tex, size_t tex_stride, int rows, int cols, unsigned *p4, size_t p4_stride,
                                float2 *pal, int *pal_n, int first_pair, int count, unsigned *work, hipStream_t s);
bool fused_uses_compact(int points_in_flight, int interp);
hipError_t launch_replicate_level(float4 *tex, const unsigned char *src_has_tex , size_t tex_stride, float *pts,
                                  uint2 *cpts, unsigned *cidx, unsigned *cpt4, unsigned *chdr, int *pt4_ok, int pt_cap, int *N, int n_src, int dst_first,
                                  int dst_count, hipStream_t s);
hipError_t launch_points_recover_compact(const float *xyz, int N, int level, const Intrinsics &K, uint2 *compact, unsigned *cidx, int *fail, hipStream_t s);
hipError_t launch_points4_build(const uint2 *cpts, const int *N, int pt_cap, int rows, unsigned *cpt4, unsigned *chdr, int *pt4_ok,
                                int first_pair, int count, hipStream_t s);
hipError_t launch_final_permute(const unsigned *cidx, const float *fe_blk, const float *fr_blk, int n, float *fe, float *fr, hipStream_t s);
hipError_t launch_replicate_compact(unsigned *p4, size_t p4_stride, float2 *pal, int *pal_n, int n_src, int dst_first,
                                    int dst_count, hipStream_t s);
hipError_t launch_align_fused(int block_threads, int points_in_flight, const LevelSet &lv,
                              const Schedule &sc, const Intrinsics &K, const DevParams &prm,
                              const Outputs &out, int first_pair, int n_pairs, hipStream_t s);
hipError_t launch_align_fused2(int block_threads, const LevelSet &lv, const Schedule &sc, const Intrinsics &K,
                               const DevParams &prm, const Outputs &out, int first_pair, int n_pairs, hipStream_t s);
size_t fused2_static_lds(int block_threads, bool with_h = false);
hipError_t launch_eval_points(const LevelSlab &L, int pair, int level, const Intrinsics &K,
                              const float *Rf, const float *tf,
                              float *reproj, float *J, float *eps, float *w, int *vis, hipStream_t s);
hipError_t launch_accumulate(const LevelSlab &L, int pair, int level, const Intrinsics &K,
                             const float *Rf, const float *tf, int first_point, int n_points,
                             double *partials, int nblocks, double *acc, hipStream_t s);
int accumulate_blocks_for(int n_points);
size_t pose_state_bytes();
hipError_t launch_iter_begin(void *state, const DevParams &prm, const double *Rt12, float *energy, int max_iters, hipStream_t s);
hipError_t launch_iter_accumulate(const LevelSlab &L, int pair, int level, const Intrinsics &K, const void *state,
                                  int first_point, int n_points, double *partials, int nblocks, double *acc,
                                  hipStream_t s);
hipError_t launch_iter_update(void *state, const DevParams &prm, int itr, int n_total, const double *acc,
                              float *energy, hipStream_t s);
hipError_t launch_iter_step_fused(const LevelSlab &L, int pair, int level, const Intrinsics &K, void *state,
                                  const DevParams &prm, int itr, int n_points, double *partials, int nblocks,
                                  float *energy, hipStream_t s);
hipError_t launch_iter_end(void *state, double *Rt12, int *best_idx, float *ratio, hipStream_t s);
int tiled_step_blocks(int n_points, int n_cu);
hipError_t launch_tiled_step(const LevelSlab &L, int pair, int level, const Intrinsics &K, const DevParams &prm, const void *st_in,
                             void *st_out, const double *acc_in, int itr, int apply_prev, int n_total, int first_point, int n_points,
                             double *partials, unsigned *ticket, double *acc_out, float *energy, int nblocks,
                             double *H_prev , hipStream_t s);
hipError_t launch_tiled_step_pk(const LevelSlab &L, int pair, int level, const Intrinsics &K, const void *st_in, void *st_out,
                                const double *acc_in, int itr, int apply_prev, int n_total, int first_point, int n_points,
                                double *partials, unsigned *ticket, double *acc_out, float *energy, int nblocks, double *H_prev, hipStream_t s);
hipError_t launch_tiled_level_solo(const LevelSlab &L, int pair, int level, const Intrinsics &K, const void *st_in, void *st_out, int iters,
                                   int n_points, float *energy, double *Rt12, int *best_idx, float *ratio, float *next_energy,
                                   int next_iters, hipStream_t s);
hipError_t launch_tiled_finish(const void *st_in, void *st_out, const DevParams &prm, const double *acc_in, int itr_last, int n_total,
                               float *energy, double *Rt12, int *best_idx, float *ratio, double *H_last, float *next_energy, int next_iters,
                               hipStream_t s);
hipError_t launch_final_outputs_state(const LevelSlab &L, int pair, int level, const Intrinsics &K, const void *state,
                                      int first_point, int n_points, float *final_eps, float *final_reproj, int *final_N,
                                      hipStream_t s);
hipError_t launch_unpack_texels(const float4 *tex, int rows, int cols, float *dt, float *gx, float *gy, hipStream_t s);
hipError_t launch_keep_warm(int us, hipStream_t s);
hipError_t launch_se3_exp(const double *psi, double *Rt12, hipStream_t s);
hipError_t launch_se3_log(const double *Rt12, double *psi, hipStream_t s);
hipError_t launch_rotationize(double *R9, hipStream_t s);

struct ImgBatch { int rows, cols, count; };

hipError_t launch_import_grey(const void *src, int dtype, int row_major, size_t src_stride,
                              unsigned char *grey, size_t stride, ImgBatch g, hipStream_t s);
hipError_t launch_import_depth(const void *src, int dtype, int row_major, size_t src_stride,
                               float *depth_mm, size_t stride, ImgBatch g, hipStream_t s);
struct SrcTab { const void *const *bgr; const void *const *depth; };
hipError_t launch_gather_images(const void *const *src, int count, void *dst, size_t bytes, size_t stride, hipStream_t s, int max_wgs_per_image = 64);
hipError_t launch_camera_level(const unsigned char *bgr, size_t bgr_stride, const float *depth_m, size_t depth_stride,
                               int src_rows, int src_cols, int shift, const short2 *umap_xy, const unsigned short *umap_frac,
                               int depth_raw, unsigned char *grey, float *depth_mm, size_t stride, ImgBatch g, hipStream_t s, SrcTab tab = {nullptr, nullptr});
hipError_t launch_camera_levels(const unsigned char *bgr, size_t bgr_stride, const float *depth_m, size_t depth_stride, int src_rows, int src_cols,
                                int n, const int *shift, const int *rows, const int *cols, const short2 *umap_xy, const unsigned short *umap_frac,
                                int depth_raw, unsigned char *const *grey, float *const *depth_mm, const size_t *stride, int count, hipStream_t s,
                                SrcTab tab = {nullptr, nullptr});
bool camera_levels_decimate_ok(int n_levels, const int *rows, const int *cols);
hipError_t launch_camera_decimate_levels(const unsigned char *grey0, const float *depth0, size_t stride0, int rows0, int cols0, int n,
                                         const int *rows, const int *cols, unsigned char *const *grey, float *const *depth, const size_t *stride,
                                         int count, hipStream_t s);
size_t canny_work_ints(int rows, int cols, int count);
size_t canny_levels_work_ints(int n, const int *rows, const int *cols, int count);
bool canny_levels_ok(int n, const int *rows, const int *cols, unsigned char *const *edge, const size_t *edge_stride);
hipError_t launch_canny_levels(int n, const int *rows, const int *cols, const unsigned char *const *grey, const size_t *grey_stride,
                               unsigned char *const *edge, const size_t *edge_stride, int count, int low, int high, int *work, hipStream_t s);
hipError_t launch_canny(const unsigned char *grey, size_t stride, ImgBatch g, int low, int high, int *work,
                        unsigned char *edge, size_t edge_stride, hipStream_t s);
hipError_t launch_count_edges(const unsigned char *edge, size_t n, int *out, hipStream_t s);
bool edt_levels_ok(int n, const int *rows, const int *cols);
size_t edt_levels_work_ints(int n, const int *rows, const int *cols, int count);
hipError_t launch_edges_to_now_levels(int n, const int *rows, const int *cols, const unsigned char *const *edge, const size_t *edge_stride, int count,
                                      int *work, float4 *const *tex_out, const size_t *tex_stride, unsigned *const *p4, const size_t *p4_stride,
                                      float2 *const *pal, int *const *pal_n, int first_pair, hipStream_t s,
                                      bool only_texels = false );
size_t float_level_work_ints(int rows, int cols);
hipError_t launch_float_level_to_compact(const float *dt, const float *gx, const float *gy, int rows, int cols, int *work,
                                         unsigned *p4, size_t p4_stride, float2 *pal, int *pal_n, int pair, hipStream_t s);
size_t edt_work_ints(int rows, int cols, int count);
hipError_t launch_edges_to_now(const unsigned char *edge, size_t edge_stride, ImgBatch g, int *work,
                               float4 *tex_out, size_t tex_stride, unsigned *p4, size_t p4_stride, float2 *pal, int *pal_n,
                               int first_pair, hipStream_t s, bool only_texels = false);
hipError_t launch_p4_decode_texels(const unsigned *p4, size_t p4_stride, const float2 *pal, const int *pal_n, float4 *tex,
                                   size_t tex_stride, int rows, int cols, int first_pair, int count, hipStream_t s);
size_t enlist_block_ints(int rows, int cols);
hipError_t launch_enlist_count(const void *edge, int edge_is_u8, size_t edge_stride, const float *depth_mm,
                               size_t depth_stride, ImgBatch g, int *col_counts, int *blk_counts, hipStream_t s);
hipError_t launch_enlist_write(const void *edge, int edge_is_u8, size_t edge_stride, const float *depth_mm,
                               size_t depth_stride, ImgBatch g, int level, const Intrinsics &K, const int *col_counts,
                               const int *blk_counts, float *xyz, size_t xyz_stride,
                               uint2 *compact , unsigned *cidx ,
                               float *uv, int capacity, int *N_dst, hipStream_t s);

hipError_t launch_photo_reference(const unsigned char *grey, const float *depth, int rows, int cols, int level,
                                  double fx, double fy, double cx, double cy, int fixed, double grad_threshold, int capacity,
                                  int *col_work , double *J, int *sel, double *zref, float *gref, double *A36,
                                  int *n_out, hipStream_t s);
hipError_t launch_photo_gauss_newton(const double *J, const int *sel, const double *zref, const float *gref, const int *n_dev,
                                     const double *A36, const unsigned char *grey_now, int rows, int cols, int level,
                                     double fx, double fy, double cx, double cy, int fixed, int max_iters, double eps_stop,
                                     double *T16, double *eps_norms, int *updates, double *eps_dump, hipStream_t s);

}
#endif
```

rgbd_odometry_amd/csrc/dvo_palette.h:

```cpp
#ifndef DVO_PALETTE_H_
#define DVO_PALETTE_H_

#include <hip/hip_runtime.h>
#include <stddef.h>

#define DVO_PAL_MAX 8192
#define DVO_PAL_BUILD_MAX 4096
#define DVO_PAL_PARTIAL (1 << 20)
#define DVO_PAL_CAP_PARTIAL 4094
#define DVO_P4_ROWS 6
#define DVO_EDT_BITMAP_BITS (1 << 18)

namespace dvo {

enum { PAL_BAD_VALUE = 1, PAL_TOO_MANY = 2, PAL_STEP = 3, PAL_GRADIENT = 4, PAL_WEIGHT = 5, PAL_SHAPE = 6, PAL_FAR = 7 };

__host__ __device__ inline int pal_count(int pal_n) { return pal_n > 0 ? (pal_n & (DVO_PAL_PARTIAL - 1)) : 0; }
__host__ __device__ inline bool pal_partial(int pal_n) { return pal_n > 0 && (pal_n & DVO_PAL_PARTIAL) != 0; }
__host__ __device__ inline int p4_tiles_per_col(int rows) { return (rows + DVO_P4_ROWS - 1) / DVO_P4_ROWS; }
__host__ __device__ inline size_t p4_count(int rows, int cols) {
    return (size_t)p4_tiles_per_col(rows) * (size_t)((cols + 3) >> 2) * 32u + 32u;
}
__host__ __device__ inline size_t p4_slot(int ty, int srow, int xx, int tiles_per_col) {
    return 32u + ((size_t)(xx >> 2) * tiles_per_col + ty) * 32u + (size_t)((xx & 3) * 8 + srow);
}

}
#endif
```

Before: 799,200.

## Add dense 16-bit haloed tile layout for distance-field lookups on fine levels

Adds a dense slab of 16-bit distance values arranged in 6x6 tiles with a one-pixel halo, stored as 8x8 lines. The EDT kernel writes it on the two finest pyramid levels, and the fused align kernel gains a TEX_D16 path that gathers the centre, up and down values with one 8-byte load plus two scalar loads. This replaces palette decoding and is meant to cut gather instructions and indirection in the inner accumulation loop. The slab is allocated only when ample device memory is free, costs extra memory and EDT write bandwidth, and has to be replicated across pairs.

```diff
diff --git a/include/dvo_amd.h b/include/dvo_amd.h
--- a/include/dvo_amd.h
+++ b/include/dvo_amd.h
@@ -138,6 +138,7 @@
 int  dvo_get_level_energy_sweeps(dvo_ctx *ctx, int pair, int level, int *n);
 int  dvo_get_level_points4(dvo_ctx *ctx, int pair, int level, int *used);
 int  dvo_get_level_ranks_in_lds(dvo_ctx *ctx, int pair, int level, int *used);
+int  dvo_get_level_dense_lines(dvo_ctx *ctx, int pair, int level, int *used);
 
 int  dvo_get_last_launch_shape(dvo_ctx *ctx, int *block_threads, int *team_size, int *packed);
 
diff --git a/rgbd_odometry_amd/capi.py b/rgbd_odometry_amd/capi.py
--- a/rgbd_odometry_amd/capi.py
+++ b/rgbd_odometry_amd/capi.py
@@ -24,7 +24,7 @@
     "dvo_set_poses", "dvo_align_batch_enqueue", "dvo_get_poses", "dvo_get_level_report",
     "dvo_get_final_outputs", "dvo_get_level_normal_matrix", "dvo_eval_points", "dvo_accumulate", "dvo_device_se3_exp",
     "dvo_device_se3_log", "dvo_device_rotationize", "dvo_algorithmic_bytes", "dvo_point_iterations",
-    "dvo_debug_stamps", "dvo_get_level_texel_mode", "dvo_get_level_exact_fallback", "dvo_get_level_energy_sweeps", "dvo_get_level_points4", "dvo_get_level_ranks_in_lds", "dvo_now_prepare", "dvo_set_direct_compact", "dvo_host_alloc_mapped", "dvo_host_free_mapped", "dvo_get_now_compact_info", "dvo_get_now_compact_partial", "dvo_get_last_launch_shape", "dvo_replicate_pairs", "dvo_set_now_level_from_edges", "dvo_get_now_level", "dvo_iter_begin", "dvo_iter_accumulate", "dvo_iter_update", "dvo_iter_end",
+    "dvo_debug_stamps", "dvo_get_level_texel_mode", "dvo_get_level_exact_fallback", "dvo_get_level_energy_sweeps", "dvo_get_level_points4", "dvo_get_level_ranks_in_lds", "dvo_get_level_dense_lines", "dvo_now_prepare", "dvo_set_direct_compact", "dvo_host_alloc_mapped", "dvo_host_free_mapped", "dvo_get_now_compact_info", "dvo_get_now_compact_partial", "dvo_get_last_launch_shape", "dvo_replicate_pairs", "dvo_set_now_level_from_edges", "dvo_get_now_level", "dvo_iter_begin", "dvo_iter_accumulate", "dvo_iter_update", "dvo_iter_end",
     "dvo_align_pyramid_wide", "dvo_tiled_attach", "dvo_tiled_detach", "dvo_align_pyramid_tiled", "dvo_tiled_shard", "dvo_tiled_graph_replayed", "dvo_wide_packed_levels", "dvo_wide_team_levels",
     "dvo_get_ref_level", "dvo_frames_reserve", "dvo_frames_upload_pyramids", "dvo_frames_upload_cameras", "dvo_frames_set_undistort",
     "dvo_photo_params_default", "dvo_photo_configure", "dvo_photo_set_ref", "dvo_photo_align", "dvo_photo_get_jacobian", "dvo_frames_as_now",
@@ -226,6 +226,7 @@
         "dvo_get_level_energy_sweeps": [vp, i, i, ip],
         "dvo_get_level_points4": [vp, i, i, ip],
         "dvo_get_level_ranks_in_lds": [vp, i, i, ip],
+        "dvo_get_level_dense_lines": [vp, i, i, ip],
         "dvo_now_prepare": [vp, i, i],
         "dvo_get_last_launch_shape": [vp, ip, ip, ip],
         "dvo_get_now_compact_info": [vp, i, i, ip],
@@ -749,6 +750,11 @@
         self._chk(self.lib.dvo_get_level_ranks_in_lds(self._h, pair, level, C.byref(m)))
         return bool(m.value)
 
+    def level_dense_lines(self, pair: int, level: int) -> bool:
+        m = C.c_int(0)
+        self._chk(self.lib.dvo_get_level_dense_lines(self._h, pair, level, C.byref(m)))
+        return bool(m.value)
+
     def last_launch_shape(self):
         b, t, k = C.c_int(0), C.c_int(0), C.c_int(0)
         self._chk(self.lib.dvo_get_last_launch_shape(self._h, C.byref(b), C.byref(t), C.byref(k)))
diff --git a/rgbd_odometry_amd/csrc/dvo_capi.cpp b/rgbd_odometry_amd/csrc/dvo_capi.cpp
--- a/rgbd_odometry_amd/csrc/dvo_capi.cpp
+++ b/rgbd_odometry_amd/csrc/dvo_capi.cpp
@@ -215,6 +215,8 @@
         free_texels(c, L);
         std::fill(L.have_now.begin(), L.have_now.end(), 0);
         if (L.p4) { (void)hipFree(L.p4); (void)hipFree(L.pal); (void)hipFree(L.d_pal_n); L.p4 = nullptr; L.pal = nullptr; L.d_pal_n = nullptr; }
+        if (L.d16) { (void)hipFree(L.d16); L.d16 = nullptr; }
+        L.d16_failed = false;
         L.pal_built.clear(); L.now_uses.clear(); L.tex16_stale.clear(); L.p4_known.clear(); L.p4_fresh.clear(); L.p4_native.clear();
     }
 
@@ -264,6 +266,18 @@
 static bool p4_addressable(int rows, int cols) {
     return !(p4_count(rows, cols) * sizeof(unsigned) >= ((size_t)1 << 32) || rows >= (1 << 16) || ((cols + 3) >> 2) >= (1 << 24) ||
              (size_t)p4_tiles_per_col(rows) * 128 >= ((size_t)1 << 24));
+}
+
+static void try_dense_slab(dvo_ctx *c, int level) {
+    Level &L = c->lv[level];
+    if (level >= DVO_D16_LEVELS || L.d16 || L.d16_failed || !L.p4) return;
+    const size_t stride = d16_count(L.rows, L.cols), bytes = sizeof(unsigned short) * stride * (size_t)c->n_pairs;
+    const size_t compact_bytes = (sizeof(unsigned) * L.p4_stride + sizeof(float2) * DVO_PAL_MAX) * (size_t)c->n_pairs;
+    size_t free_b = 0, total_b = 0;
+    if (hipMemGetInfo(&free_b, &total_b) != hipSuccess) { (void)hipGetLastError(); L.d16_failed = true; return; }
+    if (free_b < bytes + compact_bytes / 2 + ((size_t)16 << 30)) { L.d16_failed = true; return; }
+    if (hipMalloc((void **)&L.d16, bytes) != hipSuccess) { (void)hipGetLastError(); L.d16 = nullptr; L.d16_failed = true; return; }
+    L.d16_stride = stride;
 }
 
 int ensure_compact_slabs(dvo_ctx *c, int level) {
@@ -362,6 +376,7 @@
     s.cpt4 = L.cpt4; s.chdr = L.chdr; s.pt4_ok = L.d_pt4_ok;
     s.tex_stride = L.tex_stride; s.pt_cap = L.pt_cap; s.rows = L.rows; s.cols = L.cols;
     s.p4 = L.p4; s.pal = L.pal; s.pal_n = L.d_pal_n; s.p4_stride = L.p4_stride;
+    s.d16 = L.d16; s.d16_stride = L.d16_stride;
     return s;
 }
 
@@ -604,6 +619,8 @@
         sc.team_no_plain = no_plain ? 1 : 0;
         static const bool no_r16 = [] { const char *e = std::getenv("DVO_RANKS_LDS"); return e && std::strcmp(e, "off") == 0; }();
         sc.no_r16 = no_r16 ? 1 : 0;
+        static const bool no_d16 = [] { const char *e = std::getenv("DVO_DENSE_LINES"); return e && std::strcmp(e, "off") == 0; }();
+        sc.no_d16 = no_d16 ? 1 : 0;
         static const int solo_max = [] { const char *e = std::getenv("DVO_TEAM_SOLO_MAX"); return e ? std::atoi(e) : DVO_TEAM_SOLO_MAX_DEFAULT; }();
         sc.team_solo_max = solo_max;
     }
@@ -846,6 +863,7 @@
         if (c->lv[l].d_pt4_ok) (void)hipFree(c->lv[l].d_pt4_ok);
         if (c->lv[l].dN) (void)hipFree(c->lv[l].dN);
         if (c->lv[l].p4) { (void)hipFree(c->lv[l].p4); (void)hipFree(c->lv[l].pal); (void)hipFree(c->lv[l].d_pal_n); }
+        if (c->lv[l].d16) (void)hipFree(c->lv[l].d16);
     }
     if (c->pal_work) (void)hipFree(c->pal_work);
     if (c->d_order) (void)hipFree(c->d_order);
@@ -1102,10 +1120,11 @@
     Level &L = c->lv[level];
     const bool compact = native_compact_wanted(c);
     if (compact && (rc = ensure_compact_slabs(c, level))) return rc;
+    if (compact) try_dense_slab(c, level);
     const bool defer = compact && L.tex_sparse;
     if (L.tex_sparse && !compact && (rc = map_texels(c, level, pair, 1))) return rc;
     HIPCHK(c, launch_edges_to_now(d_edge, 0, ImgBatch{rows, cols, 1}, work, defer ? nullptr : L.tex + (size_t)pair * L.tex_stride, L.tex_stride,
-                                  compact ? L.p4 : nullptr, L.p4_stride, L.pal, L.d_pal_n, pair, c->stream));
+                                  compact ? L.p4 : nullptr, L.p4_stride, L.pal, L.d_pal_n, pair, c->stream, false, L.d16, L.d16_stride));
     if (defer) {
         int n_failed = 0;
         if ((rc = sparse_map_compact_failures(c, level, pair, 1, c->stream, &n_failed))) return rc;
@@ -1211,7 +1230,7 @@
             int rc = now_written(c, l, w_first, w_count);
             if (rc) return rc;
             if (any_compact) {
-                HIPCHK(c, launch_replicate_compact(L.p4, L.p4_stride, L.pal, L.d_pal_n, n_src, dst_first, dst_count, c->stream));
+                HIPCHK(c, launch_replicate_compact(L.p4, L.p4_stride, L.pal, L.d_pal_n, L.d16, L.d16_stride, n_src, dst_first, dst_count, c->stream));
                 for (int p = dst_first; p < dst_first + dst_count; p++) {
                     const int src = (p - dst_first) % n_src;
                     if (p == src) continue;
@@ -1914,6 +1933,15 @@
     *used = (v >= 0 && (v & DVO_TEXMODE_RANKS_LDS)) ? 1 : 0;
     return DVO_OK;
 }
+int dvo_get_level_dense_lines(dvo_ctx *c, int pair, int level, int *used) {
+    DVO_ENTER(c);
+    if (!pair_ok(c, pair) || !level_ok(level) || !used) return fail(c, DVO_ERR_INVALID, "bad arguments");
+    HIPCHK(c, stream_wait(c->stream));
+    int v = -1;
+    HIPCHK(c, hipMemcpy(&v, c->d_tex_mode + (size_t)pair * DVO_LEVELS + level, sizeof(int), hipMemcpyDeviceToHost));
+    *used = (v >= 0 && (v & DVO_TEXMODE_DENSE)) ? 1 : 0;
+    return DVO_OK;
+}
 int dvo_get_level_exact_fallback(dvo_ctx *c, int pair, int level, int *ran) {
     DVO_ENTER(c);
     if (!pair_ok(c, pair) || !level_ok(level) || !ran) return fail(c, DVO_ERR_INVALID, "bad arguments");
diff --git a/rgbd_odometry_amd/csrc/dvo_ctx.h b/rgbd_odometry_amd/csrc/dvo_ctx.h
--- a/rgbd_odometry_amd/csrc/dvo_ctx.h
+++ b/rgbd_odometry_amd/csrc/dvo_ctx.h
@@ -40,6 +40,9 @@
     float2 *pal = nullptr;
     int *d_pal_n = nullptr;
     size_t p4_stride = 0;
+    unsigned short *d16 = nullptr;
+    size_t d16_stride = 0;
+    bool d16_failed = false;
     std::vector<char> pal_built;
     std::vector<int> now_uses;
     std::vector<char> tex16_stale;
diff --git a/rgbd_odometry_amd/csrc/dvo_edt_band.h b/rgbd_odometry_amd/csrc/dvo_edt_band.h
--- a/rgbd_odometry_amd/csrc/dvo_edt_band.h
+++ b/rgbd_odometry_amd/csrc/dvo_edt_band.h
@@ -35,6 +35,7 @@
     unsigned *imax[DVO_LEVELS]; int *done[DVO_LEVELS]; int *flags[DVO_LEVELS];
     const int *partial[DVO_LEVELS];
     unsigned *p4[DVO_LEVELS]; size_t p4_stride[DVO_LEVELS]; float2 *pal[DVO_LEVELS]; int *pal_n[DVO_LEVELS];
+    unsigned short *d16[DVO_LEVELS]; size_t d16_stride[DVO_LEVELS];
     int *list;
 };
 
@@ -329,6 +330,26 @@
             }
         }
     }
+    if (t.d16[l]) {
+        typedef __attribute__((address_space(3))) const unsigned lds_cu;
+        unsigned short *d16 = t.d16[l] + (size_t)(t.first_pair + by) * t.d16_stride[l];
+        if (band == 0 && tid < 8) reinterpret_cast<uint4 *>(d16)[tid] = make_uint4(0u, 0u, 0u, 0u);
+        const int ntx = d16_tiles_per_row(cols), n_items = ntx * nty * 8;
+        for (int k = tid; k < n_items; k += THREADS) {
+            const int scol = k & 7, rest = k >> 3, tx = rest / nty, tyl = rest - tx * nty;
+            int x = tx * DVO_D16_SIDE + scol - 1;
+            x = x < cols ? x : cols;
+            lds_cu *pc = (lds_cu *)(size_t)(tq_lds + (unsigned)((EB_PAD + x) * CB + tyl * 12));
+            const int ys = (ty0 + tyl) * DVO_D16_SIDE - 1;
+            unsigned v[4];
+#pragma unroll
+            for (int q = 0; q < 4; q++) {
+                const unsigned keep = (ys + 2 * q <= rows ? 0x0000ffffu : 0u) | (ys + 2 * q + 1 <= rows ? 0xffff0000u : 0u);
+                v[q] = (pc[q] << 3) & 0xfff8fff8u & keep;
+            }
+            *reinterpret_cast<uint4 *>(d16 + d16_slot(tx, ty0 + tyl, scol, 0, tpc)) = make_uint4(v[0], v[1], v[2], v[3]);
+        }
+    }
     EDT_T(t_words);
     EDT_ACC(3, t_scanned, t_words);
 
@@ -396,7 +417,7 @@
         }
         if (w == nw - 1) {
             pal[r] = make_float2(0.0f, 0.0f); pal[r + 1] = make_float2(0.0f, 0.0f);
-            t.pal_n[l][pair] = r | ((f & (int)EDT_FLAG_PARTIAL) ? DVO_PAL_PARTIAL : 0);
+            t.pal_n[l][pair] = r | ((f & (int)EDT_FLAG_PARTIAL) ? DVO_PAL_PARTIAL : 0) | (t.d16[l] ? DVO_PAL_DENSE : 0);
         }
     }
 }
diff --git a/rgbd_odometry_amd/csrc/dvo_frames.hip b/rgbd_odometry_amd/csrc/dvo_frames.hip
--- a/rgbd_odometry_amd/csrc/dvo_frames.hip
+++ b/rgbd_odometry_amd/csrc/dvo_frames.hip
@@ -1765,6 +1765,7 @@
     unsigned short *g[DVO_LEVELS]; unsigned *d2[DVO_LEVELS]; int *partial[DVO_LEVELS]; unsigned *bitmap[DVO_LEVELS]; int *flags[DVO_LEVELS];
     float4 *tex[DVO_LEVELS]; size_t tex_stride[DVO_LEVELS];
     unsigned *p4[DVO_LEVELS]; size_t p4_stride[DVO_LEVELS]; float2 *pal[DVO_LEVELS]; int *pal_n[DVO_LEVELS];
+    unsigned short *d16[DVO_LEVELS]; size_t d16_stride[DVO_LEVELS];
 };
 template <int WAVES>
 __global__ void __launch_bounds__(WAVES * 64) edt_columns8_levels_kernel(const EdtLevels t) {
@@ -1937,6 +1938,7 @@
         tb.edge[l] = t.edge[l]; tb.edge_stride[l] = t.edge_stride[l];
         tb.flags[l] = t.flags[l]; tb.partial[l] = t.partial[l];
         tb.p4[l] = t.p4[l]; tb.p4_stride[l] = t.p4_stride[l]; tb.pal[l] = t.pal[l]; tb.pal_n[l] = t.pal_n[l];
+        tb.d16[l] = t.d16[l]; tb.d16_stride[l] = t.d16_stride[l];
         tb.firstA[l + 1] = tb.firstA[l] + (unsigned)((t.cols[l] + 31) / 32);
         tb.firstB[l + 1] = tb.firstB[l] + (unsigned)tb.nbands[l];
         const int ngroups = (t.cols[l] + sh.waves - 1) / sh.waves;
@@ -1967,7 +1969,7 @@
 
 hipError_t launch_edges_to_now(const unsigned char *edge, size_t edge_stride, ImgBatch gb, int *work,
                                float4 *tex_out, size_t tex_stride, unsigned *p4, size_t p4_stride, float2 *pal, int *pal_n,
-                               int first_pair, hipStream_t s, bool only_texels) {
+                               int first_pair, hipStream_t s, bool only_texels, unsigned short *d16, size_t d16_stride) {
     const int R = edt_rows_per_block(gb.cols);
     const unsigned nblk = edt_row_blocks(gb.rows, gb.cols);
     const int bm_words = edt_bitmap_words(gb.rows, gb.cols);
@@ -1986,6 +1988,7 @@
         t.edge[0] = edge; t.edge_stride[0] = edge_stride;
         t.g[0] = g; t.d2[0] = d2; t.partial[0] = partial; t.bitmap[0] = bitmap; t.flags[0] = flags;
         t.p4[0] = p4; t.p4_stride[0] = p4_stride; t.pal[0] = pal; t.pal_n[0] = pal_n;
+        t.d16[0] = d16; t.d16_stride[0] = d16_stride;
         EdtLevelShape sh;
         const size_t lds_wave = 16;
         sh.R = R; sh.waves = (R <= 8) ? 8 : 4; sh.lds_cols = lds_wave * sh.waves; sh.lds_rows = edt_pk_lds_bytes(gb.cols, R);
@@ -2107,6 +2110,7 @@
         w += (edt_level_ints(rows[l], cols[l], sh.R, count) + 3) & ~(size_t)3;
         t.tex[l] = tex_out[l]; t.tex_stride[l] = tex_stride[l];
         t.p4[l] = with_p4 ? p4[l] : nullptr; t.p4_stride[l] = p4_stride[l]; t.pal[l] = pal[l]; t.pal_n[l] = pal_n[l];
+        t.d16[l] = nullptr; t.d16_stride[l] = 0;
         const int pty = (p4_tiles_per_col(rows[l]) + PK_LR - 1) / PK_LR, ptx = (((cols[l] + 3) >> 2) + PK_LC - 1) / PK_LC;
         long long strip = (long long)count * pty * ptx / 2048;
         strip = strip < 1 ? 1 : (strip > pty ? pty : strip);
diff --git a/rgbd_odometry_amd/csrc/dvo_fused.hip b/rgbd_odometry_amd/csrc/dvo_fused.hip
--- a/rgbd_odometry_amd/csrc/dvo_fused.hip
+++ b/rgbd_odometry_amd/csrc/dvo_fused.hip
@@ -52,7 +52,7 @@
         for (int j = i; j < 6; j++) a.H[i * 6 - (i * (i - 1)) / 2 + (j - i)] = fma(jwd[i], Jd[j], a.H[i * 6 - (i * (i - 1)) / 2 + (j - i)]);
 }
 
-enum { TEX_G16 = DVO_TEXMODE_GLOBAL16, TEX_L16 = DVO_TEXMODE_LDS16, TEX_P4 = DVO_TEXMODE_PAL4, TEX_R16 = 3 };
+enum { TEX_G16 = DVO_TEXMODE_GLOBAL16, TEX_L16 = DVO_TEXMODE_LDS16, TEX_P4 = DVO_TEXMODE_PAL4, TEX_R16 = 3, TEX_D16 = 4 };
 
 struct TexSrc {
     const char *g16;
@@ -61,6 +61,8 @@
     const char *p4;
     unsigned p4_col_bytes;
     unsigned r16_org, r16_col_bytes, r16_sent;
+    const char *d16;
+    unsigned d16_col_bytes;
 };
 
 struct __attribute__((packed, aligned(4))) U3 { unsigned a, b, c; };
@@ -78,6 +80,11 @@
     v2f xn, yn, zn;
     unsigned c0, u0, d0, l0, r0, c1, u1, d1, l1, r1;
 };
+template <> struct Round2<TEX_D16> {
+    v2f xn, yn, zn;
+    uint2 m0, m1;
+    unsigned l0, r0, l1, r1;
+};
 typedef const __attribute__((address_space(3))) unsigned short lds_cushort;
 
 typedef const __attribute__((address_space(3))) float lds_cfloat;
@@ -93,6 +100,18 @@
     const unsigned ty = __umul24((unsigned)yy, 43691u) >> 18;
     return __umul24((unsigned)(xx >> 2), p4_col_bytes) + 128u  + (((unsigned)xx & 3u) << 5) + ((unsigned)yy << 2) + __umul24(ty, 104u);
 }
+
+DVO_DEV unsigned d16_centre_offset(int yy, int xx, unsigned d16_col_bytes ) {
+    static_assert(DVO_D16_SIDE == 6, "written for 6 x 6 interior pixels per line");
+    const unsigned tx = __umul24((unsigned)xx, 43691u) >> 18, ty = __umul24((unsigned)yy, 43691u) >> 18;
+    return __umul24(tx, d16_col_bytes - 96u) + __umul24(ty, 116u) + ((unsigned)xx << 4) + ((unsigned)yy << 1) + 146u;
+}
+DVO_DEV void d16_gather(const char *base, unsigned o, uint2 &m, unsigned &l, unsigned &r) {
+    const unsigned short *q = reinterpret_cast<const unsigned short *>(base + o);
+    __builtin_memcpy(&m, q - 1, 8);
+    l = q[-8]; r = q[8];
+}
+DVO_DEV void d16_unpack(const uint2 &m, unsigned &c, unsigned &u, unsigned &d) { u = m.x & 0xffffu; c = m.x >> 16; d = m.y & 0xffffu; }
 
 struct LdsPoints {
     const uint2 *p;
@@ -174,7 +193,7 @@
     const v2f Y = (Z * (yy - c.pcy)) * c.pfy;
     v2f xn, yn, zn, u, v;
 #ifndef DVO_NO_VALU_DIET
-    if constexpr (TEX == TEX_P4 || TEX == TEX_R16) {
+    if constexpr (TEX == TEX_P4 || TEX == TEX_R16 || TEX == TEX_D16) {
         lanemask odd;
         project_point2m(c, X, Y, Z, xn, yn, zn, u, v, odd);
         any_odd |= (odd != 0ull);
@@ -191,6 +210,11 @@
             b.l0 = *(lds_cushort *)(size_t)(a0 + 2u - ts.r16_col_bytes); b.r0 = *(lds_cushort *)(size_t)(a0 + 2u + ts.r16_col_bytes);
             b.u1 = *(lds_cushort *)(size_t)(a1);     b.c1 = *(lds_cushort *)(size_t)(a1 + 2u); b.d1 = *(lds_cushort *)(size_t)(a1 + 4u);
             b.l1 = *(lds_cushort *)(size_t)(a1 + 2u - ts.r16_col_bytes); b.r1 = *(lds_cushort *)(size_t)(a1 + 2u + ts.r16_col_bytes);
+        } else if constexpr (TEX == TEX_D16) {
+            const unsigned o0 = select_or(vis0, d16_centre_offset(py0, px0, ts.d16_col_bytes), DVO_D16_SENTINEL_BYTE);
+            const unsigned o1 = select_or(vis1, d16_centre_offset(py1, px1, ts.d16_col_bytes), DVO_D16_SENTINEL_BYTE);
+            d16_gather(ts.d16, o0, b.m0, b.l0, b.r0);
+            d16_gather(ts.d16, o1, b.m1, b.l1, b.r1);
         } else {
             const unsigned o0 = select_or_zero(vis0, p4_byte_offset(py0, px0, ts.p4_col_bytes));
             const unsigned o1 = select_or_zero(vis1, p4_byte_offset(py1, px1, ts.p4_col_bytes));
@@ -219,6 +243,10 @@
         b.l0 = *(lds_cushort *)(size_t)(a0 + 2u - ts.r16_col_bytes); b.r0 = *(lds_cushort *)(size_t)(a0 + 2u + ts.r16_col_bytes);
         b.u1 = *(lds_cushort *)(size_t)(a1);     b.c1 = *(lds_cushort *)(size_t)(a1 + 2u); b.d1 = *(lds_cushort *)(size_t)(a1 + 4u);
         b.l1 = *(lds_cushort *)(size_t)(a1 + 2u - ts.r16_col_bytes); b.r1 = *(lds_cushort *)(size_t)(a1 + 2u + ts.r16_col_bytes);
+    } else if constexpr (TEX == TEX_D16) {
+        nvis += __popcll(__builtin_amdgcn_ballot_w64(vis0)) + __popcll(__builtin_amdgcn_ballot_w64(vis1));
+        d16_gather(ts.d16, vis0 ? d16_centre_offset(py0, px0, ts.d16_col_bytes) : DVO_D16_SENTINEL_BYTE, b.m0, b.l0, b.r0);
+        d16_gather(ts.d16, vis1 ? d16_centre_offset(py1, px1, ts.d16_col_bytes) : DVO_D16_SENTINEL_BYTE, b.m1, b.l1, b.r1);
     } else if constexpr (TEX == TEX_P4) {
         nvis += __popcll(__builtin_amdgcn_ballot_w64(vis0)) + __popcll(__builtin_amdgcn_ballot_w64(vis1));
         unsigned o0 = p4_byte_offset(py0, px0, ts.p4_col_bytes);
@@ -297,13 +325,20 @@
 DVO_DEV void round2_compute(const IterConst &c, const Round2<TEX> &b, ACC &a) {
     v2f jw[6], J[6];
     float eps0, eps1;
-    if constexpr (TEX == TEX_R16) {
-        const v2f pw0 = *(lds_cv2f *)(size_t)(PAL + b.c0), pw1 = *(lds_cv2f *)(size_t)(PAL + b.c1);
+    if constexpr (TEX == TEX_R16 || TEX == TEX_D16) {
+        unsigned c0, u0, d0, l0, r0, c1, u1, d1, l1, r1;
+        if constexpr (TEX == TEX_D16) {
+            d16_unpack(b.m0, c0, u0, d0); d16_unpack(b.m1, c1, u1, d1);
+            l0 = b.l0; r0 = b.r0; l1 = b.l1; r1 = b.r1;
+        } else {
+            c0 = b.c0; u0 = b.u0; d0 = b.d0; l0 = b.l0; r0 = b.r0; c1 = b.c1; u1 = b.u1; d1 = b.d1; l1 = b.l1; r1 = b.r1;
+        }
+        const v2f pw0 = *(lds_cv2f *)(size_t)(PAL + c0), pw1 = *(lds_cv2f *)(size_t)(PAL + c1);
         v2f pu, pd, pr, pl, dt, wt;
-        pu.x = *(lds_cfloat *)(size_t)(PAL + b.u0); pu.y = *(lds_cfloat *)(size_t)(PAL + b.u1);
-        pd.x = *(lds_cfloat *)(size_t)(PAL + b.d0); pd.y = *(lds_cfloat *)(size_t)(PAL + b.d1);
-        pr.x = *(lds_cfloat *)(size_t)(PAL + b.r0); pr.y = *(lds_cfloat *)(size_t)(PAL + b.r1);
-        pl.x = *(lds_cfloat *)(size_t)(PAL + b.l0); pl.y = *(lds_cfloat *)(size_t)(PAL + b.l1);
+        pu.x = *(lds_cfloat *)(size_t)(PAL + u0); pu.y = *(lds_cfloat *)(size_t)(PAL + u1);
+        pd.x = *(lds_cfloat *)(size_t)(PAL + d0); pd.y = *(lds_cfloat *)(size_t)(PAL + d1);
+        pr.x = *(lds_cfloat *)(size_t)(PAL + r0); pr.y = *(lds_cfloat *)(size_t)(PAL + r1);
+        pl.x = *(lds_cfloat *)(size_t)(PAL + l0); pl.y = *(lds_cfloat *)(size_t)(PAL + l1);
         dt.x = pw0.x; dt.y = pw1.x; wt.x = pw0.y; wt.y = pw1.y;
         const v2f gx = (pr - pl) * 0.5f, gy = (pd - pu) * 0.5f;
         eps0 = dt.x; eps1 = dt.y;
@@ -865,6 +900,7 @@
         const int img_words = r16 ? r16_words : 0;
         const bool pt4 = !TEAM && mode == TEX_P4 && !r16 && !sc.no_pt4 && N >= sc.pt4_factor * (((lds_words - pal_words - img_words) >> 1) & ~1) && L.pt4_ok &&
                          __builtin_amdgcn_readfirstlane(L.pt4_ok[dpair]) != 0;
+        const bool d16 = !TEAM && !WITH_H && mode == TEX_P4 && !r16 && !sc.no_d16 && L.d16 != nullptr && pal_dense(pal_n_raw);
         float *const lds_pts = lds_dyn + pal_words + img_words;
         const int cap = (mode == TEX_L16) ? n_pad
                         : (pt4 ? ((lds_words - pal_words - img_words) & ~1) : (((lds_words - pal_words - img_words) >> 1) & ~1));
@@ -933,6 +969,8 @@
         ts.r16_org = kStatic + 4u * (unsigned)pal_words;
         ts.r16_col_bytes = 2u * (unsigned)r16_col;
         ts.r16_sent = ts.r16_org + 2u * (unsigned)(r16_col * (L.cols + 2) + r16_col);
+        ts.d16 = reinterpret_cast<const char *>(L.d16 + (size_t)dpair * L.d16_stride);
+        ts.d16_col_bytes = (unsigned)d16_tiles_per_col(L.rows) * 128u;
         if (r16) {
             unsigned short *img = reinterpret_cast<unsigned short *>(lds_dyn + pal_words);
             const int wv = tid >> 6, ln = tid & 63;
@@ -976,6 +1014,12 @@
             } else if (r16) {
                 accumulate_points2<BLOCK, true, TEX_R16, 2, kStatic, false, Acc7T<WITH_H>>(c, ts, lp, gpts, 0, n_lds, lane_off, a, any_odd);
                 accumulate_points2<BLOCK, false, TEX_R16, 2, kStatic, false, Acc7T<WITH_H>>(c, ts, lp, gpts, n_lds, N, lane_off, a, any_odd);
+            } else if (d16 && pt4) {
+                accumulate_points2<BLOCK, true, TEX_D16, (WITH_H ? 2 : DVO_P4_DEPTH(BLOCK)), kStatic, true, Acc7T<WITH_H>>(c, ts, lp, gpts, 0, n_lds, lane_off, a, any_odd);
+                accumulate_points2<BLOCK, false, TEX_D16, (WITH_H ? 2 : DVO_P4_DEPTH(BLOCK)), kStatic, true, Acc7T<WITH_H>>(c, ts, lp, gpts, n_lds, N, lane_off, a, any_odd);
+            } else if (d16) {
+                accumulate_points2<BLOCK, true, TEX_D16, (WITH_H ? 2 : DVO_P4_DEPTH(BLOCK)), kStatic, false, Acc7T<WITH_H>>(c, ts, lp, gpts, 0, n_lds, lane_off, a, any_odd);
+                accumulate_points2<BLOCK, false, TEX_D16, (WITH_H ? 2 : DVO_P4_DEPTH(BLOCK)), kStatic, false, Acc7T<WITH_H>>(c, ts, lp, gpts, n_lds, N, lane_off, a, any_odd);
             } else if (mode == TEX_P4 && pt4) {
                 accumulate_points2<BLOCK, true, TEX_P4, (WITH_H ? 2 : DVO_P4_DEPTH(BLOCK)), kStatic, true, Acc7T<WITH_H>>(c, ts, lp, gpts, 0, n_lds, lane_off, a, any_odd);
                 accumulate_points2<BLOCK, false, TEX_P4, (WITH_H ? 2 : DVO_P4_DEPTH(BLOCK)), kStatic, true, Acc7T<WITH_H>>(c, ts, lp, gpts, n_lds, N, lane_off, a, any_odd);
@@ -1110,7 +1154,7 @@
                 out.best_idx[pair * DVO_LEVELS + l] = st.bestItr;
                 out.ratio[pair * DVO_LEVELS + l] = st.bestRatio;
                 out.tex_mode[pair * DVO_LEVELS + l] = mode | (st.exact_ran ? DVO_TEXMODE_EXACT_RAN : 0) | (pt4 ? DVO_TEXMODE_PT4 : 0) | (r16 ? DVO_TEXMODE_RANKS_LDS : 0) |
-                                                       (min(st.e2_ran, DVO_TEXMODE_E2_MAX) << DVO_TEXMODE_E2_SHIFT);
+                                                       (d16 ? DVO_TEXMODE_DENSE : 0) | (min(st.e2_ran, DVO_TEXMODE_E2_MAX) << DVO_TEXMODE_E2_SHIFT);
             }
         }
         __syncthreads();
diff --git a/rgbd_odometry_amd/csrc/dvo_kernels.hip b/rgbd_odometry_amd/csrc/dvo_kernels.hip
--- a/rgbd_odometry_amd/csrc/dvo_kernels.hip
+++ b/rgbd_odometry_amd/csrc/dvo_kernels.hip
@@ -214,7 +214,7 @@
 }
 
 __global__ void __launch_bounds__(256)
-replicate_compact_kernel(unsigned *p4, size_t p4_stride, float2 *pal, int *pal_n, int n_src, int dst_first) {
+replicate_compact_kernel(unsigned *p4, size_t p4_stride, float2 *pal, int *pal_n, unsigned short *d16, size_t d16_stride, int n_src, int dst_first) {
     const int p = dst_first + blockIdx.y;
     const int src = blockIdx.y % n_src;
     if (p == src) return;
@@ -230,11 +230,16 @@
     float2 *dp = pal + (size_t)p * DVO_PAL_MAX;
     const size_t n_copy = (size_t)n + (pal_partial(pn) ? 2 : 1);
     for (size_t i = (size_t)blockIdx.x * blockDim.x + threadIdx.x; i < n_copy; i += stride) dp[i] = sp[i];
-}
-hipError_t launch_replicate_compact(unsigned *p4, size_t p4_stride, float2 *pal, int *pal_n, int n_src, int dst_first,
+    if (d16 && pal_dense(pn)) {
+        const uint4 *s16 = reinterpret_cast<const uint4 *>(d16 + (size_t)src * d16_stride);
+        uint4 *d16d = reinterpret_cast<uint4 *>(d16 + (size_t)p * d16_stride);
+        for (size_t i = (size_t)blockIdx.x * blockDim.x + threadIdx.x; i < d16_stride / 8; i += stride) d16d[i] = s16[i];
+    }
+}
+hipError_t launch_replicate_compact(unsigned *p4, size_t p4_stride, float2 *pal, int *pal_n, unsigned short *d16, size_t d16_stride, int n_src, int dst_first,
                                     int dst_count, hipStream_t s) {
     if (dst_count <= 0) return hipSuccess;
-    hipLaunchKernelGGL(replicate_compact_kernel, dim3(32, dst_count), dim3(256), 0, s, p4, p4_stride, pal, pal_n, n_src, dst_first);
+    hipLaunchKernelGGL(replicate_compact_kernel, dim3(32, dst_count), dim3(256), 0, s, p4, p4_stride, pal, pal_n, d16, d16_stride, n_src, dst_first);
     return hipGetLastError();
 }
 
diff --git a/rgbd_odometry_amd/csrc/dvo_launch.h b/rgbd_odometry_amd/csrc/dvo_launch.h
--- a/rgbd_odometry_amd/csrc/dvo_launch.h
+++ b/rgbd_odometry_amd/csrc/dvo_launch.h
@@ -14,7 +14,8 @@
        DVO_TEXMODE_EXACT_RAN = 0x100 ,
        DVO_TEXMODE_PT4 = 0x200       ,
        DVO_TEXMODE_E2_SHIFT = 12, DVO_TEXMODE_E2_MAX = 0xffff ,
-       DVO_TEXMODE_RANKS_LDS = 0x400  };
+       DVO_TEXMODE_RANKS_LDS = 0x400 ,
+       DVO_TEXMODE_DENSE = 0x800      };
 
 namespace dvo {
 
@@ -34,6 +35,8 @@
     const float2 *pal;
     const int *pal_n;
     size_t p4_stride;
+    const unsigned short *d16;
+    size_t d16_stride;
 };
 struct LevelSet { LevelSlab l[DVO_LEVELS]; };
 
@@ -59,6 +62,7 @@
     int final_blk;
     int team_no_plain;
     int no_r16;
+    int no_d16;
     unsigned team_epoch0;
     int team_solo_max;
 };
@@ -99,7 +103,7 @@
 hipError_t launch_points4_build(const uint2 *cpts, const int *N, int pt_cap, int rows, unsigned *cpt4, unsigned *chdr, int *pt4_ok,
                                 int first_pair, int count, hipStream_t s);
 hipError_t launch_final_permute(const unsigned *cidx, const float *fe_blk, const float *fr_blk, int n, float *fe, float *fr, hipStream_t s);
-hipError_t launch_replicate_compact(unsigned *p4, size_t p4_stride, float2 *pal, int *pal_n, int n_src, int dst_first,
+hipError_t launch_replicate_compact(unsigned *p4, size_t p4_stride, float2 *pal, int *pal_n, unsigned short *d16, size_t d16_stride, int n_src, int dst_first,
                                     int dst_count, hipStream_t s);
 hipError_t launch_align_fused(int block_threads, int points_in_flight, const LevelSet &lv,
                               const Schedule &sc, const Intrinsics &K, const DevParams &prm,
@@ -187,7 +191,7 @@
 size_t edt_work_ints(int rows, int cols, int count);
 hipError_t launch_edges_to_now(const unsigned char *edge, size_t edge_stride, ImgBatch g, int *work,
                                float4 *tex_out, size_t tex_stride, unsigned *p4, size_t p4_stride, float2 *pal, int *pal_n,
-                               int first_pair, hipStream_t s, bool only_texels = false);
+                               int first_pair, hipStream_t s, bool only_texels = false, unsigned short *d16 = nullptr, size_t d16_stride = 0);
 hipError_t launch_p4_decode_texels(const unsigned *p4, size_t p4_stride, const float2 *pal, const int *pal_n, float4 *tex,
                                    size_t tex_stride, int rows, int cols, int first_pair, int count, hipStream_t s);
 size_t enlist_block_ints(int rows, int cols);
diff --git a/rgbd_odometry_amd/csrc/dvo_palette.h b/rgbd_odometry_amd/csrc/dvo_palette.h
--- a/rgbd_odometry_amd/csrc/dvo_palette.h
+++ b/rgbd_odometry_amd/csrc/dvo_palette.h
@@ -9,6 +9,9 @@
 #define DVO_PAL_PARTIAL (1 << 20)
 #define DVO_PAL_CAP_PARTIAL 4094
 #define DVO_P4_ROWS 6
+#define DVO_PAL_DENSE (1 << 21)
+#define DVO_D16_SIDE 6
+#define DVO_D16_LEVELS 2
 #define DVO_EDT_BITMAP_BITS (1 << 18)
 
 namespace dvo {
@@ -25,5 +28,19 @@
     return 32u + ((size_t)(xx >> 2) * tiles_per_col + ty) * 32u + (size_t)((xx & 3) * 8 + srow);
 }
 
+__host__ __device__ inline bool pal_dense(int pal_n) { return pal_n > 0 && (pal_n & DVO_PAL_DENSE) != 0; }
+__host__ __device__ inline int d16_tiles_per_col(int rows) { return (rows + DVO_D16_SIDE - 1) / DVO_D16_SIDE; }
+__host__ __device__ inline int d16_tiles_per_row(int cols) { return (cols + DVO_D16_SIDE - 1) / DVO_D16_SIDE; }
+__host__ __device__ inline size_t d16_count(int rows, int cols) {
+    return ((size_t)d16_tiles_per_col(rows) * (size_t)d16_tiles_per_row(cols) + 1u) * 64u;
+}
+__host__ __device__ inline size_t d16_slot(int tx, int ty, int scol, int srow, int tiles_per_col) {
+    return 64u + ((size_t)tx * tiles_per_col + ty) * 64u + (size_t)(scol * 8 + srow);
+}
+__host__ __device__ inline size_t d16_byte_offset(int yy, int xx, int tiles_per_col) {
+    return 2u * d16_slot(xx / DVO_D16_SIDE, yy / DVO_D16_SIDE, xx % DVO_D16_SIDE + 1, yy % DVO_D16_SIDE + 1, tiles_per_col);
+}
+#define DVO_D16_SENTINEL_BYTE 18u
+
 }
 #endif
```

After: 810,500 (median of 6 runs). 1.4% higher.
